# tensor4all/tensor4all-rs

Measured on AMD Instinct MI355X. Metric: TCI2 full-sweep GF/s (d=30, chi=256 fp64), higher is better.
Workload: dtype f64

## Files before the change

include/t4a_gpu.h:

```cpp
#ifndef T4A_GPU_H
#define T4A_GPU_H

#include <stddef.h>
#include <stdint.h>

#ifdef __cplusplus
extern "C" {
#endif
#if defined(__GNUC__)
#pragma GCC visibility push(default)
#endif

typedef int32_t t4a_gpu_status;
#define T4A_GPU_SUCCESS 0
#define T4A_GPU_NULL_POINTER (-1)
#define T4A_GPU_INVALID_ARGUMENT (-2)
#define T4A_GPU_BUFFER_TOO_SMALL (-5)
#define T4A_GPU_INTERNAL_ERROR (-6)
#define T4A_GPU_NOT_IMPLEMENTED (-7)
#define T4A_GPU_NAN_ENCOUNTERED (-8)
#define T4A_GPU_SINGULAR_MATRIX (-9)
#define T4A_GPU_NO_DEVICE (-10)
#define T4A_GPU_KERNEL_TIMEOUT (-11)
#define T4A_GPU_CALLBACK_ERROR (-12)
// ... 372 lines not shown
t4a_gpu_status t4a_gpu_mpo_from_tt(const t4a_gpu_tt* tt, t4a_gpu_mpo** out);
t4a_gpu_status t4a_gpu_mpo_to_tt(const t4a_gpu_mpo* mpo, t4a_gpu_tt** out);
t4a_gpu_status t4a_gpu_mpo_transpose(const t4a_gpu_mpo* mpo, t4a_gpu_mpo** out);

typedef struct t4a_gpu_qt_op t4a_gpu_qt_op;
#define T4A_GPU_QT_PERIODIC 0
#define T4A_GPU_QT_ANTIPERIODIC 1
#define T4A_GPU_QT_OPEN 2
#define T4A_GPU_QT_LOWER 0
#define T4A_GPU_QT_UPPER 1
t4a_gpu_status t4a_gpu_qt_shift_operator(size_t r, int64_t offset, int32_t bc, t4a_gpu_qt_op** out);
t4a_gpu_status t4a_gpu_qt_shift_operator_multivar(size_t r, int64_t offset, int32_t bc, size_t nvariables, size_t target_var,
                                                  t4a_gpu_qt_op** out);
t4a_gpu_status t4a_gpu_qt_flip_operator(size_t r, int32_t bc, t4a_gpu_qt_op** out);
t4a_gpu_status t4a_gpu_qt_flip_operator_multivar(size_t r, int32_t bc, size_t nvariables, size_t target_var, t4a_gpu_qt_op** out);
t4a_gpu_status t4a_gpu_qt_triangle_operator(size_t r, int32_t triangle, t4a_gpu_qt_op** out);
t4a_gpu_status t4a_gpu_qt_cumsum_operator(size_t r, t4a_gpu_qt_op** out);
t4a_gpu_status t4a_gpu_qt_affine_operator(size_t r, const int64_t* a, size_t a_len, const int64_t* b, size_t b_len, int64_t scale,
                                          size_t m, size_t n, const int32_t* bc, size_t n_bc, t4a_gpu_qt_op** out);
void t4a_gpu_qt_op_release(t4a_gpu_qt_op* h);
t4a_gpu_status t4a_gpu_qt_op_len(const t4a_gpu_qt_op* h, size_t* out);
t4a_gpu_status t4a_gpu_qt_op_dims(const t4a_gpu_qt_op* h, size_t* dims4 );
t4a_gpu_status t4a_gpu_qt_op_site_tensor(const t4a_gpu_qt_op* h, size_t site, double* out);
t4a_gpu_status t4a_gpu_qt_op_to_mpo(const t4a_gpu_qt_op* h, t4a_gpu_mpo** out);
t4a_gpu_status t4a_gpu_qt_difference_kernel(const t4a_gpu_tt* f, int32_t bc, t4a_gpu_mpo** out);

t4a_gpu_status t4a_gpu_tt_to_tensors(const t4a_gpu_tt* tt, const int64_t* site_labels, const int64_t* bond_labels,
                                     t4a_gpu_tensor** out);
t4a_gpu_status t4a_gpu_tensors_to_tt(const t4a_gpu_tensor* const* tensors, size_t n_sites, t4a_gpu_tt** out);

typedef struct t4a_gpu_aci_options {
    size_t max_iters;
    size_t min_iters;
    int32_t has_max_bond_dim;
    size_t max_bond_dim;
    double tolerance;
    int32_t scale_tolerance;
    uint64_t rng_seed;
    int32_t enable_global_guard;
    size_t nsearch_global_pivots;
    size_t max_nglobal_pivot;
    size_t nsweeps_global_search;
    double tol_margin_global_search;
} t4a_gpu_aci_options;
t4a_gpu_status t4a_gpu_aci_options_default(t4a_gpu_aci_options* opts);
typedef int32_t (*t4a_gpu_aci_op_fn)(void* user, const double* values, size_t n_inputs, size_t n_points, double* out);
#define T4A_GPU_ACI_OP_CALLBACK 0
#define T4A_GPU_ACI_OP_PRODUCT 1
#define T4A_GPU_ACI_OP_SUM 2
t4a_gpu_status t4a_gpu_aci_elementwise(const t4a_gpu_tt* const* inputs, size_t n_inputs, int32_t op_kind, t4a_gpu_aci_op_fn op,
                                       void* user, const t4a_gpu_aci_options* options, const t4a_gpu_tt* initial_guess,
                                       t4a_gpu_tt** result, size_t* n_iters, size_t* ranks, double* errors,
                                       size_t* nglobal_pivots, int32_t* termination);
typedef struct t4a_gpu_aci_problem t4a_gpu_aci_problem;
t4a_gpu_status t4a_gpu_aci_problem_new(const t4a_gpu_tt* const* inputs, size_t n_inputs, int32_t op_kind, t4a_gpu_aci_op_fn op,
                                       void* user, const t4a_gpu_aci_options* options, const t4a_gpu_tt* initial_guess,
                                       t4a_gpu_aci_problem** out);
void t4a_gpu_aci_problem_release(t4a_gpu_aci_problem* h);
t4a_gpu_status t4a_gpu_aci_problem_local_update(t4a_gpu_aci_problem* h, size_t bond, int32_t left_orthogonal);
t4a_gpu_status t4a_gpu_aci_problem_add_global_pivots(t4a_gpu_aci_problem* h, const size_t* pivots, size_t n_pivots,
                                                     size_t* added);
t4a_gpu_status t4a_gpu_aci_problem_find_global_pivots(t4a_gpu_aci_problem* h, uint64_t seed, size_t* count, size_t* out);
t4a_gpu_status t4a_gpu_aci_problem_solution(t4a_gpu_aci_problem* h, t4a_gpu_tt** out);
t4a_gpu_status t4a_gpu_aci_problem_frame(t4a_gpu_aci_problem* h, int32_t right, size_t input, size_t site, size_t* rows,
                                         size_t* cols, double* out);
t4a_gpu_status t4a_gpu_aci_problem_errors(const t4a_gpu_aci_problem* h, double* pivot_errors, double* pivot_scales);

t4a_gpu_status t4a_gpu_treeaci_local_update_f64(size_t n_inputs, const size_t* bond_dims, const double* const* row_frames,
                                                const double* const* col_frames, size_t row_count, size_t col_count, int32_t op_kind,
                                                t4a_gpu_aci_op_fn op, void* user, size_t max_bond_dim, double tolerance,
                                                int32_t scale_tolerance, int32_t left_orthogonal, size_t* rank, size_t* row_indices,
                                                size_t* col_indices, double* pivot_errors, size_t* n_pivot_errors, double* left,
                                                double* right, double* sampled_scale, double* local_values);

t4a_gpu_status t4a_gpu_tci2_last_sweep_shapes(const t4a_gpu_tci2* h, size_t* out);
#define T4A_GPU_PROFILE_SLOTS 16
t4a_gpu_status t4a_gpu_tci2_profile_enable(t4a_gpu_tci2* h, int32_t enable);
t4a_gpu_status t4a_gpu_tci2_profile_reset(t4a_gpu_tci2* h);
t4a_gpu_status t4a_gpu_tci2_profile_get(const t4a_gpu_tci2* h, double* out );
t4a_gpu_status t4a_gpu_tci2_profile_variants(const t4a_gpu_tci2* h, double* out , size_t cap_rows, size_t* n_rows);

t4a_gpu_status t4a_gpu_tci2_chain_stats(const t4a_gpu_tci2* h, uint64_t* out );
t4a_gpu_status t4a_gpu_tci2_chain_stats_ext(const t4a_gpu_tci2* h, uint64_t* out );
t4a_gpu_status t4a_gpu_tci2_fill_stats(const t4a_gpu_tci2* h, uint64_t* out );
t4a_gpu_status t4a_gpu_tci2_rook_stats(const t4a_gpu_tci2* h, uint64_t* out );
t4a_gpu_status t4a_gpu_tci2_optimize_group(t4a_gpu_tci2* const* handles, size_t n_handles, const t4a_gpu_tci2_options* options,
                                           int32_t final_sweep1site);
t4a_gpu_status t4a_gpu_tci2_fill_site_tensors_group(t4a_gpu_tci2* const* handles, size_t n_handles);
t4a_gpu_status t4a_gpu_tci2_set_chain(t4a_gpu_tci2* h, int32_t enable, int32_t verify);
t4a_gpu_status t4a_gpu_tci2_set_callback_threads(t4a_gpu_tci2* h, size_t n_threads);
t4a_gpu_status t4a_gpu_tci2_small_stats(const t4a_gpu_tci2* h, uint64_t* out );

t4a_gpu_status t4a_gpu_fn_eval(int32_t fid, int32_t n_acc, const double* params, const uint64_t* weights,
                               const size_t* local_dims, size_t n_sites, const size_t* idx, size_t n_pts,
                               double* out);

#if defined(__GNUC__)
#pragma GCC visibility pop
#endif
#ifdef __cplusplus
}
#endif
#endif
```

tensor4all-rs_amd/build.py:

```python
#!/usr/bin/env python3
import os
import subprocess
import sys
from concurrent.futures import ThreadPoolExecutor

HERE = os.path.dirname(os.path.abspath(__file__))
CSRC = os.path.join(HERE, "csrc")
OUT = os.path.join(HERE, "lib")
OBJ = os.path.join(HERE, "build")
SOURCES = ["kernels_rrlu.hip", "kernels_rrlu_reg.hip", "rrlu_xcd_plan.hip", "kernels_rrlu_xcd2.hip", "kernels_rrlu_xcd2_group.hip", "kernels_rrlu_xcd2m.hip", "kernels_rrlu_wg.hip", "kernels_rrlu_wg_group.hip", "kernels_rrlu_w1.hip", "kernels_rrlu_global.hip", "kernels_pi.hip", "kernels_chain.hip", "kernels_small.hip", "kernels_dense.hip", "kernels_linalg.hip",
           "kernels_tt.hip", "kernels_mpo.hip", "pool.hip", "engine.hip", "rook.hip", "tt.hip", "mpo.hip", "globalsearch.hip", "tci2.hip", "tci2_chain.hip", "tci2_small.hip", "conversion.hip", "patching.hip", "tree.hip", "quantics.hip", "tensorops.hip", "aci.hip", "quanticstransform.hip", "capi.hip"]
FLAGS = ["--offload-arch=gfx950", "-O3", "-std=c++17", "-fPIC", "-ffp-contract=off", "-Wall", "-Wno-unused-function",
         "-fvisibility=hidden"] + os.environ.get("T4A_EXTRA_FLAGS", "").split()
FILE_FLAGS = {"kernels_dense.hip": ["-mllvm", "-amdgpu-mfma-vgpr-form=1"], "kernels_linalg.hip": ["-ffp-contract=fast"]}
HEADERS = ["common.hpp", "stdrng.hpp", "pishard.hpp", "kernels.hpp", "kernels_rrlu_xcd_common.hpp", "kernels_rrlu_w1_body.hpp", "engine.hpp", "tci2.hpp", "tt.hpp", "mpo.hpp", "globalsearch.hpp", "rook.hpp", "patching.hpp", "tree.hpp", "quantics.hpp", "tensorops.hpp", "aci.hpp", "quanticstransform.hpp", "../../include/t4a_gpu.h",
           "../../include/t4a_testfunctions.h"]


_INC_CACHE = {}


def _includes(path):
    path = os.path.normpath(path)
    if path in _INC_CACHE:
        return _INC_CACHE[path]
    _INC_CACHE[path] = set()
    found = set()
    try:
        with open(path) as f:
            text = f.read()
    except OSError:
        return found
    import re
    for inc in re.findall(r'^\s*#\s*include\s+"([^"]+)"', text, flags=re.M):
        cand = os.path.normpath(os.path.join(os.path.dirname(path), inc))
        if os.path.exists(cand):
            found.add(cand)
            found |= _includes(cand)
    _INC_CACHE[path] = found
    return found


def _newer(target, deps):
    if not os.path.exists(target):
        return True
    t = os.path.getmtime(target)
    return any(os.path.getmtime(d) > t for d in deps)


def build(force=False, verbose=True):
    hipcc = os.environ.get("HIPCC", "/opt/rocm/bin/hipcc")
    os.makedirs(OUT, exist_ok=True)
    os.makedirs(OBJ, exist_ok=True)
    stamp = os.path.join(OBJ, "flags.stamp")
    flags_now = " ".join(FLAGS) + " | " + repr(sorted(FILE_FLAGS.items()))
    try:
        with open(stamp) as f:
            flags_then = f.read()
    except OSError:
        flags_then = None
    if flags_then != flags_now:
        force = True
    hdrs = [os.path.join(CSRC, h) for h in HEADERS]
    jobs = []
    objs = []
    for s in SOURCES:
        src = os.path.join(CSRC, s)
        obj = os.path.join(OBJ, s.replace(".hip", ".o"))
        objs.append(obj)
        if force or _newer(obj, [src] + sorted(_includes(src))):
            jobs.append([hipcc] + FLAGS + FILE_FLAGS.get(s, []) + ["-c", src, "-o", obj])

    def run(cmd):
        if verbose:
            print(" ".join(cmd), flush=True)
        subprocess.check_call(cmd)

    with ThreadPoolExecutor(max_workers=4) as ex:
        list(ex.map(run, jobs))
    lib = os.path.join(OUT, "libt4a_gpu.so")
    if force or jobs or not os.path.exists(lib):
        run([hipcc, "--offload-arch=gfx950", "-shared", "-fPIC", "-o", lib] + objs)
    with open(stamp, "w") as f:
        f.write(flags_now)
    hooks = os.path.join(OUT, "libt4a_gpu_testhooks.so")
    src = os.path.join(CSRC, "tci2.hip")
    hobj = os.path.join(OBJ, "tci2_testhooks.obj")
    if force or jobs or _newer(hobj, [src] + sorted(_includes(src))) or not os.path.exists(hooks):
        run([hipcc] + FLAGS + ["-DT4A_TEST_HOOKS", "-c", src, "-o", hobj])
        run([hipcc, "--offload-arch=gfx950", "-shared", "-fPIC", "-o", hooks] + [o for o in objs if os.path.basename(o) != "tci2.o"] + [hobj])
    return lib


if __name__ == "__main__":
    print(build(force="--force" in sys.argv))
```

tensor4all-rs_amd/csrc/capi.hip:

```cpp
#include "stdrng.hpp"
#include "smallrng.hpp"
#include <memory>
#include <initializer_list>
#include <mutex>

#include "patching.hpp"
#include "tci2.hpp"
#include "tree.hpp"
#include "quantics.hpp"
#include "tensorops.hpp"
#include "aci.hpp"
#include "globalsearch.hpp"
#include "mpo.hpp"
#include "quanticstransform.hpp"

struct t4a_gpu_tci2 {
    t4a::Tci2 impl;
    explicit t4a_gpu_tci2(const std::vector<size_t>& d) : impl(d) {}
};

struct t4a_gpu_treetci {
    t4a::TreeTci impl;
    t4a_gpu_treetci(const std::vector<size_t>& d, const t4a::TreeGraph& g) : impl(d, g) {}
};
// ... 1084 lines not shown
        h->impl.keep_site_tensors = keep != 0;
    });
}

t4a_gpu_status t4a_gpu_tci2_last_sweep_shapes(const t4a_gpu_tci2* h, size_t* out)
{
    return guarded([&] {
        T4A_REQUIRE_PTR(h);
        T4A_REQUIRE_PTR(out);
        for (size_t b = 0; b < h->impl.last_sweep_shapes.size(); ++b)
            for (int k = 0; k < 3; ++k) out[3 * b + k] = h->impl.last_sweep_shapes[b][k];
    });
}

t4a_gpu_status t4a_gpu_tci2_profile_enable(t4a_gpu_tci2* h, int32_t enable)
{
    return guarded([&] {
        T4A_REQUIRE_PTR(h);
        h->impl.eng.prof.enabled = enable != 0;
    });
}
t4a_gpu_status t4a_gpu_tci2_profile_reset(t4a_gpu_tci2* h)
{
    return guarded([&] {
        T4A_REQUIRE_PTR(h);
        for (double& v : h->impl.eng.prof.v) v = 0.0;
        h->impl.eng.variant_stats_.clear();
    });
}
t4a_gpu_status t4a_gpu_tci2_profile_get(const t4a_gpu_tci2* h, double* out)
{
    return guarded([&] {
        T4A_REQUIRE_PTR(h);
        T4A_REQUIRE_PTR(out);
        for (int i = 0; i < T4A_GPU_PROFILE_SLOTS; ++i) out[i] = h->impl.eng.prof.v[i];
        double best = -1.0;
        for (const auto& kv : h->impl.eng.variant_stats_)
            if (kv.second[0] > best) {
                best = kv.second[0];
                out[12] = kv.second[0];
                out[13] = kv.second[1];
                out[14] = kv.second[2];
                out[15] = (double)kv.first;
            }
    });
}
t4a_gpu_status t4a_gpu_tci2_profile_variants(const t4a_gpu_tci2* h, double* out, size_t cap_rows, size_t* n_rows)
{
    return guarded([&] {
        T4A_REQUIRE_PTR(h);
        T4A_REQUIRE_PTR(n_rows);
        const auto& vs = h->impl.eng.variant_stats_;
        *n_rows = vs.size();
        if (out == nullptr) return;
        if (cap_rows < vs.size()) throw Error(T4A_GPU_BUFFER_TOO_SMALL, "profile_variants: buffer too small");
        size_t i = 0;
        for (const auto& kv : vs) {
            out[5 * i + 0] = (double)kv.first;
            for (int j = 0; j < 4; ++j) out[5 * i + 1 + j] = kv.second[j];
            ++i;
        }
    });
}


t4a_gpu_status t4a_gpu_tci2_chain_stats(const t4a_gpu_tci2* h, uint64_t* out)
{
    return guarded([&] {
        T4A_REQUIRE_PTR(h);
        T4A_REQUIRE_PTR(out);
        for (int k = 0; k < 5; ++k) out[k] = h->impl.chain_stats[k];
    });
}

t4a_gpu_status t4a_gpu_tci2_chain_stats_ext(const t4a_gpu_tci2* h, uint64_t* out)
{
    return guarded([&] {
        T4A_REQUIRE_PTR(h);
        T4A_REQUIRE_PTR(out);
        for (int k = 0; k < 4; ++k) out[k] = h->impl.chain_stats_ext[k];
    });
}

t4a_gpu_status t4a_gpu_tci2_rook_stats(const t4a_gpu_tci2* h, uint64_t* out)
{
    return guarded([&] {
        T4A_REQUIRE_PTR(h);
        T4A_REQUIRE_PTR(out);
        const RookWork& w = h->impl.rook_work();
        out[0] = w.n_device_searches;
        out[1] = w.n_device_visits;
        out[2] = w.n_host_searches;
        out[3] = w.n_host_syncs;
    });
}

t4a_gpu_status t4a_gpu_tci2_fill_stats(const t4a_gpu_tci2* h, uint64_t* out)
{
    return guarded([&] {
        T4A_REQUIRE_PTR(h);
        T4A_REQUIRE_PTR(out);
        for (int k = 0; k < 3; ++k) out[k] = h->impl.fill_stats()[k];
    });
}

t4a_gpu_status t4a_gpu_tci2_set_chain(t4a_gpu_tci2* h, int32_t enable, int32_t verify)
{
    return guarded([&] {
        T4A_REQUIRE_PTR(h);
        h->impl.chain_enabled = enable != 0;
        h->impl.chain_verify = (verify & 1) != 0;
        h->impl.chain_event_timing = (verify & 2) != 0;
        h->impl.small_enabled = (verify & 4) == 0;
        h->impl.small_stamps = (verify & 8) != 0;
        h->impl.fill_graph_relaxed = (verify & 16) != 0;
        h->impl.small_tile_max = (verify & 32) ? 32 : 16;
    });
}

t4a_gpu_status t4a_gpu_tci2_set_callback_threads(t4a_gpu_tci2* h, size_t n_threads)
{
    return guarded([&] {
        T4A_REQUIRE_PTR(h);
        if (n_threads < 1 || n_threads > 256) throw Error(T4A_GPU_INVALID_ARGUMENT, "callback threads: between 1 and 256");
        h->impl.callback_threads = n_threads;
    });
}

t4a_gpu_status t4a_gpu_tci2_small_stats(const t4a_gpu_tci2* h, uint64_t* out)
{
    return guarded([&] {
        T4A_REQUIRE_PTR(h);
        T4A_REQUIRE_PTR(out);
        for (int k = 0; k < 4; ++k) out[k] = h->impl.small_stats[k];
        for (int k = 0; k < 3; ++k) out[4 + k] = h->impl.small_last_clocks_[k];
        out[7] = (uint64_t)h->impl.small_last_reason_;
        for (int k = 0; k < 8; ++k) out[8 + k] = h->impl.small_last_clocks_[3 + k];
    });
}

extern "C++" {
static void rook_outputs(Engine& e, const LuciResult& r, size_t m, size_t n, size_t* rank, size_t* rows, size_t* cols,
                         double* pivot_errors, double* left, double* right)
{
    *rank = (size_t)r.rank;
    for (int i = 0; i < r.rank; ++i) {
        rows[i] = (size_t)r.row_perm[i];
        cols[i] = (size_t)r.col_perm[i];
    }
    for (size_t i = 0; i < r.pivot_errors.size(); ++i) pivot_errors[i] = r.pivot_errors[i];
    if (r.rank > 0) {
        download(e, left, e.left(), m * (size_t)r.rank);
        download(e, right, e.right(), n * (size_t)r.rank);
    }
}
static RookWork& dense_rook_work()
{
    static RookWork w;
    return w;
}
}

t4a_gpu_status t4a_gpu_luci_blocks_f64(size_t m, size_t n, t4a_gpu_fill_block_fn fill_block, void* ctx,
                                       size_t max_bond_dim, double rel_tol, double abs_tol, int32_t left_orthogonal,
                                       size_t* rank, size_t* rows, size_t* cols, double* pivot_errors, double* left,
                                       double* right)
{
    return guarded([&] {
        T4A_REQUIRE_PTR(rank);
        T4A_REQUIRE_PTR(rows);
        T4A_REQUIRE_PTR(cols);
        T4A_REQUIRE_PTR(pivot_errors);
        const size_t count = checked_mul(m, n, "matrix shape");
        require_int_dims({m, n}, "matrix shape");
        if (count) {
            T4A_REQUIRE_PTR(fill_block);
            T4A_REQUIRE_PTR(left);
            T4A_REQUIRE_PTR(right);
        }
        if (m > 65535 || n > 65535) throw Error(T4A_GPU_NOT_IMPLEMENTED, "luci: dimensions above 65535 are not supported");
        std::lock_guard<std::mutex> lock(g_dense_mutex);
        Engine& e = dense_engine();
        hipStream_t st = e.stream();
        std::vector<size_t> all_rows(m), all_cols(n);
        for (size_t i = 0; i < m; ++i) all_rows[i] = i;
        for (size_t j = 0; j < n; ++j) all_cols[j] = j;
        std::vector<double> hbuf(std::max(m, n));
        RookSource src;
        src.M = (int)m;
        src.N = (int)n;
        src.column = [&](int c, double* d_out) {
            const size_t cc = (size_t)c;
            fill_block(ctx, all_rows.data(), m, &cc, 1, hbuf.data());
            T4A_HIP(hipMemcpyAsync(d_out, hbuf.data(), m * sizeof(double), hipMemcpyHostToDevice, st));
            T4A_HIP(hipStreamSynchronize(st));
        };
        src.row = [&](int r, double* d_out) {
            const size_t rr = (size_t)r;
            fill_block(ctx, &rr, 1, all_cols.data(), n, hbuf.data());
// ... 2350 lines not shown
```

tensor4all-rs_amd/csrc/engine.hip:

```cpp
#include "engine.hpp"

#include <algorithm>
#include <cmath>
#include <cstdio>
#include <cstdlib>
#include <cstring>
#include <atomic>
#include <condition_variable>
#include <mutex>

namespace t4a {

namespace {
thread_local std::string g_last_error;

__global__ void __launch_bounds__(256) tri_extract_kernel(const double* __restrict__ in, int ldi, int rows, int cols,
                                                          int keep_lower, int unit_diag, double* __restrict__ out,
                                                          int ldo)
{
    const int i = blockIdx.x * blockDim.x + threadIdx.x;
    if (i >= rows) return;
    for (int j = blockIdx.y; j < cols; j += gridDim.y) {
        double v;
        if (i == j)
// ... 37 lines not shown
                                std::getenv("T4A_WG_MIN") ? std::atol(std::getenv("T4A_WG_MIN")) : 64};
    return env;
}
void acquire_for(XcdArbiter::Lock& lock, RrluLock scope, int xcc)
{
    if (scope != RrluLock::None) lock.acquire(scope == RrluLock::Chip ? -1 : xcc);
}
void reg_args(RrluRegArgs& a, const RrluRoute& rt, bool left, const double* A, int max_steps, double rel_tol, double abs_tol, const RrluBlock& blk)
{
    std::memset(&a, 0, sizeof(a));
    a.A = A;
    a.M = rt.kM;
    a.N = rt.kN;
    a.max_steps = max_steps;
    a.rel_tol = rel_tol;
    a.abs_tol = abs_tol;
    a.tie_row_major = left ? 0 : 1;
    a.out_transposed = left ? 0 : 1;
    a.W = rt.reg.W;
    a.TR = rt.reg.TR;
    a.TC = rt.reg.TC;
    a.row_perm = left ? blk.row_perm() : blk.col_perm();
    a.col_perm = left ? blk.col_perm() : blk.row_perm();
    a.iresult = blk.iresult();
    a.dresult = blk.dresult();
    a.pivot_vals = blk.pivot_vals();
    a.ncopy = 1;
    a.spec = 2;
    a.spec_frac = 0.8;
    a.key16 = 1;
    a.spin_limit = 1u << 20;
    a.h_block = reinterpret_cast<unsigned long long*>(blk.host);
    a.block_u64 = (int)(blk.bytes / 8);
    a.ts_u64 = (int)(blk.off_ts / 8);
}
}

RrluRoute RrluRoute::of_xcd(const RrluXcdPlan& plan, int kM, int kN)
{
    RrluRoute rt;
    rt.kind = plan.wg == 2 ? RrluKind::OneWave : plan.wg ? RrluKind::OneWorkgroup : plan.big() ? RrluKind::MultiXcd : RrluKind::SingleXcd;
    rt.xcd = plan;
    rt.kM = kM;
    rt.kN = kN;
    return rt;
}
RrluRoute RrluRoute::of_reg(const RrluRegPlan& plan, int kM, int kN)
{
    RrluRoute rt;
    rt.kind = RrluKind::Reg;
    rt.reg = plan;
    rt.kM = kM;
    rt.kN = kN;
    rt.fused = plan.RPT * plan.CPT <= RRLU_FUSED_MAX_VALUES;
    return rt;
}
int RrluRoute::code(bool tie_row_major, bool saturated) const
{
    const int tie = tie_row_major ? 4 : 0, sat = saturated ? 10000000 : 0;
    switch (kind) {
    case RrluKind::OneWave: return sat + 300000 + xcd.RPT * 1000 + xcd.CPT * 10 + tie;
    case RrluKind::OneWorkgroup: return sat + 200000 + xcd.RPT * 1000 + xcd.CPT * 10 + tie;
    case RrluKind::SingleXcd: return sat + 100000 + xcd.RPT * 100 + xcd.CPT * 10 + tie;
    case RrluKind::MultiXcd: return sat + 400000 + xcd.K * 10000 + xcd.RPT * 100 + xcd.CPT * 10 + tie;
    case RrluKind::Reg: return sat + reg.RPT * 1000 + reg.CPT * 10 + tie + (reg.W == 1 ? 2 : 0) + ((reg.TR % 64) == 0 ? 1 : 0);
    case RrluKind::Lds: return sat + (lds.W == 1 ? -1 : -2);
    case RrluKind::Global: return sat - 3;
    default: return 0;
    }
}
RrluLock RrluRoute::lock() const
{
    switch (kind) {
    case RrluKind::OneWave:
    case RrluKind::OneWorkgroup:
    case RrluKind::SingleXcd:
    case RrluKind::MultiXcd:
        return xcd.W > kXcdSharedMaxW || xcd.K > 1 ? RrluLock::Chip : RrluLock::Xcd;
    case RrluKind::Reg: return reg.W > 1 ? RrluLock::Chip : RrluLock::None;
    case RrluKind::Lds: return lds.W > 1 ? RrluLock::Chip : RrluLock::None;
    default: return RrluLock::None;
    }
}
size_t RrluRoute::xcd_mailbox_words() const { return (rrlu_xcd_keys_bytes(xcd) + rrlu_xcd_cols_bytes(xcd, kM)) / sizeof(unsigned long long); }
void RrluRoute::launch(const RrluXcdArgs& args, hipStream_t stream) const
{
    switch (kind) {
    case RrluKind::OneWave: rrlu_w1_launch(xcd, args, stream); break;
    case RrluKind::OneWorkgroup: rrlu_wg_launch(xcd, args, stream); break;
    case RrluKind::SingleXcd: rrlu_xcd2_launch(xcd, args, stream); break;
    case RrluKind::MultiXcd: rrlu_xcd2m_launch(xcd, args, stream); break;
    default: throw Error(T4A_GPU_INTERNAL_ERROR, "rrLU: the route has no single-XCD launch");
    }
}
void RrluRoute::launch_group(const RrluXcdGroupArgs& args, bool tie_row_major, hipStream_t stream) const
{
    switch (kind) {
    case RrluKind::OneWave: rrlu_w1_group_launch(xcd, args, tie_row_major, stream); break;
    case RrluKind::OneWorkgroup: rrlu_wg_group_launch(xcd, args, tie_row_major, stream); break;
    case RrluKind::SingleXcd: rrlu_xcd2_group_launch(xcd, args, tie_row_major, stream); break;
    default: throw Error(T4A_GPU_INTERNAL_ERROR, "rrLU: the route has no group launch");
    }
}

RrluBlock RrluBlock::layout(size_t max_steps, size_t M, size_t N, bool with_timestamps)
{
    RrluBlock b;
    b.off_rp = b.off_piv + sizeof(double) * std::max<size_t>(max_steps, 1);
    b.off_cp = b.off_rp + sizeof(int) * M;
    const size_t end = (b.off_cp + sizeof(int) * N + 7) / 8 * 8;
    b.off_ts = with_timestamps ? end : 0;
    b.bytes = with_timestamps ? end + 16 : end;
    return b;
}

namespace {
__global__ void xcd_census_kernel(unsigned* counts)
{
    if (threadIdx.x == 0) {
        unsigned v;
        asm volatile("s_getreg_b32 %0, hwreg(HW_REG_XCC_ID)" : "=s"(v));
        atomicAdd(&counts[v & 0xF], 1u);
        if ((v & 0xF) != (blockIdx.x & 7u)) atomicAdd(&counts[16], 1u);
    }
}
std::once_flag g_census_once;
void xcd_census()
{
    if (g_xcd_disabled.load(std::memory_order_relaxed) || std::getenv("T4A_NO_XCD")) return;
    unsigned* d = nullptr;
    unsigned h[17] = {0};
    if (hipMalloc(&d, sizeof(h)) != hipSuccess) return;
    bool ok = hipMemset(d, 0, sizeof(h)) == hipSuccess;
    if (ok) {
        hipLaunchKernelGGL(xcd_census_kernel, dim3(256), dim3(64), 0, nullptr, d);
        ok = hipMemcpy(h, d, sizeof(h), hipMemcpyDeviceToHost) == hipSuccess;
    }
    (void)hipFree(d);
    if (!ok) {
        (void)hipGetLastError();
        return;
    }
    bool even = true;
    for (int x = 0; x < 8; ++x) even &= (h[x] == 32u);
    if (!even) xcd_disable();
}
}
int xcd_assign() { return g_xcd_next.fetch_add(1, std::memory_order_relaxed) & 7; }
int xcd_plan_max_w() { return g_live_engines.load(std::memory_order_relaxed) > 1 ? kXcdSharedMaxW : 32; }
namespace {
std::mutex g_arb_mutex;
std::condition_variable g_arb_cv;
std::thread::id g_arb_owner[8];
int g_arb_count[8] = {0, 0, 0, 0, 0, 0, 0, 0};
}
void XcdArbiter::Lock::acquire(int xcc)
{
    release();
    const std::thread::id me = std::this_thread::get_id();
    std::unique_lock<std::mutex> lk(g_arb_mutex);
    auto holds_some = [&] {
        for (int i = 0; i < 8; ++i)
            if (g_arb_count[i] > 0 && g_arb_owner[i] == me) return true;
        return false;
    };
    auto take = [&](int i) {
        g_arb_owner[i] = me;
        ++g_arb_count[i];
        held_ |= 1 << i;
    };
    owner_ = me;
    if (xcc >= 0) {
        const int i = xcc & 7;
// ... 501 lines not shown
    a.h_block = reinterpret_cast<unsigned long long*>(blk.host);
    a.block_u64 = (int)(blk.bytes / 8);
    a.ts_u64 = (int)(blk.off_ts / 8);
}

void Engine::rrlu_account(const RrluRoute& rt, bool tie_row_major, int M, int N, int rank, bool record, float ms, bool saturated)
{
    double bytes = 8.0 * M * N, flops = 0.0;
    for (int k = 0; k < rank; ++k) {
        const double mr = (double)(M - k - 1), nr = (double)(N - k - 1);
        bytes += 16.0 * mr * nr;
        flops += 2.0 * mr * nr + mr;
    }
    prof.v[8] += rank;
    prof.v[9] += bytes;
    prof.v[10] += flops;
    if (!record) return;
    auto add = [&](int code) {
        auto& vs = variant_stats_[code];
        vs[0] += ms;
        vs[1] += 1.0;
        vs[2] += bytes;
        vs[3] += rank;
    };
    add(rt.code(tie_row_major));
    if (saturated) add(rt.code(tie_row_major, true));
}

RrluRoute Engine::chain_route(int kM, int kN) const
{
    if (kM < 1 || kN < 1 || kM > 65535 || kN > 65535) return RrluRoute();
    RrluXcdPlan xplan;
    if ((long long)kM * kN > rrlu_env().wg_min && (rrlu_w1_make_plan(kM, kN, &xplan, 63) || rrlu_wg_make_plan(kM, kN, &xplan, 63)))
        return RrluRoute::of_xcd(xplan, kM, kN);
    RrluRegPlan rplan;
    if ((long long)kM * kN <= 64 * 64 && rrlu_reg_make_plan(kM, kN, num_cus_, &rplan) && rplan.W == 1) return RrluRoute::of_reg(rplan, kM, kN);
    if (!xcd_disabled() && (rrlu_xcd_make_plan(kM, kN, &xplan, true, xcd_plan_max_w()) || rrlu_xcd_make_plan(kM, kN, &xplan, true, 32, true)))
        return RrluRoute::of_xcd(xplan, kM, kN);
    return RrluRoute();
}

void Engine::chain_begin(const std::vector<RrluRoute>& routes, size_t reserve_mailbox_words)
{
    chain_group_reserve(routes, reserve_mailbox_words, stream_);
    RrluLock scope = RrluLock::None;
    for (const RrluRoute& rt : routes)
        if (rt.on_xcd()) scope = std::max(scope, rt.lock());
    acquire_for(chain_lock_, scope, xcc_);
}

void Engine::chain_end() { chain_lock_.release(); }

RrluRoute Engine::chain_group_route(int kM, int kN)
{
    if (kM < 1 || kN < 1 || kM > 1024 || kN > 1024 || xcd_disabled()) return RrluRoute();
    RrluXcdPlan xplan;
    if (rrlu_w1_make_plan(kM, kN, &xplan, 0) || rrlu_wg_make_plan(kM, kN, &xplan, 0) || rrlu_xcd_make_plan(kM, kN, &xplan, true, 32))
        return RrluRoute::of_xcd(xplan, kM, kN);
    return RrluRoute();
}

void Engine::chain_group_reserve(const std::vector<RrluRoute>& routes, size_t reserve_mailbox_words, hipStream_t order_stream)
{
    size_t need = 0;
    for (const RrluRoute& rt : routes)
        if (rt.on_xcd()) need = std::max(need, rt.xcd_mailbox_words());
    if (need > 0 && (need > d_xkeys_.cap || !d_xticket_.get())) xcd_mailbox_clear(std::max(need, reserve_mailbox_words), order_stream);
}

unsigned Engine::chain_group_args(const RrluRoute& rt, bool left, const double* d_a, const int* d_dims, size_t max_bond_dim, double rel_tol,
                                  double abs_tol, const RrluBlock& blk, int slot, RrluXcdArgs* out, hipStream_t order_stream)
{
    if (++xcd_salt_ > 65535u) {
        T4A_HIP(hipMemsetAsync(d_xkeys_.get(), 0, d_xkeys_.cap * sizeof(unsigned long long), order_stream));
        xcd_salt_ = 1;
    }
    xcd_args(*out, rt, left, d_a, chain_max_steps(rt, max_bond_dim), rel_tol, abs_tol, blk, slot);
    out->dims = d_dims;
    out->dims_swap = left ? 0 : 1;
    return xcd_salt_;
}

unsigned Engine::chain_rrlu(const RrluRoute& rt, bool left, const double* d_a, const int* d_rowmap, const FusedPi* fused, const int* d_dims,
                            size_t max_bond_dim, double rel_tol, double abs_tol, const RrluBlock& blk, const XcdSpecArgs* spec, double* d_aout, double* d_urows)
{
    unsigned token = 0u;
    if (rt.on_xcd()) {
        RrluXcdArgs a;
        token = chain_group_args(rt, left, d_a, d_dims, max_bond_dim, rel_tol, abs_tol, blk, xcc_, &a, stream_);
        a.rowmap = d_rowmap;
        a.Aout = d_aout;
        a.urows = d_aout ? d_urows : nullptr;
        if (spec) a.spec = *spec;
        rt.launch(a, stream_);
    } else {
        if (++done_token_ == 0u) ++done_token_;
        RrluRegArgs a;
        reg_args(a, rt, left, d_a, chain_max_steps(rt, max_bond_dim), rel_tol, abs_tol, blk);
        a.Aout = d_aout;
        a.salt = 1;
        a.fused = (rt.fused && fused) ? 1 : 0;
        if (a.fused) {
            a.rowacc = fused->d_rowacc;
            a.colacc = fused->d_colacc;
            a.fn = fused->fn;
        }
        a.dims = d_dims;
        a.dims_swap = left ? 0 : 1;
        a.rowmap = a.fused ? nullptr : d_rowmap;
        a.dev_token = done_token_;
        a.done_token = done_token_;
        rrlu_reg_launch(rt.reg, a, stream_, true);
        token = done_token_;
    }
    T4A_HIP(hipGetLastError());
    return token;
}

void Engine::build_factors(const LuciResult& r, bool left_orth) { build_factors_from(d_lu_.get(), d_rowperm_ptr_, d_colperm_ptr_, r.M, r.N, r.rank, left_orth); }

void Engine::build_factors_from(const double* lu, const int* d_rowperm_ptr_, const int* d_colperm_ptr_, int M, int N, int rk, bool left_orth)
{
    d_left_.reserve((size_t)M * (rk > 0 ? rk : 1));
    d_right_.reserve((size_t)N * (rk > 0 ? rk : 1));
    if (rk == 0) return;
    if (luci_factors_small_launch(lu, M, N, rk, d_rowperm_ptr_, d_colperm_ptr_, left_orth, d_left_.get(), d_right_.get(), stream_)) {
        T4A_HIP(hipGetLastError());
        return;
    }
    d_w1_.reserve((size_t)(M > N ? M : N) * rk + (size_t)rk * rk);
    d_w2_.reserve((size_t)(M > N ? M : N) * rk + (size_t)rk * rk);
    d_trsm_.reserve(1);
    h_trsm_.reserve(1);

    if (left_orth) {
        double* Wl = d_w1_.get();
        set_identity_launch(Wl, M, rk, M, stream_);
        if (rk < M) {
            double* Tt = d_w2_.get();
            double* Bt = d_w2_.get() + (size_t)rk * rk;
            transpose_launch(lu, rk, rk, M, Tt, rk, stream_);
            transpose_launch(lu + rk, M - rk, rk, M, Bt, rk, stream_);
            TrsmProblem tp;
            tp.T = Tt;
            tp.ldt = rk;
            tp.n = rk;
            tp.B = Bt;
            tp.ldb = rk;
            tp.nrhs = M - rk;
            tp.lower = 0;
            tp.unit_diag = 1;
            tp.skip_flag = nullptr;
            T4A_HIP(hipStreamSynchronize(stream_));
            *h_trsm_.get() = tp;
            T4A_HIP(hipMemcpyAsync(d_trsm_.get(), h_trsm_.get(), sizeof(TrsmProblem), hipMemcpyHostToDevice, stream_));
            trsm_left_batched_launch(d_trsm_.get(), 1, rk, M - rk, stream_);
            transpose_launch(Bt, rk, M - rk, rk, Wl + rk, M, stream_);
        }
        scatter_rows_launch(Wl, M, d_rowperm_ptr_, M, rk, d_left_.get(), M, stream_);
        double* L11 = d_w2_.get();
        double* Ue = d_w1_.get();
        tri_extract_launch(lu, M, rk, rk, 1, 1, L11, rk, stream_);
        tri_extract_launch(lu, M, rk, N, 0, 0, Ue, rk, stream_);
        double* Rp = d_w2_.get() + (size_t)rk * rk;
        GemmDesc g;
        g.m = rk;
        g.n = N;
        g.k = rk;
        g.A = L11;
        g.lda = rk;
        g.strideA = 0;
        g.transA = 0;
        g.B = Ue;
        g.ldb = rk;
        g.strideB = 0;
        g.transB = 0;
        g.C = Rp;
// ... 270 lines not shown
```

tensor4all-rs_amd/csrc/engine.hpp:

```cpp
#pragma once

#include <array>
#include <functional>
#include <thread>
#include <map>
#include <limits>
#include <vector>

#include "common.hpp"
#include "kernels.hpp"

namespace t4a {

struct RrLUOptions {
    size_t max_bond_dim = std::numeric_limits<size_t>::max();
    double rel_tol = 1e-14;
    double abs_tol = 0.0;
    bool left_orthogonal = true;
};

struct LuciResult {
    int M = 0, N = 0;
    int rank = 0;
    std::vector<int> row_perm, col_perm;
    std::vector<double> pivot_errors;
    double last_error = 0.0;
    double abs_max = 0.0;
    bool has_factors = false;
};

struct FusedPi {
    FnDevice fn;
    const uint64_t* d_rowacc;
    const uint64_t* d_colacc;
    bool host_resident = false;
};

struct Profile {
    double v[T4A_GPU_PROFILE_SLOTS] = {0};
    bool enabled = false;
};

bool xcd_disabled();
void xcd_disable();
int xcd_assign();
int xcd_plan_max_w();
struct XcdArbiter {
    class Lock {
    public:
        Lock() = default;
        Lock(const Lock&) = delete;
        Lock& operator=(const Lock&) = delete;
        ~Lock() { release(); }
        void acquire(int xcc);
        void release();
    private:
        int held_ = 0;
        std::thread::id owner_;
    };
};

enum class RrluKind {
    None,
    OneWave,
    OneWorkgroup,
    SingleXcd,
    MultiXcd,
    Reg,
    Lds,
    Global,
};
enum class RrluLock { None, Xcd, Chip };
struct RrluRoute {
    RrluKind kind = RrluKind::None;
    RrluXcdPlan xcd;
    RrluRegPlan reg;
    RrluPlan lds;
    int kM = 0, kN = 0;
    bool fused = false;

    static RrluRoute of_xcd(const RrluXcdPlan& plan, int kM, int kN);
    static RrluRoute of_reg(const RrluRegPlan& plan, int kM, int kN);
    bool ok() const { return kind != RrluKind::None; }
    bool on_xcd() const { return kind == RrluKind::OneWave || kind == RrluKind::OneWorkgroup || kind == RrluKind::SingleXcd || kind == RrluKind::MultiXcd; }
    int code(bool tie_row_major, bool saturated = false) const;
    RrluLock lock() const;
    size_t xcd_mailbox_words() const;
    void launch(const RrluXcdArgs& args, hipStream_t stream) const;
    void launch_group(const RrluXcdGroupArgs& args, bool tie_row_major, hipStream_t stream) const;
};

struct RrluBlock {
    char* dev = nullptr;
    char* host = nullptr;
    size_t off_piv = 32, off_rp = 0, off_cp = 0, off_ts = 0, bytes = 0;
    static RrluBlock layout(size_t max_steps, size_t M, size_t N, bool with_timestamps);
    double* dresult() const { return reinterpret_cast<double*>(dev); }
    int* iresult() const { return reinterpret_cast<int*>(dev + 16); }
    double* pivot_vals() const { return reinterpret_cast<double*>(dev + off_piv); }
    int* row_perm() const { return reinterpret_cast<int*>(dev + off_rp); }
    int* col_perm() const { return reinterpret_cast<int*>(dev + off_cp); }
};

class Engine {
public:
    Engine();
    ~Engine();
    Engine(const Engine&) = delete;
    Engine& operator=(const Engine&) = delete;

    hipStream_t stream() const { return stream_; }
    int num_cus() const { return num_cus_; }
    void sync() { T4A_HIP(hipStreamSynchronize(stream_)); }

    double* pi(size_t count)
    {
        d_pi_.reserve(count);
        return d_pi_.get();
    }
    double* lu_buf() { return d_lu_.get(); }
    double* left() { return d_left_.get(); }
    double* right() { return d_right_.get(); }
    void reserve_factors(size_t left_count, size_t right_count)
    {
        d_left_.reserve(left_count > 0 ? left_count : 1);
        d_right_.reserve(right_count > 0 ? right_count : 1);
    }

    LuciResult luci(const double* d_a, int M, int N, const RrLUOptions& opts, bool need_factors, bool want_lu_copy,
                    const FusedPi* fused = nullptr);

    void lu_permuted_factors(const LuciResult& r, bool left_orth);

    static constexpr size_t FACTOR_DIM_MAX = 65535;
    static void require_factor_dims(size_t m, size_t n, const std::string& what)
    {
        if (m > FACTOR_DIM_MAX || n > FACTOR_DIM_MAX)
            throw Error(T4A_GPU_NOT_IMPLEMENTED, what + " above " + std::to_string(FACTOR_DIM_MAX) + " are not supported");
    }
    void svd(const double* d_a, int M, int N, double* d_u, double* d_s, double* d_vt);
    void svd_plain(const double* d_a, int M, int N, double* d_u, double* d_s, double* d_vt);
    void svd_in_range(const double* d_a, int M, int N, double* d_u, double* d_s, double* d_vt);
    void qr(const double* d_a, int M, int N, double* d_q, double* d_r);

    RrluRoute chain_route(int kM, int kN) const;
    void chain_begin(const std::vector<RrluRoute>& routes, size_t reserve_mailbox_words = 0);
    unsigned chain_rrlu(const RrluRoute& rt, bool left, const double* d_a, const int* d_rowmap, const FusedPi* fused, const int* d_dims,
                        size_t max_bond_dim, double rel_tol, double abs_tol, const RrluBlock& blk, const XcdSpecArgs* spec, double* d_aout = nullptr, double* d_urows = nullptr);
    void chain_end();
    static RrluRoute chain_group_route(int kM, int kN);
    void chain_group_reserve(const std::vector<RrluRoute>& routes, size_t reserve_mailbox_words, hipStream_t order_stream);
    void chain_group_lock() { chain_lock_.acquire(-1); }
    unsigned chain_group_args(const RrluRoute& rt, bool left, const double* d_a, const int* d_dims, size_t max_bond_dim, double rel_tol,
                              double abs_tol, const RrluBlock& blk, int slot, RrluXcdArgs* out, hipStream_t order_stream);
    void rrlu_account(const RrluRoute& rt, bool tie_row_major, int M, int N, int rank, bool record, float ms, bool saturated);
    int xcc() const { return xcc_; }
    void set_xcc(int xcc) { xcc_ = xcc & 7; }

    std::function<void()> overlap_hook;

    Profile prof;
    std::map<int, std::array<double, 4>> variant_stats_;

    DevBuf<double> d_tmp, d_tmp2;

private:
    RrluRoute luci_route(int M, int N, bool left) const;
    void build_factors(const LuciResult& r, bool left_orth);
public:
    void build_factors_from(const double* d_lu, const int* d_rowperm, const int* d_colperm, int M, int N, int rank, bool left_orth);
private:

    XcdArbiter::Lock chain_lock_;
    hipStream_t stream_ = nullptr;
    int num_cus_ = 0;
    unsigned rrlu_salt_ = 0;
    int xcc_ = 0;
    bool nonfinite_retry_ = false;
    unsigned xcd_salt_ = 0, xcd_ticket_base_ = 0, xcd_ticket_base_multi_ = 0;
    void xcd_take_tickets(const RrluXcdPlan& plan, RrluXcdArgs& a);
    void xcd_mailbox_clear(size_t words, hipStream_t stream);
    void xcd_args(RrluXcdArgs& a, const RrluRoute& rt, bool left, const double* A, int max_steps, double rel_tol, double abs_tol,
                  const RrluBlock& blk, int xcc);
    DevBuf<unsigned long long> d_xkeys_;
    DevBuf<unsigned> d_xticket_;
    DevBuf<double> d_xurows_;
    bool header_clean_ = false, keys_clean_ = false;
    unsigned done_token_ = 0;
    DevBuf<uint64_t> d_accstage_;
    char* header_ptr_ = nullptr;
    int key_parity_ = 0;
    DevBuf<double> d_pi_, d_lu_, d_left_, d_right_, d_w1_, d_w2_, d_at_;
    DevBuf<char> d_out_;
    PinBuf<char> h_out_;
    int* d_rowperm_ptr_ = nullptr;
    int* d_colperm_ptr_ = nullptr;
    DevBuf<unsigned long long> d_keys_, d_cols_, d_rkeys_, d_rcols_, d_stamps_;
    DevBuf<TrsmProblem> d_trsm_;
    PinBuf<TrsmProblem> h_trsm_;
    DevBuf<int> d_gints_;
    DevBuf<double> d_gdbls_;
    EventTimer ev_rrlu_, ev_fac_;
#ifdef T4A_RRLU_TRACE
    DevBuf<unsigned long long> d_trace_;
    int trace_dumps_ = 0;
#endif
    DevBuf<double> d_sw_, d_sv_, d_su_, d_svs_, d_ssig_;
    DevBuf<double> d_pa_, d_pq_, d_pr_, d_pl_, d_pul_, d_pvl_, d_pu_;
    size_t svd_sweeps_last_ = 0;
    DevBuf<int> d_sflags_;
    DevBuf<unsigned long long> d_sabs_;
    DevBuf<double> d_sscaled_;
};

void tri_extract_launch(const double* in, int ldi, int rows, int cols, int keep_lower, int unit_diag, double* out,
                        int ldo, hipStream_t stream);

}
```

tensor4all-rs_amd/csrc/kernels.hpp:

```cpp
#pragma once

#include <hip/hip_runtime.h>

#include <cstddef>
#include <cstdint>

#include "../../include/t4a_testfunctions.h"

namespace t4a {

struct RrluWorkspace;

struct RrluPlan {
    int W = 1;
    int T = 256;
    int cpw = 0;
    int Mld = 0;
    size_t lds_bytes = 0;
};

RrluPlan rrlu_make_plan(int M, int N, int num_cus);

struct RrluArgs {
    const double* A;
// ... 74 lines not shown
    double* pivot_vals;
    unsigned long long* keys;
    unsigned long long* cols;
    unsigned salt;
    int col_delay;
    int poll_delay;
    int ncopy;
    int key16;
    int spec;
    double spec_frac;
    unsigned spin_limit;
    unsigned long long* stamps;
    unsigned long long* h_block;
    int block_u64;
    unsigned long long* keys_next;
    int keys_next_u64;
    unsigned long long* trace;
    int fused;
    const uint64_t* rowacc;
    const uint64_t* colacc;
    FnDevice fn;
    unsigned done_token;
    const int* dims;
    int dims_swap;
    unsigned dev_token;
    const int* rowmap;
    int ts_u64;
};
bool rrlu_reg_make_plan(int M, int N, int num_cus, RrluRegPlan* out);
size_t rrlu_reg_keys_bytes(const RrluRegPlan& plan);
size_t rrlu_reg_cols_bytes(const RrluRegPlan& plan, int M);
void rrlu_reg_launch(const RrluRegPlan& plan, const RrluRegArgs& args, hipStream_t stream, bool keys_zeroed = false);

struct XcdSpecArgs {
    double* out;
    const uint64_t* dep_acc;
    const uint64_t* w_site;
    const uint64_t* ext_acc;
    const int* ext_cnt;
    const uint64_t* ind_acc;
    const int* ind_cnt;
    unsigned* tile_counter;
    int total, d;
    FnDevice fn;
};
struct RrluXcdPlan {
    int W = 1;
    int RPT = 1, CPT = 1;
    int grid = 8;
    size_t lds_bytes = 0;
    int wg = 0;
    int K = 1;
    bool big() const { return K > 1 || RPT > 16; }
};
struct RrluXcdArgs {
    const double* A;
    double* Aout;
    double* urows;
    int M, N;
    int max_steps;
    double rel_tol, abs_tol;
    int tie_row_major;
    int out_transposed;
    int W;
    int xcc;
    unsigned* ticket;
    unsigned ticket_base;
    int* row_perm;
    int* col_perm;
    int* iresult;
    double* dresult;
    double* pivot_vals;
    unsigned long long* keys;
    unsigned salt;
    double spec_frac;
    unsigned long long* stamps;
    unsigned long long* h_block;
    int block_u64;
    const int* dims;
    int dims_swap;
    const int* rowmap;
    XcdSpecArgs spec;
    int ts_u64;
};
bool rrlu_xcd_make_plan(int M, int N, RrluXcdPlan* out, bool any_size = false, int max_w = 32, bool allow_big = false);
size_t rrlu_xcd_keys_bytes(const RrluXcdPlan& plan);
size_t rrlu_xcd_cols_bytes(const RrluXcdPlan& plan, int M);
struct RrluXcdGroupArgs {
    RrluXcdArgs p[8];
};
void rrlu_xcd2_launch(const RrluXcdPlan& plan, const RrluXcdArgs& args, hipStream_t stream);
void rrlu_xcd2m_launch(const RrluXcdPlan& plan, const RrluXcdArgs& args, hipStream_t stream);
void rrlu_xcd2_group_launch(const RrluXcdPlan& plan, const RrluXcdGroupArgs& args, bool tie_row_major, hipStream_t stream);
bool rrlu_wg_make_plan(int M, int N, RrluXcdPlan* out, int spec_blocks = 0);
void rrlu_wg_launch(const RrluXcdPlan& plan, const RrluXcdArgs& args, hipStream_t stream);
void rrlu_wg_group_launch(const RrluXcdPlan& plan, const RrluXcdGroupArgs& args, bool tie_row_major, hipStream_t stream);
bool rrlu_w1_make_plan(int M, int N, RrluXcdPlan* out, int spec_blocks = 0);
void rrlu_w1_launch(const RrluXcdPlan& plan, const RrluXcdArgs& args, hipStream_t stream);
void rrlu_w1_group_launch(const RrluXcdPlan& plan, const RrluXcdGroupArgs& args, bool tie_row_major, hipStream_t stream);

void pi_eval_launch(const FnDevice& fn, const uint64_t* rowacc, int M, const uint64_t* colacc, int N, double* out,
                    int ld, bool transpose_out, unsigned long long* max_abs_bits, hipStream_t stream);
struct PiJob {
    const uint64_t* rowacc;
    const uint64_t* colacc;
    double* out;
    unsigned long long* max_abs_bits;
    int M, N, ld, pad_;
};
void pi_eval_batched_launch(const FnDevice& fn, const PiJob* d_jobs, int n_jobs, int max_M, int max_N, hipStream_t stream);
struct PackJob {
    const double* src;
    double* core;
    const int* info;
    int ld, L, S, R, last, pad_;
};
struct LuProblem;
constexpr int FILL_SMALL_MAX_N = 32, FILL_SMALL_MAX_RHS = 64;
void fill_small_launch(const FnDevice& fn, const PiJob* d_pis, const LuProblem* d_lups, const PackJob* d_packs, int n_jobs, int last_site,
                       hipStream_t stream);
void stage_copy_launch(const uint64_t* pinned_src, uint64_t* dst, size_t count, hipStream_t stream);
void absmax_launch(const double* data, size_t count, unsigned long long* max_abs_bits, hipStream_t stream);

constexpr int CHAIN_MAX_SET = 1024;
struct ChainTab {
    uint64_t* code;
    uint64_t* acc;
    int* cnt;
};
struct ChainCommon {
    ChainTab I, J, HI, HJ;
    ChainTab mI, mJ;
    int cap, K;
    const uint64_t* w;
    int total;
    const int* ldim;
    const int* woff;
    int forward, use_extras;
    int one_site;
    uint64_t* ind_code;
    uint64_t* ind_acc;
    int* ind_cnt;
    int ind_cap;
    uint64_t* dep_code;
    uint64_t* dep_acc;
    int dep_cap;
    int* rowmap;
    int* dims;
    int* hdims;
    uint64_t* snap_dst;
    int* snap_cnt_dst;
    size_t snap_words;
    int n_sites;
    uint64_t* zero_a;
    size_t zero_a_words;
    uint64_t* zero_b;
    size_t zero_b_words;
};
struct ChainPrepArgs {
    int b;
    int do_build;
    int with_rowmap;
    int prev_b;
    const int* prev_iresult;
    const int* prev_rowperm;
    const int* prev_colperm;
    unsigned prev_token;
    unsigned long long* dbg;
    int defer_host_writes;
};
struct ChainWalkArgs {
    char* blocks;
    size_t block_bytes, off_piv, off_rp, off_cp, off_ts;
    double* pi;
    int n_bonds;
    int max_steps;
    double rel_tol, abs_tol;
    double* factors;
    size_t factors_stride;
    unsigned token_base;
    int timed;
    int lean_prep;
    unsigned long long* phase_ticks;
};
void chain_walk_launch(const ChainCommon& c, const FnDevice& fn, const ChainWalkArgs& w, int columns, hipStream_t stream);
void chain_indep_launch(const ChainCommon& c, int n_bonds, hipStream_t stream);
void chain_last_core_launch(const ChainCommon& c, const FnDevice& fn, double* core, int max_entries, hipStream_t stream);
void chain_prep_launch(const ChainCommon& c, const ChainPrepArgs& a, hipStream_t stream);
void chain_pi_launch(const ChainCommon& c, const FnDevice& fn, int b, int n_dep_ub, int n_ind_ub, double* out, hipStream_t stream);

constexpr int CHAIN_GROUP_MAX = 8;
struct ChainGroupSlot {
    ChainCommon c;
    FnDevice fn;
    double* pi;
};
struct ChainPrepGroupArgs {
    ChainPrepArgs a[CHAIN_GROUP_MAX];
};
void chain_indep_group_launch(const ChainGroupSlot* d_slots, int n_handles, int n_bonds, hipStream_t stream);
void chain_prep_group_launch(const ChainGroupSlot* d_slots, const ChainPrepGroupArgs& a, int n_handles, hipStream_t stream);
void chain_pi_group_launch(const ChainGroupSlot* d_slots, int n_handles, int b, int n_dep_ub, int n_ind_ub, hipStream_t stream);

struct GemmDesc {
    int m, n, k;
    const double* A; int lda; long long strideA; int transA;
    const double* B; int ldb; long long strideB; int transB;
    double* C; int ldc; long long strideC;
    double alpha, beta;
    int batch;
    int ksplit = 1;
    double* partial = nullptr;
};
void gemm_launch(const GemmDesc& d, hipStream_t stream);

constexpr int LUCI_LEFT_CORES_MAX_JOBS = 80;
constexpr int LUCI_LEFT_CORES_MAX_RANK = 16;
struct LeftCoreJob {
    const double* lu;
    const int* dims;
    const int* iresult;
    const int* row_perm;
    double* core;
    int S;
    unsigned token;
};
struct LeftCoreJobs {
    LeftCoreJob j[LUCI_LEFT_CORES_MAX_JOBS];
};
void luci_left_cores_batched_launch(const LeftCoreJobs& jobs, int n_jobs, int max_rows, hipStream_t stream);
bool luci_factors_small_launch(const double* lu, int M, int N, int rk, const int* row_perm, const int* col_perm, bool left_orth,
                               double* left, double* right, hipStream_t stream);
void transpose_launch(const double* in, int rows, int cols, int ldi, double* out, int ldo, hipStream_t stream);

struct TrsmProblem {
    const double* T; int ldt; int n;
    double* B; int ldb; int nrhs;
    int lower; int unit_diag;
    const int* skip_flag;
};
void trsm_left_batched_launch(const TrsmProblem* d_problems, int n_problems, int max_n, int max_nrhs, hipStream_t stream);

struct LuProblem {
    double* A; int lda; int n;
    int* piv;
    int* info;
    double* B; int ldb; int nrhs;
    const unsigned long long* pmax_bits;
};
void lu_batched_launch(const LuProblem* d_problems, int n_problems, int max_n, hipStream_t stream);
constexpr int LU_MAX_PANEL_STEPS = 128;
bool lu_forward_blocked_launch(const LuProblem* d_problems, int n_problems, int max_n, int max_nrhs, hipStream_t stream, int avoid_xcc = -1,
// ... 121 lines not shown
```

tensor4all-rs_amd/csrc/kernels_chain.hip:

```cpp
#include "kernels.hpp"
#include "kernels_rrlu_w1_body.hpp"

namespace t4a {

namespace {

__device__ __forceinline__ const char* chain_kernarg_base()
{
#if defined(__HIP_DEVICE_COMPILE__)
    return (const char*)__builtin_amdgcn_kernarg_segment_ptr();
#else
    return nullptr;
#endif
}

constexpr int CHAIN_T = 1024;
constexpr int WALK_T = 1024;
constexpr int CHAIN_HASH = 4096;

__device__ __forceinline__ unsigned chain_hash(unsigned long long c)
{
    c ^= c >> 33;
    c *= 0xff51afd7ed558ccdull;
    c ^= c >> 29;
    return (unsigned)c & (CHAIN_HASH - 1);
}

__device__ __forceinline__ int block_scan_flag(bool flag, int* wave_sums, int* total)
{
    const int lane = threadIdx.x & 63, wave = threadIdx.x >> 6;
    const unsigned long long bal = __ballot(flag);
    const int before = __builtin_popcountll(bal & ((1ull << lane) - 1ull));
    __syncthreads();
    if (lane == 0) wave_sums[wave] = __builtin_popcountll(bal);
    __syncthreads();
    int base = 0, tot = 0;
    for (int w = 0; w < (int)blockDim.x / 64; ++w) {
        const int v = wave_sums[w];
        if (w < wave) base += v;
        tot += v;
    }
    *total = tot;
    return base + before;
}

template <bool PARENT_OUTER>
__device__ int build_side(const uint64_t* __restrict__ pcode, const uint64_t* __restrict__ pacc, int np, int d,
                          const uint64_t* __restrict__ w, int K, int total_w, int w_off, const uint64_t* __restrict__ ecode,
                          const uint64_t* __restrict__ eacc, int ne, uint64_t* __restrict__ ocode, uint64_t* __restrict__ oacc, int ocap,
                          const int* srcpos, int n_prev, int* __restrict__ rowmap, unsigned long long* hkeys, int* wave_sums)
{
    const int tid = threadIdx.x;
    const int m0 = np * d;
    if (m0 > ocap) return -1;
    if (ne > 0) {
        for (int e = tid; e < CHAIN_HASH; e += (int)blockDim.x) hkeys[e] = 0ull;
        __syncthreads();
    }
    for (int idx = tid; idx < m0; idx += (int)blockDim.x) {
        const int i = PARENT_OUTER ? idx / d : idx % np;
        const int s = PARENT_OUTER ? idx % d : idx / np;
        const uint64_t c = pcode[i];
        ocode[idx] = (uint64_t)s + (uint64_t)d * c;
        for (int k = 0; k < K; ++k) oacc[(size_t)idx * K + k] = pacc[(size_t)i * K + k] + w[(size_t)k * total_w + w_off + s];
        if (rowmap) rowmap[idx] = srcpos[i] * d + s;
    }
    if (ne <= 0) return m0;
    for (int i = tid; i < np; i += (int)blockDim.x) {
        const unsigned long long key = (unsigned long long)pcode[i] + 1ull;
        unsigned h = chain_hash(key);
        for (;;) {
            const unsigned long long old = atomicCAS(&hkeys[h], 0ull, key);
            if (old == 0ull || old == key) break;
            h = (h + 1) & (CHAIN_HASH - 1);
        }
    }
    __syncthreads();
    int count = m0;
    for (int base = 0; base < ne; base += (int)blockDim.x) {
        const int e = base + tid;
        bool keep = false;
        uint64_t c = 0ull;
        if (e < ne) {
            c = ecode[e];
            const unsigned long long key = (unsigned long long)(c / (uint64_t)d) + 1ull;
            unsigned h = chain_hash(key);
            keep = true;
            for (;;) {
                const unsigned long long v = hkeys[h];
                if (v == 0ull) break;
                if (v == key) {
                    keep = false;
                    break;
                }
                h = (h + 1) & (CHAIN_HASH - 1);
            }
        }
        int tot = 0;
        const int pos = block_scan_flag(keep, wave_sums, &tot);
        if (count + tot > ocap) return -1;
        if (keep) {
            const int o = count + pos;
            ocode[o] = c;
            for (int k = 0; k < K; ++k) oacc[(size_t)o * K + k] = eacc[(size_t)e * K + k];
            if (rowmap) rowmap[o] = n_prev * d + e;
        }
        count += tot;
    }
    return count;
}

__device__ __forceinline__ void chain_indep_body(const ChainCommon& c)
{
    __shared__ unsigned long long hkeys[CHAIN_HASH];
    __shared__ int wave_sums[CHAIN_T / 64];
    const int b = blockIdx.x;
    const int K = c.K;
    const size_t cap = (size_t)c.cap;
    uint64_t* ocode = c.ind_code + (size_t)b * c.ind_cap;
    uint64_t* oacc = c.ind_acc + (size_t)b * c.ind_cap * K;
    int n;
    if (c.one_site) {
        const ChainTab& T = c.forward ? c.J : c.I;
        const int site = c.forward ? b : b + 1;
        const int np = T.cnt[site];
        n = (np >= 1 && np <= c.cap && np <= c.ind_cap) ? np : -1;
        for (int i = threadIdx.x; i < n; i += (int)blockDim.x) {
            ocode[i] = T.code[(size_t)site * cap + i];
            for (int k = 0; k < K; ++k) oacc[(size_t)i * K + k] = T.acc[((size_t)site * cap + i) * K + k];
        }
    } else if (c.forward) {
        const int np = c.J.cnt[b + 1], ne = c.use_extras ? c.HJ.cnt[b] : 0;
        n = (np >= 1 && np <= c.cap && ne <= c.cap)
                ? build_side<false>(c.J.code + (size_t)(b + 1) * cap, c.J.acc + (size_t)(b + 1) * cap * K, np, c.ldim[b + 1], c.w, K, c.total,
                                    c.woff[b + 1], c.HJ.code + (size_t)b * cap, c.HJ.acc + (size_t)b * cap * K, ne, ocode, oacc, c.ind_cap,
                                    nullptr, 0, nullptr, hkeys, wave_sums)
                : -1;
    } else {
        const int np = c.I.cnt[b], ne = c.use_extras ? c.HI.cnt[b + 1] : 0;
        n = (np >= 1 && np <= c.cap && ne <= c.cap)
                ? build_side<true>(c.I.code + (size_t)b * cap, c.I.acc + (size_t)b * cap * K, np, c.ldim[b], c.w, K, c.total, c.woff[b],
                                   c.HI.code + (size_t)(b + 1) * cap, c.HI.acc + (size_t)(b + 1) * cap * K, ne, ocode, oacc, c.ind_cap,
                                   nullptr, 0, nullptr, hkeys, wave_sums)
                : -1;
    }
    if (threadIdx.x == 0) c.ind_cnt[b] = n;
    const size_t gtid = (size_t)blockIdx.x * blockDim.x + threadIdx.x, gsz = (size_t)gridDim.x * blockDim.x;
    if (c.snap_dst) {
        for (size_t i = gtid; i < c.snap_words; i += gsz) c.snap_dst[i] = c.I.code[i];
        for (size_t i = gtid; i < (size_t)2 * c.n_sites; i += gsz) c.snap_cnt_dst[i] = c.I.cnt[i];
    }
    for (size_t i = gtid; i < c.zero_a_words; i += gsz) c.zero_a[i] = 0ull;
    for (size_t i = gtid; i < c.zero_b_words; i += gsz) c.zero_b[i] = 0ull;
}
__global__ void __launch_bounds__(CHAIN_T) chain_indep_kernel(ChainCommon c) { chain_indep_body(c); }
__global__ void __launch_bounds__(CHAIN_T) chain_indep_group_kernel(const ChainGroupSlot* __restrict__ slots)
{
    chain_indep_body(slots[blockIdx.y].c);
}

constexpr int WALK_MAX_BONDS = 128;
constexpr int WALK_MAX_LIST = 64;
constexpr int WALK_MAX_IND = 32;
constexpr int WALK_MAX_W = 512;
struct WalkShared {
    int prev_ires[4];
    int perm_rp[WALK_MAX_LIST], perm_cp[WALK_MAX_LIST];
    int np;
    int pad_;
    uint64_t par_code[WALK_MAX_LIST], par_acc[WALK_MAX_LIST * T4A_FN_MAX_ACC];
    uint64_t dep_code[WALK_MAX_LIST], dep_acc[WALK_MAX_LIST * T4A_FN_MAX_ACC];
    int dims[WALK_MAX_BONDS * 4];
    int ind_cnt[WALK_MAX_BONDS];
    uint64_t ind_code[2][WALK_MAX_IND], ind_acc[2][WALK_MAX_IND * T4A_FN_MAX_ACC];
    uint64_t ext_code[2][WALK_MAX_LIST], ext_acc[2][WALK_MAX_LIST * T4A_FN_MAX_ACC];
    int ext_cnt[2];
    int ldim[WALK_MAX_BONDS + 1], woff[WALK_MAX_BONDS + 1];
    uint64_t w[WALK_MAX_W];
};

__device__ __forceinline__ void chain_prep_body(const ChainCommon& c, const ChainPrepArgs& p, unsigned long long* dbg = nullptr, WalkShared* ws = nullptr)
{
    unsigned long long dbg_last = dbg ? wall_clock64() : 0ull;
    auto stamp = [&](int slot) {
        if (dbg) {
            const unsigned long long now = wall_clock64();
            if (threadIdx.x == 0) dbg[slot] += now - dbg_last;
            dbg_last = now;
        }
    };
    __shared__ unsigned long long hkeys[CHAIN_HASH];
    __shared__ int wave_sums[CHAIN_T / 64];
    __shared__ int s_srcpos[CHAIN_MAX_SET];
// ... 590 lines not shown
```

tensor4all-rs_amd/csrc/kernels_rrlu_xcd2.hip:

```cpp
#include "kernels_rrlu_xcd_common.hpp"

namespace t4a {

namespace {

template <int RPT, int KX = 1> struct Xcd2Lds {
    static constexpr int LSTR = xcd_lstr(RPT);
    static constexpr int TBL = xcd2_tbl(RPT, KX);
    static constexpr int o_l = 0;
    static constexpr int o_wd = o_l + 64 * LSTR * 8;
    static constexpr int o_wi = o_wd + 16;
    static constexpr int o_pp = o_wi + 64;
    static constexpr int o_st = o_pp + 16;
    static constexpr int o_pv = o_st + 128;
    static constexpr int o_pr = o_pv + TBL * 8;
    static constexpr int o_rp = o_pr + TBL * 2;
    static constexpr int o_pc = o_rp + TBL * 2;
    static constexpr int o_cp = o_pc + TBL * 2;
    static constexpr int bytes = o_cp + TBL * 2;
};
static_assert(Xcd2Lds<12>::bytes == (int)xcd_lds_total(12), "plan.lds_bytes must cover the layout");
static_assert(Xcd2Lds<24>::bytes == (int)xcd2_lds_total(24), "plan.lds_bytes must cover the layout (plans beyond 1024 rows)");
static_assert(Xcd2Lds<16, 3>::bytes == (int)xcd2_lds_total(16, 3), "plan.lds_bytes must cover the layout (plans beyond 1024 columns)");

#ifndef T4A_XCD_STAMP_WAVE
#define T4A_XCD_STAMP_WAVE 0
#endif

constexpr unsigned X2_META_VALID = 1u << 13;
constexpr unsigned X2_ROW_MASK = 2047u;
constexpr int X2_QSHIFT = 11, X2_PSHIFT = 11;

constexpr int X2_DIVW = XWAVES - 1;

template <int RPT, int CPT, bool ROWMAJOR, int KX = 1>
__device__ __forceinline__ void rrlu_xcd2_body(const RrluXcdArgs& p, const RrluXcdArgs* pk)
{
    static_assert(XWAVES == 8, "the second-generation kernel is written for eight waves per workgroup");
    static_assert(KX >= 1 && KX <= 3, "instantiated for up to three XCDs");
    constexpr int ST_AUX = KX > 1 ? BUF_SC1 : 0;
    extern __shared__ __attribute__((aligned(16))) char smem_raw[];
    using L = Xcd2Lds<RPT, KX>;
    constexpr int LSTR = L::LSTR;
    constexpr int MP = 64 * RPT;
    double* const lbuf = reinterpret_cast<double*>(smem_raw + L::o_l);
    int* const ctl = reinterpret_cast<int*>(smem_raw + L::o_wi);
    unsigned long long* const lds_ptrs = reinterpret_cast<unsigned long long*>(smem_raw + L::o_pp);
    unsigned long long* const lds_stamps = reinterpret_cast<unsigned long long*>(smem_raw + L::o_st);
    double* const lds_pivots = reinterpret_cast<double*>(smem_raw + L::o_pv);
    unsigned short* const posrow = reinterpret_cast<unsigned short*>(smem_raw + L::o_pr);
    unsigned short* const rowpos = reinterpret_cast<unsigned short*>(smem_raw + L::o_rp);
    unsigned short* const poscol = reinterpret_cast<unsigned short*>(smem_raw + L::o_pc);
    unsigned short* const colpos = reinterpret_cast<unsigned short*>(smem_raw + L::o_cp);

    const int tid = threadIdx.x;
    const int lane = tid & 63;
    const int wave = __builtin_amdgcn_readfirstlane(tid >> 6);
    const unsigned long long t_entry = (kXcdStamps && p.stamps) ? __builtin_amdgcn_s_memtime() : 0ull;

    if (tid == 0) {
        int rank = -1;
        if constexpr (KX == 1) {
            if ((int)xcc_id() == p.xcc) {
                const unsigned t = atomicAdd(p.ticket, 1u) - p.ticket_base;
                if (t < (unsigned)p.W) rank = (int)t;
            }
        } else {
            const unsigned x = xcc_id() & 7u;
            const unsigned t = atomicAdd(p.ticket + x, 1u) - p.ticket_base;
            const unsigned xi = (x - (unsigned)p.xcc) & 7u;
            if (xi < (unsigned)KX && t < (unsigned)p.W) rank = (int)(xi * (unsigned)p.W + t);
        }
        ctl[3] = rank;
        ctl[0] = 0;
        ctl[1] = 0;
        ctl[2] = 0;
        for (int e = 8; e < 16; ++e) ctl[e] = 0;
        lds_ptrs[0] = (unsigned long long)p.iresult;
        lds_ptrs[1] = (unsigned long long)p.h_block;
        for (int e = 0; e < 16; ++e) lds_stamps[e] = 0ull;
    }
    __syncthreads();
    const int rank = __builtin_amdgcn_readfirstlane(ctl[3]);
    if (rank < 0) {
        if (p.spec.out && p.dims) {
            const int m_spec = p.dims[2] != 0 ? 0 : (p.dims_swap ? p.dims[1] : p.dims[0]);
            if (m_spec > 0 && m_spec <= p.M)
                xcd_spec_work(reinterpret_cast<const XcdSpecArgs*>(kernarg_base() + offsetof(RrluXcdArgs, spec)), m_spec, ctl + 8);
        }
        return;
    }
    const unsigned long long ts_begin = p.ts_u64 > 0 ? wall_clock64() : 0ull;
    const unsigned long long t_elected = (kXcdStamps && p.stamps) ? __builtin_amdgcn_s_memtime() : 0ull;
    const int NWL = p.W * XWAVES;
    const int NW = KX * NWL;
    const int g = rank * XWAVES + wave;
    const bool poller = wave == 0;
    const int xi = KX > 1 ? rank / p.W : 0;
    const int pbase = xi * NWL;
    int M = p.M, N = p.N, max_steps = p.max_steps;
    int lda = p.M;
    if (p.dims) {
        const int d0 = __builtin_amdgcn_readfirstlane(p.dims[0]), d1 = __builtin_amdgcn_readfirstlane(p.dims[1]);
        M = p.dims_swap ? d1 : d0;
        N = p.dims_swap ? d0 : d1;
        if (M > p.M || N > p.N) M = N = 0;
        const int mn = M < N ? M : N;
        max_steps = max_steps < mn ? max_steps : mn;
        if (mn <= 0) return;
        lda = p.rowmap ? __builtin_amdgcn_readfirstlane(p.dims[3]) : M;
    }
    M = __builtin_amdgcn_readfirstlane(M);
    N = __builtin_amdgcn_readfirstlane(N);
    max_steps = __builtin_amdgcn_readfirstlane(max_steps);
    lda = __builtin_amdgcn_readfirstlane(lda);

    unsigned active = 0u;
#pragma unroll
    for (int q = 0; q < CPT; ++q)
        if (g + NW * q < N) active |= 1u << q;
    XSlab<RPT> a[CPT];
    double local_sqmax = 0.0;
    bool bad = false;
    int srow[RPT];
    unsigned rowmask = 0u;
#pragma unroll
    for (int r = 0; r < RPT; ++r) {
        const int i = lane + 64 * r;
        const bool rok = i < M;
        rowmask |= rok ? (1u << r) : 0u;
        srow[r] = rok ? i : 0;
        if (p.rowmap) srow[r] = p.rowmap[rok ? i : 0];
    }
#pragma unroll
    for (int q = 0; q < CPT; ++q) {
        const bool cok = g + NW * q < N;
        const double* const colp = p.A + (cok ? (size_t)(g + NW * q) * lda : (size_t)0);
        const unsigned rm = (unsigned)opaque_v((int)rowmask);
#pragma unroll
        for (int r = 0; r < RPT; ++r) a[q].set(r, colp[(cok && ((rm >> r) & 1u)) ? srow[r] : 0]);
    }
#pragma unroll
    for (int q = 0; q < CPT; ++q) {
        const bool cok = g + NW * q < N;
        const unsigned rm = (unsigned)opaque_v((int)rowmask);
#pragma unroll
        for (int r = 0; r < RPT; ++r) {
            const bool ok = cok && ((rm >> r) & 1u);
            const double v = ok ? a[q].get(r) : 0.0;
            const double sqv = v * v;
            if (sqv > local_sqmax) local_sqmax = sqv;
            bad |= !((v - v) == 0.0);
            a[q].set(r, v);
        }
    }
    for (int i = tid; i < M; i += XT) {
        posrow[i] = (unsigned short)i;
        rowpos[i] = (unsigned short)i;
    }
    for (int j = tid; j < N; j += XT) {
        poscol[j] = (unsigned short)j;
        colpos[j] = (unsigned short)j;
    }
    for (int e = tid; e < 64 * LSTR; e += XT) lbuf[e] = 0.0;
    {
        const double wm = wave_max_f64(sqrt(local_sqmax));
        if (lane == 0 && wm > 0.0)
            atomicMax((unsigned long long*)&p.dresult[1], (unsigned long long)__double_as_longlong(wm));
    }
    const unsigned wave_bad = __ballot(bad) != 0ull ? 1u : 0u;
    __syncthreads();

    const bool stamp_on = kXcdStamps && (p.stamps != nullptr) && rank == 0 && tid == 64 * T4A_XCD_STAMP_WAVE;
    unsigned long long stamp_last = stamp_on ? __builtin_amdgcn_s_memtime() : 0ull;
    const unsigned long long t_loop = stamp_last;

    const unsigned k2_base = 2u * (unsigned)NW * 16u;
    const unsigned cols_base = 4u * (unsigned)NW * 16u;
    const unsigned fin_base = cols_base + 2u * (unsigned)NW * (unsigned)(MP / 16) * 256u;
    const unsigned k3_base = fin_base + 256u;
    const __amdgpu_buffer_rsrc_t mail =
        __builtin_amdgcn_make_buffer_rsrc((void*)p.keys, 0, (int)(k3_base + (KX > 1 ? 2u * (unsigned)NW * 16u : 0u)), 0x00020000);

    int npiv = 0;
    double max_error = 0.0;
    double error = __builtin_nan("");
    bool timed_out = false;
    const double min_pivot_abs = (p.rel_tol == 0.0 && p.abs_tol == 0.0) ? 0.0 : 2.220446049250313e-16;
    double u[CPT];
#pragma unroll
    for (int q = 0; q < CPT; ++q) u[q] = 0.0;
    double prev_sq = __builtin_huge_val();
    double spec_frac = p.spec_frac, rel_tol_v = p.rel_tol, abs_tol_v = p.abs_tol;
    asm volatile("" : "+v"(spec_frac), "+v"(rel_tol_v), "+v"(abs_tol_v));
    constexpr unsigned XSPIN = 1u << 20;

    double mq[CPT];
#pragma unroll
    for (int q = 0; q < CPT; ++q) {
        mq[q] = -1.0;
        if (active & (1u << q)) {
            double m0 = -1.0, m1 = -1.0;
#pragma unroll
            for (int r = 0; r < RPT; ++r) {
                if (r & 1) m1 = vmax_abs(m1, a[q].get(r));
                else m0 = vmax_abs(m0, a[q].get(r));
            }
            mq[q] = vmax(m0, m1);
        }
    }
    constexpr int XR = (RPT + X2_DIVW - 1) / X2_DIVW;
    const int sr0 = wave - 1;

    for (int kn = 0; kn < max_steps; ++kn) {
        const int k = kn - 1;
        const int par = kn & 1;
        const unsigned tag = (p.salt << 16) | (unsigned)(kn + 1);
        double m = mq[0];
#pragma unroll
        for (int q = 1; q < CPT; ++q) m = vmax(m, mq[q]);
        const int whi = wave_max_i32((int)hi32(m));
        const unsigned long long whb = __ballot((int)hi32(m) == whi);
        const bool hi_single = __builtin_popcountll(whb) == 1;
        const double wmax = hi_single ? readlane_f64(m, (int)__builtin_ctzll(whb)) : wave_max_f64(m);
        const double sq = wmax * wmax;
        const int kslot = (par * NW + g) * 16;
        {
            const double k1 = (wmax >= 0.0) ? wmax : 0.0;
            u32x4 kv;
            kv.x = lo32(k1);
            kv.y = hi32(k1);
            kv.z = wave_bad;
            kv.w = tag ^ kv.x ^ kv.y ^ kv.z;
            if (lane == 0) __builtin_amdgcn_raw_buffer_store_b128(kv, mail, kslot, 0, 0);
        }
        u32x4 kg[4], kh[4];
        bool has_cand = false;
        double cval = 0.0;
        int cirow = 0, qstar = 0;
        if (wmax >= 0.0) {
            bool done = false;
            if (hi_mid(whi)) {
                unsigned long long bq[CPT];
                int nhit = 0;
#pragma unroll
                for (int q = 0; q < CPT; ++q) {
                    bq[q] = __ballot(mq[q] == wmax);
                    nhit += __builtin_popcountll(bq[q]);
                }
                if (nhit == 1) {
#pragma unroll
                    for (int q = 0; q < CPT; ++q)
                        if (bq[q] != 0ull) {
                            const int hl = (int)__builtin_ctzll(bq[q]);
                            unsigned bits = 0u;
#pragma unroll
                            for (int r = 0; r < RPT; ++r)
                                asm("v_cmp_eq_f64 vcc, |%1|, %2\n\tv_addc_co_u32 %0, vcc, %0, %0, vcc" : "+v"(bits) : "v"((double)a[q].get(r)), "s"(wmax) : "vcc");
                            const unsigned hb_ = (unsigned)__builtin_amdgcn_readlane((int)bits, hl);
                            if (__builtin_popcount(hb_) == 1) {
                                const int rstar = RPT - 1 - (int)__builtin_ctz(hb_);
                                cirow = hl + 64 * rstar;
                                has_cand = true;
                                cval = readlane_f64(a[q].dyn(rstar), hl);
                                qstar = q;
// ... 342 lines not shown
                *reinterpret_cast<int4*>(ctl + 4) = rec;
            }
            XSTAMP(9);
        }
        __syncthreads();
        XSTAMP(3);
        int4 rec;
        {
            int zero = 0;
            asm volatile("ds_read_b128 %0, %1 offset:%2\n\ts_waitcnt lgkmcnt(0)" : "=&v"(rec) : "v"(zero), "n"(L::o_wi + 16) : "memory");
        }
        const unsigned recw = (unsigned)__builtin_amdgcn_readfirstlane(rec.x);
        if (recw >> 30) {
            timed_out = true;
            break;
        }
        const int wag = (int)recw;
        if (g == wag && !early_pub) {
            if (qstar == 0) xcd_publish_column<0, RPT, ST_AUX>(a[0], mail, myslot, tag, 4 * CS);
            if constexpr (CPT > 1) if (qstar == 1) xcd_publish_column<1, RPT, ST_AUX>(a[1], mail, myslot, tag, 4 * CS);
            if constexpr (CPT > 2) if (qstar == 2) xcd_publish_column<2, RPT, ST_AUX>(a[2], mail, myslot, tag, 4 * CS);
            if constexpr (CPT > 3) if (qstar == 3) xcd_publish_column<3, RPT, ST_AUX>(a[3], mail, myslot, tag, 4 * CS);
        }
        const int slot_off = (int)cols_base + (par * NW + wag) * SLOTB + ((lane >> 4) + 4 * sr0) * CS + (lane & 15) * 16;
        u32x4 cc[XR];
#pragma unroll
        for (int j = 0; j < XR; ++j)
            if (sr0 >= 0 && sr0 + X2_DIVW * j < RPT) cc[j] = __builtin_amdgcn_raw_buffer_load_b128(mail, slot_off + j * X2_DIVW * 4 * CS, 0, BUF_SC1);
        int rk_ = 0, ck_ = 0;
        int prp_ = 0, pcp_ = 0;
        if (wave == 0) {
            rk_ = posrow[kn];
            ck_ = poscol[kn];
            prp_ = rowpos[rec.w & (int)X2_ROW_MASK];
            pcp_ = colpos[min(wag + NW * ((rec.w >> X2_QSHIFT) & 3), N - 1)];
        }
        const double wval = mk_f64((unsigned)__builtin_amdgcn_readfirstlane(rec.y), (unsigned)__builtin_amdgcn_readfirstlane(rec.z));
        const unsigned wmeta = (unsigned)__builtin_amdgcn_readfirstlane(rec.w);
        const int irow_p = (int)(wmeta & X2_ROW_MASK);
        const int qslot = (int)((wmeta >> X2_QSHIFT) & 3u);
        XSTAMP(10);
        const bool p_mid = exp_mid(wval);
        double rp = refined_rcp(wval);
        asm volatile("" : "+v"(rp));
        prev_sq = wval * wval;
        {
            const int ls = irow_p & 63, rs = irow_p >> 6;
            double ue[CPT];
#pragma unroll
            for (int q = 0; q < CPT; ++q) ue[q] = a[q].dyn(rs);
#pragma unroll
            for (int q = 0; q < CPT; ++q) u[q] = readlane_f64(ue[q], ls);
            if (p.urows) {
#pragma unroll
                for (int q = 0; q < CPT; ++q)
                    if ((active & (1u << q)) && lane == ls) p.urows[(unsigned)(kn * N + (g + NW * q))] = u[q];
            }
        }
        if (g == wag) active &= ~(1u << qslot);
        if (wave == 0) {
            const double wsq = wval * wval;
            double pivot_abs = __builtin_fabs(wval);
            if (!(wsq >= 2.2250738585072014e-308 && wsq < __builtin_huge_val())) pivot_abs = sqrt(mk_f64((unsigned)opaque_v((int)lo32(wsq)), hi32(wsq)));
            error = pivot_abs;
            int stop = 0;
            if (kn > 0 && (pivot_abs < rel_tol_v * max_error || pivot_abs < abs_tol_v)) stop = 1;
            else if (pivot_abs <= min_pivot_abs) stop = 1;
            else max_error = fmax(max_error, pivot_abs);
            if (lane == 0) {
                if (stop) {
                    ctl[0] = 1;
                } else {
                    const int prp = prp_, pcp = pcp_;
                    const int pc = wag + NW * qslot;
                    posrow[prp] = (unsigned short)rk_;
                    posrow[kn] = (unsigned short)irow_p;
                    rowpos[rk_] = (unsigned short)prp;
                    rowpos[irow_p] = (unsigned short)kn;
                    poscol[pcp] = (unsigned short)ck_;
                    poscol[kn] = (unsigned short)pc;
                    colpos[ck_] = (unsigned short)pcp;
                    colpos[pc] = (unsigned short)kn;
                    lds_pivots[kn] = wval;
                }
            }
        }
        XSTAMP(11);

        if (sr0 >= 0) {
            unsigned spins = 0;
            for (;;) {
                bool ok = true;
#pragma unroll
                for (int j = 0; j < XR; ++j)
                    if (sr0 + X2_DIVW * j < RPT) ok &= ((cc[j].x ^ cc[j].y ^ cc[j].z ^ cc[j].w) == tag);
                if (__all(ok)) break;
                xcd_poll_again();
                if (++spins > XSPIN) {
                    atomicExch(reinterpret_cast<int*>(lds_ptrs[0]) + 1, 1);
                    if (lds_ptrs[1]) reinterpret_cast<volatile int*>(lds_ptrs[1])[5] = 1;
                    ctl[1] = 1;
                    break;
                }
#pragma unroll
                for (int j = 0; j < XR; ++j)
                    if (sr0 + X2_DIVW * j < RPT) cc[j] = __builtin_amdgcn_raw_buffer_load_b128(mail, slot_off + j * X2_DIVW * 4 * CS, 0, BUF_SC1);
            }
            XSTAMP(12);
            double lq[XR];
            bool slow = false;
#pragma unroll
            for (int j = 0; j < XR; ++j) {
                lq[j] = 0.0;
                if (sr0 + X2_DIVW * j < RPT) {
                    const double x = mk_f64(cc[j].x, cc[j].y);
                    const double q0 = x * rp;
                    const double qf = __builtin_fma(__builtin_fma(-wval, q0, x), rp, q0);
                    lq[j] = (x == 0.0) ? q0 : qf;
                    slow |= (__builtin_fabs(x) < 4.909093465297727e-91) & (x != 0.0);
                }
            }
            slow |= !p_mid;
            if (__ballot(slow) != 0ull) {
#pragma unroll
                for (int j = 0; j < XR; ++j)
                    if (sr0 + X2_DIVW * j < RPT) {
                        const double x = mk_f64(cc[j].x, cc[j].y);
                        if (!(p_mid & (exp_mid(x) | (x == 0.0)))) lq[j] = x / wval;
                    }
            }
#pragma unroll
            for (int j = 0; j < XR; ++j)
                if (sr0 + X2_DIVW * j < RPT) lbuf[lane * LSTR + sr0 + X2_DIVW * j] = lq[j];
        }
        XSTAMP(4);
        __syncthreads();
        XSTAMP(13);
        int2 fl;
        {
            static_assert(L::o_wi % 8 == 0, "the verdict pair is read with one 8-byte LDS load");
            int zero = 0;
            asm volatile("ds_read_b64 %0, %1 offset:%2" : "=&v"(fl) : "v"(zero), "n"(L::o_wi) : "memory");
        }
        constexpr int NH = RPT > 16 ? 2 : 1, HR = RPT / NH;
        static_assert(RPT % NH == 0, "row slots split evenly into the halves of the l read");
        xvec<HR> l;
#pragma unroll
        for (int r = 0; r < HR; ++r) l[r] = lbuf[lane * LSTR + r];
        {
            asm volatile("s_waitcnt lgkmcnt(%1)" : "+v"(fl) : "n"((HR + 1) / 2) : "memory");
            if (__builtin_amdgcn_readfirstlane(fl.y)) {
                timed_out = true;
                break;
            }
            if (__builtin_amdgcn_readfirstlane(fl.x)) break;
        }
        XSTAMP(7);
        if constexpr (NH == 1) {
#pragma unroll
            for (int q = 0; q < CPT; ++q) {
                mq[q] = -1.0;
                if (active & (1u << q)) {
#pragma unroll
                    for (int r = 0; r < RPT; ++r) {
                        double t = a[q].get(r);
                        sub_in_place(t, l[r] * u[q]);
                        a[q].set(r, t);
                    }
                    double m0 = -1.0, m1 = -1.0;
#pragma unroll
                    for (int r = 0; r < RPT; ++r) {
                        if (r & 1) m1 = vmax_abs(m1, a[q].get(r));
                        else m0 = vmax_abs(m0, a[q].get(r));
                    }
                    mq[q] = vmax(m0, m1);
                }
            }
        } else {
            double m0[CPT], m1[CPT];
#pragma unroll
            for (int q = 0; q < CPT; ++q) m0[q] = m1[q] = -1.0;
#pragma unroll
            for (int h = 0; h < NH; ++h) {
                if (h > 0) {
                    asm volatile("" ::: "memory");
#pragma unroll
                    for (int r = 0; r < HR; ++r) l[r] = lbuf[lane * LSTR + h * HR + r];
                }
#pragma unroll
                for (int q = 0; q < CPT; ++q) {
                    if (active & (1u << q)) {
#pragma unroll
                        for (int r = 0; r < HR; ++r) {
                            double t = a[q].get(h * HR + r);
                            sub_in_place(t, l[r] * u[q]);
                            a[q].set(h * HR + r, t);
                        }
#pragma unroll
                        for (int r = 0; r < HR; ++r) {
                            if (r & 1) m1[q] = vmax_abs(m1[q], a[q].get(h * HR + r));
                            else m0[q] = vmax_abs(m0[q], a[q].get(h * HR + r));
                        }
                    }
                }
            }
#pragma unroll
            for (int q = 0; q < CPT; ++q) mq[q] = (active & (1u << q)) ? vmax(m0[q], m1[q]) : -1.0;
        }
        npiv = kn + 1;
        XSTAMP(0);
    }

    const RrluXcdArgs* pe_ptr = pk;
    asm volatile("" : "+s"(pe_ptr));
    const RrluXcdArgs& pe = *pe_ptr;
    const int Me = opaque_s(M), Ne = opaque_s(N);
    const unsigned long long t_done = stamp_on ? __builtin_amdgcn_s_memtime() : 0ull;
    __syncthreads();
    if (ctl[1]) timed_out = true;
    if (npiv >= (Me < Ne ? Me : Ne)) error = 0.0;
    if (rank == 0 && tid == 0) {
        pe.iresult[0] = npiv;
        pe.dresult[0] = error;
    }
    if (stamp_on) {
        for (int e = 0; e < 16; ++e) pe.stamps[e] = lds_stamps[e];
        pe.stamps[16] = t_elected - t_entry;
        pe.stamps[17] = t_loop - t_elected;
        pe.stamps[18] = t_done - t_loop;
    }
    if (timed_out) return;
    if (rank == 0) {
        int* const h_rp = pe.h_block ? reinterpret_cast<int*>(reinterpret_cast<char*>(pe.h_block) + (reinterpret_cast<const char*>(pe.row_perm) - reinterpret_cast<const char*>(pe.dresult))) : nullptr;
        int* const h_cp = pe.h_block ? reinterpret_cast<int*>(reinterpret_cast<char*>(pe.h_block) + (reinterpret_cast<const char*>(pe.col_perm) - reinterpret_cast<const char*>(pe.dresult))) : nullptr;
        for (int i = tid; i < Me; i += XT) {
            const int v = posrow[i];
            pe.row_perm[i] = v;
            if (h_rp) h_rp[i] = v;
        }
        for (int j = tid; j < Ne; j += XT) {
            const int v = poscol[j];
            pe.col_perm[j] = v;
            if (h_cp) h_cp[j] = v;
        }
        unsigned long long* const h_pv = pe.h_block ? pe.h_block + (reinterpret_cast<const char*>(pe.pivot_vals) - reinterpret_cast<const char*>(pe.dresult)) / 8 : nullptr;
        for (int e = tid; e < npiv; e += XT) {
            const double v = lds_pivots[e];
            pe.pivot_vals[e] = v;
            if (h_pv) h_pv[e] = (unsigned long long)__double_as_longlong(v);
        }
    }
    int nan_seen = 0;
#pragma unroll
    for (int q = 0; q < CPT; ++q)
#pragma unroll
        for (int r = 0; r < RPT; ++r) {
            const int i = lane + 64 * r;
            if (g + NW * q < Ne && i < Me) {
                const int cp = colpos[g + NW * q], rp = rowpos[i];
                const bool from_u = (rp < npiv) && (cp >= rp);
                double v = a[q].get(r);
                const bool in_l = (cp < npiv) && (rp > cp);
                if (in_l) {
                    const double pv = lds_pivots[cp];
                    v = xcd_div(v, pv, refined_rcp(pv), exp_mid(pv));
                    if (v != v) nan_seen = 1;
                }
                if (pe.Aout) {
                    if (from_u)
                        v = __longlong_as_double((long long)__hip_atomic_load(
                            reinterpret_cast<const unsigned long long*>(pe.urows) + ((size_t)rp * Ne + (g + NW * q)), __ATOMIC_RELAXED,
                            __HIP_MEMORY_SCOPE_AGENT));
                    if (pe.out_transposed)
                        pe.Aout[(size_t)rp * Ne + cp] = v;
                    else
                        pe.Aout[(size_t)cp * Me + rp] = v;
                }
            }
        }
    if (nan_seen) {
        atomicExch(&pe.iresult[2], 1);
        if (pe.h_block) ((volatile int*)pe.h_block)[6] = 1;
    }
    if (pe.h_block && rank == 0 && tid == 0) {
        pe.h_block[0] = (unsigned long long)__double_as_longlong(error);
        pe.h_block[1] = __hip_atomic_load(reinterpret_cast<const unsigned long long*>(pe.dresult) + 1, __ATOMIC_RELAXED, __HIP_MEMORY_SCOPE_AGENT);
        ((volatile int*)pe.h_block)[4] = npiv;
        ((volatile int*)pe.h_block)[7] = (int)pe.salt;
        if (pe.ts_u64 > 0) {
            pe.h_block[pe.ts_u64] = ts_begin;
            pe.h_block[pe.ts_u64 + 1] = wall_clock64();
        }
        reinterpret_cast<unsigned long long*>(pe.dresult)[1] = 0ull;
        if (pe.dims) {
            __threadfence();
            pe.iresult[3] = (int)pe.salt;
        }
        if (stamp_on) pe.stamps[19] = __builtin_amdgcn_s_memtime() - t_done;
    }
    if (!pe.h_block && pe.dims && rank == 0 && tid == 0) {
        if (pe.ts_u64 > 0) {
            unsigned long long* const blk = reinterpret_cast<unsigned long long*>(pe.dresult);
            blk[pe.ts_u64] = ts_begin;
            blk[pe.ts_u64 + 1] = wall_clock64();
        }
        __threadfence();
        pe.iresult[3] = (int)pe.salt;
    }
}

#if defined(T4A_XCD2_MULTI_TU)
template <int RPT, int CPT, bool ROWMAJOR, int KX>
__global__ void __launch_bounds__(XT) __attribute__((amdgpu_waves_per_eu(XWAVES / 4, XWAVES / 4))) rrlu_xcd2m_kernel(RrluXcdArgs p)
{
    rrlu_xcd2_body<RPT, CPT, ROWMAJOR, KX>(p, reinterpret_cast<const RrluXcdArgs*>(kernarg_base()));
}
template <int RPT, int CPT, bool ROWMAJOR, int KX> void xcd2m_launch_tie(const RrluXcdPlan& plan, const RrluXcdArgs& a, hipStream_t stream)
{
    static std::once_flag attr_once;
    std::call_once(attr_once, [] {
        (void)hipFuncSetAttribute(reinterpret_cast<const void*>(&rrlu_xcd2m_kernel<RPT, CPT, ROWMAJOR, KX>),
                                  hipFuncAttributeMaxDynamicSharedMemorySize, 160 * 1024);
    });
    hipLaunchKernelGGL((rrlu_xcd2m_kernel<RPT, CPT, ROWMAJOR, KX>), dim3(plan.grid), dim3(XT), plan.lds_bytes, stream, a);
}
template <int RPT, int CPT, int KX> bool xcd2m_launch_rc(const RrluXcdPlan& plan, const RrluXcdArgs& a, hipStream_t stream)
{
    if (plan.RPT != RPT || plan.CPT != CPT || plan.K != KX) return false;
    if (a.tie_row_major) xcd2m_launch_tie<RPT, CPT, true, KX>(plan, a, stream);
    else xcd2m_launch_tie<RPT, CPT, false, KX>(plan, a, stream);
    return true;
}
#elif !defined(T4A_XCD_GROUP_TU)
template <int RPT, int CPT, bool ROWMAJOR>
__global__ void __launch_bounds__(XT) __attribute__((amdgpu_waves_per_eu(XWAVES / 4, XWAVES / 4))) rrlu_xcd2_kernel(RrluXcdArgs p)
{
    rrlu_xcd2_body<RPT, CPT, ROWMAJOR>(p, reinterpret_cast<const RrluXcdArgs*>(kernarg_base()));
}
template <int RPT, int CPT, bool ROWMAJOR> void xcd2_launch_tie(const RrluXcdPlan& plan, const RrluXcdArgs& a, hipStream_t stream)
{
    static std::once_flag attr_once;
    std::call_once(attr_once, [] {
        (void)hipFuncSetAttribute(reinterpret_cast<const void*>(&rrlu_xcd2_kernel<RPT, CPT, ROWMAJOR>),
                                  hipFuncAttributeMaxDynamicSharedMemorySize, 160 * 1024);
    });
    hipLaunchKernelGGL((rrlu_xcd2_kernel<RPT, CPT, ROWMAJOR>), dim3(plan.grid), dim3(XT), plan.lds_bytes, stream, a);
}

template <int RPT, int CPT> void xcd2_launch_rc(const RrluXcdPlan& plan, const RrluXcdArgs& a, hipStream_t stream)
{
    if (a.tie_row_major) xcd2_launch_tie<RPT, CPT, true>(plan, a, stream);
    else xcd2_launch_tie<RPT, CPT, false>(plan, a, stream);
}

template <int RPT> void xcd2_launch_r(const RrluXcdPlan& plan, const RrluXcdArgs& a, hipStream_t stream)
{
    switch (plan.CPT) {
    case 1: xcd2_launch_rc<RPT, 1>(plan, a, stream); break;
    case 2: xcd2_launch_rc<RPT, 2>(plan, a, stream); break;
    case 3: if constexpr (RPT * 3 <= XCD_MAX_VALUES) xcd2_launch_rc<RPT, 3>(plan, a, stream); break;
    default: if constexpr (RPT * 4 <= XCD_MAX_VALUES) xcd2_launch_rc<RPT, 4>(plan, a, stream); break;
    }
}

#else
template <int RPT, int CPT, bool ROWMAJOR>
__global__ void __launch_bounds__(XT) __attribute__((amdgpu_waves_per_eu(XWAVES / 4, XWAVES / 4))) rrlu_xcd2_group_kernel(RrluXcdGroupArgs g)
{
    (void)g;
    const unsigned x = (unsigned)__builtin_amdgcn_readfirstlane((int)xcc_id()) & 7u;
    const RrluXcdArgs* const slot = reinterpret_cast<const RrluXcdArgs*>(kernarg_base() + (size_t)x * sizeof(RrluXcdArgs));
    rrlu_xcd2_body<RPT, CPT, ROWMAJOR>(*slot, slot);
}

template <int RPT, int CPT, bool ROWMAJOR> void xcd2_group_launch_tie(const RrluXcdPlan& plan, const RrluXcdGroupArgs& a, hipStream_t stream)
{
    static std::once_flag attr_once;
    std::call_once(attr_once, [] {
        (void)hipFuncSetAttribute(reinterpret_cast<const void*>(&rrlu_xcd2_group_kernel<RPT, CPT, ROWMAJOR>),
                                  hipFuncAttributeMaxDynamicSharedMemorySize, 160 * 1024);
    });
    hipLaunchKernelGGL((rrlu_xcd2_group_kernel<RPT, CPT, ROWMAJOR>), dim3(plan.grid), dim3(XT), plan.lds_bytes, stream, a);
}
template <int RPT, int CPT> void xcd2_group_launch_rc(const RrluXcdPlan& plan, const RrluXcdGroupArgs& a, bool row_major, hipStream_t stream)
{
    if (row_major) xcd2_group_launch_tie<RPT, CPT, true>(plan, a, stream);
    else xcd2_group_launch_tie<RPT, CPT, false>(plan, a, stream);
}
template <int RPT> void xcd2_group_launch_r(const RrluXcdPlan& plan, const RrluXcdGroupArgs& a, bool row_major, hipStream_t stream)
{
    switch (plan.CPT) {
    case 1: xcd2_group_launch_rc<RPT, 1>(plan, a, row_major, stream); break;
    case 2: xcd2_group_launch_rc<RPT, 2>(plan, a, row_major, stream); break;
    case 3: if constexpr (RPT * 3 <= XCD_MAX_VALUES) xcd2_group_launch_rc<RPT, 3>(plan, a, row_major, stream); break;
    default: if constexpr (RPT * 4 <= XCD_MAX_VALUES) xcd2_group_launch_rc<RPT, 4>(plan, a, row_major, stream); break;
    }
}

#endif

}

#if defined(T4A_XCD2_MULTI_TU)
void rrlu_xcd2m_launch(const RrluXcdPlan& plan, const RrluXcdArgs& a, hipStream_t stream)
{
    const bool ok = xcd2m_launch_rc<24, 1, 1>(plan, a, stream) || xcd2m_launch_rc<24, 2, 1>(plan, a, stream) ||
                    xcd2m_launch_rc<16, 2, 3>(plan, a, stream) || xcd2m_launch_rc<24, 2, 3>(plan, a, stream) ||
                    xcd2m_launch_rc<16, 3, 2>(plan, a, stream) || xcd2m_launch_rc<24, 2, 2>(plan, a, stream);
    if (!ok) throw std::runtime_error("no kernel instantiation for this multi-XCD rrLU plan");
}
#elif !defined(T4A_XCD_GROUP_TU)
void rrlu_xcd2_launch(const RrluXcdPlan& plan, const RrluXcdArgs& a, hipStream_t stream)
{
    switch (plan.RPT) {
#ifdef T4A_XCD_DEV
    case 2: xcd2_launch_r<2>(plan, a, stream); break;
    default: xcd2_launch_r<12>(plan, a, stream); break;
#else
    case 1: xcd2_launch_r<1>(plan, a, stream); break;
    case 2: xcd2_launch_r<2>(plan, a, stream); break;
    case 3: xcd2_launch_r<3>(plan, a, stream); break;
    case 4: xcd2_launch_r<4>(plan, a, stream); break;
    case 6: xcd2_launch_r<6>(plan, a, stream); break;
    case 8: xcd2_launch_r<8>(plan, a, stream); break;
    case 12: xcd2_launch_r<12>(plan, a, stream); break;
    default: xcd2_launch_r<16>(plan, a, stream); break;
#endif
    }
}
#else
void rrlu_xcd2_group_launch(const RrluXcdPlan& plan, const RrluXcdGroupArgs& a, bool tie_row_major, hipStream_t stream)
{
    switch (plan.RPT) {
    case 1: xcd2_group_launch_r<1>(plan, a, tie_row_major, stream); break;
    case 2: xcd2_group_launch_r<2>(plan, a, tie_row_major, stream); break;
    case 3: xcd2_group_launch_r<3>(plan, a, tie_row_major, stream); break;
    case 4: xcd2_group_launch_r<4>(plan, a, tie_row_major, stream); break;
    case 6: xcd2_group_launch_r<6>(plan, a, tie_row_major, stream); break;
    case 8: xcd2_group_launch_r<8>(plan, a, tie_row_major, stream); break;
    case 12: xcd2_group_launch_r<12>(plan, a, tie_row_major, stream); break;
    default: xcd2_group_launch_r<16>(plan, a, tie_row_major, stream); break;
    }
}
#endif

}
```

tensor4all-rs_amd/csrc/tci2.hpp:

```cpp
#pragma once

#include <memory>
#include <vector>

#include "engine.hpp"
#include "stdrng.hpp"
#include "pishard.hpp"
#include "rook.hpp"
#include "tt.hpp"

namespace t4a {

struct IndexSet {
    size_t width = 0;
    size_t count = 0;
    std::vector<uint32_t> d;
    const uint32_t* at(size_t k) const { return d.data() + k * width; }
    void push(const uint32_t* v)
    {
        d.insert(d.end(), v, v + width);
        ++count;
    }
    void clear()
    {
// ... 15 lines not shown
    int sweep_strategy = 2;
    size_t ncheck_history = 3;
    bool strictly_nested = false;
    double tol_margin_global_search = 10.0;
    bool has_seed = false;
    uint64_t seed = 0;
    size_t max_bond_dim_or_max() const
    {
        return max_bond_dim == 0 ? std::numeric_limits<size_t>::max() : max_bond_dim;
    }
    void validate() const;
};

struct FromTensorTrainOptions {
    double tolerance = 1e-12;
    size_t max_bond_dim = 0;
    size_t max_iter = 3;
};

class Tci2 {
    pool::IdleScope idle_scope_;
public:
    explicit Tci2(const std::vector<size_t>& local_dims);
    ~Tci2();

    void set_builtin(int fid, int n_acc, const double* params, const uint64_t* weights);
    void set_callback(t4a_gpu_batch_eval_fn cb, void* ctx);

    size_t len() const { return n_; }
    size_t rank() const;
    std::vector<size_t> link_dims() const;
    double max_bond_error() const;
    void add_global_pivots(const std::vector<std::vector<uint32_t>>& pivots);
    void crossinterpolate2(std::vector<std::vector<uint32_t>> initial_pivots, const TCI2Options& options);
    void optimize(const TCI2Options& options, bool final_sweep1site);
    static void optimize_group(const std::vector<Tci2*>& handles, const TCI2Options& options, bool final_sweep1site);
    static void fill_site_tensors_group(const std::vector<Tci2*>& handles);
    struct OptRun {
        TCI2Options options;
        bool final_sweep1site = false;
        std::vector<size_t> nglobal_hist;
        StdRng rng;
        bool pending_fill = false;
        size_t iter = 0;
        bool done = false;
        double norm = 1.0, abs_tol = 0.0;
        bool is_forward = true, chained = false, fill_ahead = false;
        long ext_idx = -1;
        bool allow_small = true;
        bool small_complete = false;
    };
    bool small_enabled = true;
    std::array<uint64_t, 4> small_stats{{0, 0, 0, 0}};
    uint64_t small_last_clocks_[12] = {0, 0, 0, 0, 0, 0, 0, 0, 0, 0, 0, 0};
    int small_tile_max = 16;
    bool small_stamps = false;
    int small_last_reason_ = 0;
    bool small_engine_eligible(const TCI2Options& options) const;
    bool small_engine_run(OptRun& r);
    void opt_begin(OptRun& r);
    void opt_iter_issue_pending_fill(OptRun& r);
    void opt_end_issue_fill(OptRun& r);
    bool opt_iter_start(OptRun& r, bool defer_launch = false);
    void opt_iter_finish(OptRun& r);
    void opt_end(OptRun& r);
    void sweep2site(bool forward, const TCI2Options& options);
    void sweep1site(bool forward, double rel_tol, double abs_tol, size_t max_bond_dim, bool update_tensors);
    void fill_site_tensors();
    void fill_site_tensors_impl(bool async);
    void fill_wait();
    void export_site_tensors_async(double* d_dst, size_t stride, hipStream_t consumer);
    void export_site_shard_async(double* d_dst, size_t stride, hipStream_t consumer);
    void import_site_shard_async(const double* d_src, size_t stride, size_t per_rank, hipStream_t producer);
    void make_canonical(double rel_tol, double abs_tol, size_t max_bond_dim);
    void invalidate_site_tensors();
    void flush_pivot_errors() { pivot_errors.clear(); }
    void mark_sets_changed()
    {
        chain_.tables_valid = false;
        chain_.digits_stale = false;
    }
    std::array<uint64_t, 5> chain_stats{{0, 0, 0, 0, 0}};
    std::array<uint64_t, 4> chain_stats_ext{{0, 0, 0, 0}};
    const uint64_t* fill_stats() const { return fill_stats_; }
    const RookWork& rook_work() const { return rook_work_; }
    bool chain_enabled = true;
    bool chain_verify = false;
    bool chain_event_timing = false;

    std::vector<double> evaluate(const uint32_t* idx, size_t n_pts);
    double sum();
    std::vector<double> site_tensor_host(size_t site, size_t dims3[3]);

    void assign_from_tensor_train(const TensorTrain& tt, const FromTensorTrainOptions& options);

    size_t n_;
    std::vector<size_t> local_dims;
    std::vector<IndexSet> i_set, j_set;
    struct HistEntry {
        std::vector<IndexSet> is, js;
        bool digits_valid = true;
        std::vector<uint64_t> code;
        size_t cap = 0;
        uint64_t serial = 0;
    };
    std::vector<HistEntry> history;
    void clear_history()
    {
        history.clear();
        chain_.hist_serial += 16;
    }
    void sync_digits();
    std::vector<double> bond_errors, pivot_errors;
    double max_sample_value = 0.0;
    std::vector<DevCore> cores;
    std::vector<size_t> ranks_hist;
    std::vector<double> errors_hist;
    int termination = T4A_GPU_TCI2_MAX_ITERATIONS;
    std::vector<std::array<size_t, 3>> last_sweep_shapes;
    size_t shard_rank = 0, shard_world = 1;
    PiShard pi_shard;
    bool keep_site_tensors = false;
    size_t callback_threads = 1;
    Engine eng;

private:
    enum class FnKind { None, Builtin, Callback };
    FnKind fn_kind_ = FnKind::None;
    FnDevice fn_dev_{};
    std::vector<uint64_t> weights_;
    std::vector<size_t> offset_;
    size_t total_ = 0;
    t4a_gpu_batch_eval_fn cb_ = nullptr;
    void* cb_ctx_ = nullptr;

    IndexSet kronecker_i(size_t p) const;
    IndexSet kronecker_j(size_t p) const;
    static void union_extras(IndexSet& base, const IndexSet& extras);
    void accumulate(const IndexSet& set, size_t first_site, std::vector<uint64_t>& acc) const;

    void eval_matrix(const IndexSet& a, size_t a0, const IndexSet& b, size_t b0, double* d_out,
                     unsigned long long* d_maxbits, const std::vector<uint64_t>* acc_a = nullptr,
                     const std::vector<uint64_t>* acc_b = nullptr);
    void stage_accumulators(const IndexSet& a, size_t a0, const IndexSet& b, size_t b0, const std::vector<uint64_t>* acc_a,
                            const std::vector<uint64_t>* acc_b, const uint64_t** d_ra, const uint64_t** d_rb, bool in_place = false);
    std::vector<double> eval_points_host(const std::vector<uint32_t>& idx, size_t n_pts);
    void require_fn() const;

    struct BondOut {
        LuciResult lu;
    };
    struct SidePrep {
        bool valid = false;
        size_t bond = 0;
        bool cols = false;
        IndexSet set;
        std::vector<uint64_t> acc;
    };
    SidePrep prep_;
    struct Prefetch {
        bool wanted = false;
        size_t bond = 0;
        bool cols = false;
        const IndexSet* extra = nullptr;
        long fill_site = -1;
    } prefetch_;
    struct FillAcc {
        bool valid = false;
        std::vector<uint64_t> accJ, accK, accI;
    };
// ... 135 lines not shown
```

tensor4all-rs_amd/csrc/tci2_chain.hip:

```cpp
#include "tci2.hpp"

#include <algorithm>
#include <atomic>
#include <chrono>
#include <cmath>
#include <cstdlib>

namespace t4a {

namespace {
size_t round_up_sz(size_t v, size_t m) { return (v + m - 1) / m * m; }
std::atomic<int> g_chains_inflight{0};
}
thread_local double g_chain_wait_seconds = 0.0;

bool Tci2::chain_usable(const TCI2Options& options) const
{
    static const bool off = std::getenv("T4A_NO_CHAIN") != nullptr;
    if (off || !chain_enabled || fn_kind_ != FnKind::Builtin || options.pivot_search != 0) return false;
    long double space = 1.0L;
    for (size_t d : local_dims) space *= (long double)d;
    if (space >= 9.0e18L) return false;
    for (size_t p = 0; p < n_; ++p) {
        if (i_set[p].count == 0 || j_set[p].count == 0) return false;
// ... 199 lines not shown
        cI[p] = i_set[p].count;
        cJ[p] = j_set[p].count;
        if (ext) {
            eI[p] = ext->is[p].count;
            eJ[p] = ext->js[p].count;
        }
        use_extras |= eI[p] != 0 || eJ[p] != 0;
        need_cap = std::max({need_cap, cI[p], cJ[p], eI[p], eJ[p]});
    }
    std::vector<size_t> order(nb);
    for (size_t k = 0; k < nb; ++k) order[k] = forward ? k : nb - 1 - k;
    std::vector<size_t> dep_ub(nb), ind_ub(nb), lda_ub(nb, 0);
    std::vector<RrluRoute> plans(nb);
    size_t Mcap = 1, Ncap = 1, steps_cap = 1, pi_cap = 0, spec_cap = 0, dep_cap = 1, ind_cap = 1;
    for (size_t k = 0; k < nb; ++k) {
        const size_t b = order[k];
        const size_t Mub = one ? (forward ? cI[b] * local_dims[b] : cI[b + 1]) : cI[b] * local_dims[b] + eI[b + 1];
        const size_t Nub = one ? (forward ? cJ[b] : cJ[b + 1] * local_dims[b + 1]) : cJ[b + 1] * local_dims[b + 1] + eJ[b];
        const size_t rub = std::max<size_t>(std::min({Mub, Nub, chi}), 1);
        cI[b + 1] = rub;
        cJ[b] = rub;
        need_cap = std::max(need_cap, rub);
        dep_ub[b] = forward ? Mub : Nub;
        ind_ub[b] = forward ? Nub : Mub;
        if (dep_ub[b] > 65535 || ind_ub[b] > 65535 || !(plans[b] = eng.chain_route((int)dep_ub[b], (int)ind_ub[b])).ok()) {
            ++(one ? chain_stats_ext[2] : chain_stats[3]);
            return false;
        }
        Mcap = std::max(Mcap, Mub);
        Ncap = std::max(Ncap, Nub);
        dep_cap = std::max(dep_cap, dep_ub[b]);
        ind_cap = std::max(ind_cap, ind_ub[b]);
        steps_cap = std::max(steps_cap, rub);
        const bool fused = plans[b].fused;
        if (!launch) pi_cap = std::max(pi_cap, dep_ub[b] * ind_ub[b]);
        if (!fused) {
            pi_cap = std::max(pi_cap, dep_ub[b] * ind_ub[b]);
            if (k > 0 && plans[order[k - 1]].on_xcd()) {
                const size_t site = forward ? b : b + 1;
                lda_ub[b] = dep_ub[order[k - 1]] * local_dims[site] + (forward ? eI[b + 1] : eJ[b]);
                spec_cap = std::max(spec_cap, lda_ub[b] * ind_ub[b]);
            }
        }
    }
    if (need_cap > (size_t)CHAIN_MAX_SET) {
        ++(one ? chain_stats_ext[2] : chain_stats[3]);
        return false;
    }

    size_t cap_side = 0;
    {
        size_t dmax = 1;
        for (size_t d : local_dims) dmax = std::max(dmax, d);
        if (chi <= (size_t)CHAIN_MAX_SET && chi * dmax + chi <= 2048) {
            need_cap = std::max(need_cap, chi);
            const size_t side = chi * dmax + chi;
            dep_cap = std::max(dep_cap, side);
            ind_cap = std::max(ind_cap, side);
            Mcap = std::max(Mcap, side);
            Ncap = std::max(Ncap, side);
            steps_cap = std::max(steps_cap, chi);
            spec_cap = std::max(spec_cap, (side * dmax + chi) * side);
            pi_cap = std::max(pi_cap, side * side);
            cap_side = side;
        }
    }
    chain_layout(round_up_sz(need_cap, 64));
    const size_t cap = chain_.cap;
    if (!chain_.weights_valid) {
        chain_.weights.reserve(weights_.size());
        chain_.siteinfo.reserve(2 * n_);
        std::vector<int> si(2 * n_);
        for (size_t p = 0; p < n_; ++p) {
            si[p] = (int)local_dims[p];
            si[n_ + p] = (int)offset_[p];
        }
        T4A_HIP(hipMemcpyAsync(chain_.weights.get(), weights_.data(), weights_.size() * sizeof(uint64_t), hipMemcpyHostToDevice, st));
        T4A_HIP(hipMemcpyAsync(chain_.siteinfo.get(), si.data(), si.size() * sizeof(int), hipMemcpyHostToDevice, st));
        T4A_HIP(hipStreamSynchronize(st));
        chain_.weights_valid = true;
    }
    chain_.ind.reserve(nb * ind_cap * (1 + K));
    chain_.ind_cnt.reserve(nb);
    chain_.dep.reserve(dep_cap * (1 + K));
    chain_.rowmap.reserve(dep_cap);
    chain_.pi.reserve(std::max<size_t>(pi_cap, 64 * 64));
    chain_.factors_stride = 0;
    if (one && chain_.one_factors) {
        size_t stride = 1;
        for (size_t b = 0; b < nb; ++b) stride = std::max(stride, dep_ub[b] * ind_ub[b]);
        if (nb * stride > ((size_t)1 << 27)) {
            ++chain_stats_ext[2];
            return false;
        }
        chain_.factors_stride = stride;
        chain_.factors.reserve(nb * stride);
        chain_.urows.reserve(std::max<size_t>(steps_cap, 1) * std::max(dep_cap, ind_cap));
    }
    if (spec_cap) {
        chain_.spec[0].reserve(spec_cap);
        chain_.spec[1].reserve(spec_cap);
    }
    const RrluBlock proto = RrluBlock::layout(steps_cap, Mcap, Ncap, true);
    chain_.blocks.reserve(nb * proto.bytes);
    chain_.hblocks.reserve(nb * proto.bytes);
    chain_.dims.reserve(nb * 5 + 2);
    chain_.hdims.reserve(nb * 4);
    const bool timed = eng.prof.enabled;
    const bool timed_events = timed && chain_event_timing;
    while (timed_events && chain_.t0.size() < nb) {
        hipEvent_t a = nullptr, b2 = nullptr;
        T4A_HIP(hipEventCreate(&a));
        T4A_HIP(hipEventCreate(&b2));
        chain_.t0.push_back(a);
        chain_.t1.push_back(b2);
    }

    if (!chain_.tables_valid) chain_upload_current();
    int ext_slot = 0;
    if (use_extras) {
        const uint64_t want = ext->serial;
        if (chain_.snap_serial[0] == want)
            ext_slot = 0;
        else if (chain_.snap_serial[1] == want)
            ext_slot = 1;
        else {
            ext_slot = (in_optimize && chain_.snap_serial[0] == chain_.hist_serial) ? 1 : 0;
            chain_upload_hist(*ext, ext_slot);
            chain_.snap_serial[ext_slot] = want;
        }
    }
    int snap = -1;
    if (in_optimize) {
        snap = use_extras ? 1 - ext_slot : 0;
        chain_.snap_serial[snap] = chain_.hist_serial;
    }

    for (size_t b = 0; b < nb; ++b) {
        std::memset(chain_.hblocks.get() + b * proto.bytes, 0, 32);
        std::memset(chain_.hdims.get() + b * 4, 0xFF, 4 * sizeof(int));
    }
    ChainCommon c;
    std::memset(&c, 0, sizeof(c));
    c.I = chain_tab(0);
    c.J = chain_tab(1);
    c.HI = chain_tab(2 + 2 * ext_slot);
    c.HJ = chain_tab(3 + 2 * ext_slot);
    c.mI = chain_mirror(1 - chain_.mcur, 0);
    c.mJ = chain_mirror(1 - chain_.mcur, 1);
    c.cap = (int)cap;
    c.K = (int)K;
    c.w = chain_.weights.get();
    c.total = (int)total_;
    c.ldim = chain_.siteinfo.get();
    c.woff = chain_.siteinfo.get() + n_;
    c.forward = forward ? 1 : 0;
    c.use_extras = use_extras ? 1 : 0;
    c.one_site = one ? 1 : 0;
    c.ind_code = chain_.ind.get();
    c.ind_acc = chain_.ind.get() + nb * ind_cap;
    c.ind_cnt = chain_.ind_cnt.get();
    c.ind_cap = (int)ind_cap;
    c.dep_code = chain_.dep.get();
    c.dep_acc = chain_.dep.get() + dep_cap;
    c.dep_cap = (int)dep_cap;
    c.rowmap = chain_.rowmap.get();
    c.dims = chain_.dims.get();
    c.hdims = chain_.hdims.get();
    c.n_sites = (int)n_;
    if (snap >= 0) {
        c.snap_dst = chain_tab(2 + 2 * snap).code;
        c.snap_cnt_dst = chain_tab(2 + 2 * snap).cnt;
        c.snap_words = 2 * n_ * cap * (1 + K);
    }
    c.zero_a = reinterpret_cast<uint64_t*>(chain_.blocks.get());
    c.zero_a_words = nb * proto.bytes / 8;
    c.zero_b = reinterpret_cast<uint64_t*>(chain_.dims.get());
    c.zero_b_words = (nb * 5 * sizeof(int) + 7) / 8;

    chain_.common = c;
    chain_.prepared = true;
    chain_.forward = forward;
    chain_.in_optimize = in_optimize;
    chain_.ext_idx = ext_idx;
    chain_.chi = chi;
    chain_.tol = options.tolerance;
    chain_.order = std::move(order);
    chain_.plans = std::move(plans);
    chain_.dep_ub = std::move(dep_ub);
    chain_.ind_ub = std::move(ind_ub);
    chain_.use_extras = use_extras;
    chain_.ind_cap = ind_cap;
    chain_.cap_side = cap_side;
    chain_.proto = proto;
    chain_.timed = timed;
    chain_.timed_events = timed_events;
    chain_.tokens.assign(nb, 0u);
    if (launch) chain_launch();
    return true;
}

void Tci2::chain_launch()
{
    if (!chain_.prepared) throw Error(T4A_GPU_INTERNAL_ERROR, "bond chain: nothing prepared to launch");
    chain_.prepared = false;
    const size_t nb = n_ - 1;
    const size_t K = (size_t)chain_.n_acc, cap = chain_.cap;
    const bool forward = chain_.forward, use_extras = chain_.use_extras, timed_events = chain_.timed_events;
    const size_t chi = chain_.chi, ind_cap = chain_.ind_cap, cap_side = chain_.cap_side;
    const ChainCommon& c = chain_.common;
    const RrluBlock& proto = chain_.proto;
    const std::vector<size_t>& order = chain_.order;
    const std::vector<RrluRoute>& plans = chain_.plans;
    const std::vector<size_t>& dep_ub = chain_.dep_ub;
    const std::vector<size_t>& ind_ub = chain_.ind_ub;
    std::vector<unsigned>& tokens = chain_.tokens;
    hipStream_t st = eng.stream();
    auto block_of = [&](size_t b) {
        RrluBlock k = proto;
        k.dev = chain_.blocks.get() + b * proto.bytes;
        return k;
    };
    {
        size_t reserve_words = 0;
        const RrluRoute cr = cap_side ? eng.chain_route((int)cap_side, (int)cap_side) : RrluRoute();
        if (cr.on_xcd()) reserve_words = cr.xcd_mailbox_words();
        eng.chain_begin(plans, reserve_words);
    }
    bool counted = false;
    try {
        chain_indep_launch(c, (int)nb, st);
        unsigned* tile_counters = reinterpret_cast<unsigned*>(chain_.dims.get() + nb * 4);
        const bool solo = g_chains_inflight.fetch_add(1) == 0;
        counted = true;
        static const bool no_walk = std::getenv("T4A_NO_WALK") != nullptr;
        size_t walk_cols = 0;
        bool walk = !no_walk && !timed_events && nb <= 128;
        for (size_t b = 0; walk && b < nb; ++b) {
            walk = dep_ub[b] <= 64 && ind_ub[b] <= 32;
            walk_cols = std::max(walk_cols, ind_ub[b]);
        }
        if (walk) {
            ChainWalkArgs w;
            std::memset(&w, 0, sizeof(w));
            w.blocks = chain_.blocks.get();
            w.block_bytes = proto.bytes;
            w.off_piv = proto.off_piv;
            w.off_rp = proto.off_rp;
            w.off_cp = proto.off_cp;
            w.off_ts = proto.off_ts;
            w.pi = chain_.pi.get();
            w.n_bonds = (int)nb;
            w.max_steps = (int)std::min<size_t>(chi, 64);
            w.rel_tol = chain_.tol;
            w.abs_tol = chain_.one_site ? chain_.abs_tol : 0.0;
            w.factors = chain_.factors_stride ? chain_.factors.get() : nullptr;
            w.factors_stride = chain_.factors_stride;
            if (chain_.walk_token > 0xFFFF0000u || chain_.walk_token == 0u) chain_.walk_token = 1u;
            w.token_base = chain_.walk_token;
            chain_.walk_token += (unsigned)nb;
            w.timed = chain_.timed ? 1 : 0;
            w.lean_prep = 1;
            static const bool walk_dbg = std::getenv("T4A_WALK_DEBUG") != nullptr;
            if (walk_dbg) {
                chain_.walk_dbg.reserve(8);
                T4A_HIP(hipMemsetAsync(chain_.walk_dbg.get(), 0, 8 * sizeof(unsigned long long), st));
                w.phase_ticks = chain_.walk_dbg.get();
            }
            chain_.walked = true;
            for (size_t k = 0; k < nb; ++k) tokens[order[k]] = w.token_base + (unsigned)k;
            chain_walk_launch(c, fn_dev_, w, (int)walk_cols, st);
            ++chain_stats_ext[0];
        }
        static const bool want_prep_dbg = std::getenv("T4A_PREP_DEBUG") != nullptr;
        unsigned long long* prep_dbg = nullptr;
        if (want_prep_dbg && !walk) {
            chain_.walk_dbg.reserve(8);
            T4A_HIP(hipMemsetAsync(chain_.walk_dbg.get(), 0, 8 * sizeof(unsigned long long), st));
            prep_dbg = chain_.walk_dbg.get();
            chain_.prep_dbg = true;
        }
        bool spec_pending = false;
        for (size_t k = 0; !walk && k < nb; ++k) {
            const size_t b = order[k];
            const RrluRoute& pl = plans[b];
            const bool fused = pl.fused;
            const bool spec_here = spec_pending && !fused;
            const RrluBlock blk = block_of(b);
            ChainPrepArgs pa;
            std::memset(&pa, 0, sizeof(pa));
            pa.b = (int)b;
            pa.do_build = 1;
            pa.dbg = prep_dbg;
            pa.defer_host_writes = 0;
            pa.with_rowmap = spec_here ? 1 : 0;
            pa.prev_b = -1;
            if (k > 0) {
                const size_t pb = order[k - 1];
                const RrluBlock pblk = block_of(pb);
                pa.prev_b = (int)pb;
                pa.prev_iresult = pblk.iresult();
                pa.prev_rowperm = pblk.row_perm();
                pa.prev_colperm = pblk.col_perm();
                pa.prev_token = tokens[pb];
            }
            chain_prep_launch(c, pa, st);
            if (!fused && !spec_here) chain_pi_launch(c, fn_dev_, (int)b, (int)dep_ub[b], (int)ind_ub[b], chain_.pi.get(), st);
            XcdSpecArgs sp;
            std::memset(&sp, 0, sizeof(sp));
            spec_pending = false;
            if (solo && k + 1 < nb && pl.on_xcd()) {
                const size_t nx = order[k + 1];
                if (!plans[nx].fused) {
                    const size_t site = forward ? nx : nx + 1;
                    const ChainTab& H = forward ? c.HI : c.HJ;
                    const size_t hsite = forward ? nx + 1 : nx;
                    sp.out = chain_.spec[(k + 1) & 1].get();
                    sp.dep_acc = c.dep_acc;
                    sp.w_site = c.w + offset_[site];
                    sp.ext_acc = H.acc + hsite * cap * K;
                    sp.ext_cnt = use_extras ? H.cnt + hsite : nullptr;
                    sp.ind_acc = c.ind_acc + nx * ind_cap * K;
                    sp.ind_cnt = c.ind_cnt + nx;
                    sp.tile_counter = tile_counters + nx;
                    sp.total = (int)total_;
                    sp.d = (int)local_dims[site];
                    sp.fn = fn_dev_;
                    spec_pending = true;
                }
            }
            FusedPi fp;
            fp.fn = fn_dev_;
            fp.d_rowacc = c.dep_acc;
            fp.d_colacc = c.ind_acc + b * ind_cap * K;
            fp.host_resident = false;
            const double* A = fused ? nullptr : (spec_here ? chain_.spec[k & 1].get() : chain_.pi.get());
            if (timed_events) T4A_HIP(hipEventRecord(chain_.t0[b], st));
            tokens[b] = eng.chain_rrlu(pl, forward, A, spec_here ? c.rowmap : nullptr, fused ? &fp : nullptr, c.dims + b * 4, chi, chain_.tol,
                                       chain_.one_site ? chain_.abs_tol : 0.0, blk, spec_pending ? &sp : nullptr,
                                       chain_.factors_stride ? chain_.factors.get() + b * chain_.factors_stride : nullptr, chain_.urows.get());
            if (timed_events) T4A_HIP(hipEventRecord(chain_.t1[b], st));
        }
        if (!walk) {
            const size_t pb = order[nb - 1];
            const RrluBlock pblk = block_of(pb);
            ChainPrepArgs pa;
            std::memset(&pa, 0, sizeof(pa));
            pa.do_build = 0;
            pa.defer_host_writes = 0;
            pa.prev_b = (int)pb;
            pa.prev_iresult = pblk.iresult();
            pa.prev_rowperm = pblk.row_perm();
            pa.prev_colperm = pblk.col_perm();
            pa.prev_token = tokens[pb];
            chain_prep_launch(c, pa, st);
        }
        chain_.cores_batched = false;
        if (chain_.one_site && chain_.factors_stride && forward && nb <= (size_t)LUCI_LEFT_CORES_MAX_JOBS) {
            LeftCoreJobs jobs;
            std::memset(&jobs, 0, sizeof(jobs));
            size_t max_rows = 1;
            for (size_t b = 0; b < nb; ++b) {
                const RrluBlock blk = block_of(b);
                const size_t rub = std::max<size_t>(std::min({dep_ub[b], ind_ub[b], chi}), 1);
                DevCore& core = cores[b];
                core.buf.reserve(std::max<size_t>(dep_ub[b] * rub, 1));
                LeftCoreJob& j = jobs.j[b];
                j.lu = chain_.factors.get() + b * chain_.factors_stride;
                j.dims = c.dims + b * 4;
                j.iresult = blk.iresult();
                j.row_perm = blk.row_perm();
                j.core = core.buf.get();
                j.S = (int)local_dims[b];
                j.token = tokens[b];
                max_rows = std::max(max_rows, dep_ub[b]);
            }
            luci_left_cores_batched_launch(jobs, (int)nb, (int)max_rows, st);
            chain_.cores_batched = true;
        }
        chain_.last_core_launched = false;
        if (chain_.one_site && chain_.factors_stride && forward) {
            const size_t last = n_ - 1;
            const size_t a_ub = std::max<size_t>(std::min({dep_ub[nb - 1], ind_ub[nb - 1], chi}), 1);
            const size_t entries = a_ub * local_dims[last] * std::max<size_t>(j_set[last].count, 1);
            if (entries <= ((size_t)1 << 24)) {
                cores[last].buf.reserve(entries);
                chain_last_core_launch(c, fn_dev_, cores[last].buf.get(), (int)entries, st);
                chain_.last_core_launched = true;
            }
        }
        T4A_HIP(hipMemcpyAsync(chain_.hblocks.get(), chain_.blocks.get(), nb * proto.bytes, hipMemcpyDeviceToHost, st));
        T4A_HIP(hipGetLastError());
    } catch (...) {
        (void)hipStreamSynchronize(st);
        eng.chain_end();
        if (counted) g_chains_inflight.fetch_sub(1);
        chain_.tables_valid = false;
        chain_.snap_serial[0] = chain_.snap_serial[1] = ~0ull;
        throw;
    }
    chain_.inflight = true;
    chain_.wait_stream = st;
    chain_.group_role = 0;
}

void Tci2::chain_group_launch(const std::vector<Tci2*>& hs)
{
    const size_t nh = hs.size();
    if (nh == 0) return;
    bool ok = nh >= 2 && nh <= (size_t)CHAIN_GROUP_MAX;
    Tci2* lead = hs[0];
    for (Tci2* h : hs) {
        if (!h->chain_.prepared) throw Error(T4A_GPU_INTERNAL_ERROR, "bond chain: a handle of the group has nothing prepared");
        ok = ok && h->n_ == lead->n_ && h->chain_.forward == lead->chain_.forward && h->chain_.chi == lead->chain_.chi &&
             h->chain_.tol == lead->chain_.tol && !h->chain_.timed_events;
    }
    const size_t nb = lead->n_ - 1;
    const bool forward = lead->chain_.forward;
    std::vector<RrluRoute> gplans(nb);
    size_t side_ub = 0;
    if (ok) {
        for (size_t b = 0; b < nb && ok; ++b) {
            size_t dm = 1, im = 1;
            for (Tci2* h : hs) {
                dm = std::max(dm, h->chain_.dep_ub[b]);
                im = std::max(im, h->chain_.ind_ub[b]);
            }
            gplans[b] = Engine::chain_group_route((int)dm, (int)im);
            ok = gplans[b].ok();
        }
        for (Tci2* h : hs) side_ub = std::max(side_ub, h->chain_.cap_side);
    }
    if (!ok) {
        for (Tci2* h : hs) h->chain_launch();
        return;
    }
    hipStream_t st = lead->eng.stream();
    size_t reserve_words = 0;
// ... 68 lines not shown
            ChainPrepGroupArgs pg;
            std::memset(&pg, 0, sizeof(pg));
            for (size_t i = 0; i < nh; ++i) prev_of(hs[i], order[nb - 1], pg.a[i]);
            chain_prep_group_launch(d_slots, pg, (int)nh, st);
        }
        for (Tci2* h : hs)
            T4A_HIP(hipMemcpyAsync(h->chain_.hblocks.get(), h->chain_.blocks.get(), nb * h->chain_.proto.bytes, hipMemcpyDeviceToHost, st));
        T4A_HIP(hipGetLastError());
    } catch (...) {
        (void)hipStreamSynchronize(st);
        if (locked) lead->eng.chain_end();
        for (size_t i = 0; i < nh; ++i) {
            if (counted[i]) g_chains_inflight.fetch_sub(1);
            hs[i]->chain_.prepared = false;
            hs[i]->chain_.tables_valid = false;
            hs[i]->chain_.snap_serial[0] = hs[i]->chain_.snap_serial[1] = ~0ull;
        }
        throw;
    }
    for (Tci2* h : hs) {
        h->chain_.plans = gplans;
        h->chain_.inflight = true;
        h->chain_.wait_stream = st;
        h->chain_.group_role = h == lead ? 1 : 2;
    }
}

void Tci2::chain_abort() noexcept
{
    if (chain_.prepared) {
        chain_.snap_serial[0] = chain_.snap_serial[1] = ~0ull;
        chain_.tables_valid = false;
    }
    chain_.prepared = false;
    chain_.walked = false;
    if (!chain_.inflight) return;
    chain_.inflight = false;
    hipStream_t st = chain_.wait_stream ? chain_.wait_stream : eng.stream();
    (void)hipStreamSynchronize(st);
    (void)hipGetLastError();
    if (chain_.group_role != 2) eng.chain_end();
    chain_.group_role = 0;
    chain_.wait_stream = nullptr;
    g_chains_inflight.fetch_sub(1);
    chain_.tables_valid = false;
    chain_.snap_serial[0] = chain_.snap_serial[1] = ~0ull;
}

void Tci2::chain_finish(const TCI2Options& options)
{
    if (!chain_.inflight) return;
    chain_.inflight = false;
    hipStream_t st = chain_.wait_stream ? chain_.wait_stream : eng.stream();
    const size_t nb = n_ - 1;
    const size_t K = (size_t)chain_.n_acc, cap = chain_.cap;
    const bool forward = chain_.forward;
    const RrluBlock& proto = chain_.proto;
    const auto wait_t0 = std::chrono::steady_clock::now();
    const hipError_t sync_err = hipStreamSynchronize(st);
    g_chain_wait_seconds += std::chrono::duration<double>(std::chrono::steady_clock::now() - wait_t0).count();
    if (chain_.group_role != 2) eng.chain_end();
    const bool was_group = chain_.group_role != 0;
    chain_.group_role = 0;
    chain_.wait_stream = nullptr;
    g_chains_inflight.fetch_sub(1);
    if (sync_err != hipSuccess) {
        chain_.tables_valid = false;
        T4A_HIP(sync_err);
    }
    if (chain_.walked && chain_.walk_dbg.get() && std::getenv("T4A_WALK_DEBUG")) {
        unsigned long long t[8] = {0, 0, 0, 0, 0, 0, 0, 0};
        (void)hipMemcpy(t, chain_.walk_dbg.get(), sizeof(t), hipMemcpyDeviceToHost);
        std::fprintf(stderr, "[t4a walk] %zu bonds: preparation %.1f us (gather %.1f, dependent list %.1f), candidate matrix %.1f us, rrLU %.1f us, kernel %.1f us\n", nb,
                     t[0] * 0.01, t[4] * 0.01, t[5] * 0.01, t[1] * 0.01, t[2] * 0.01, t[3] * 0.01);
    }
    chain_.walked = false;
    if (chain_.prep_dbg && chain_.walk_dbg.get()) {
        unsigned long long t[8] = {0, 0, 0, 0, 0, 0, 0, 0};
        (void)hipMemcpy(t, chain_.walk_dbg.get(), sizeof(t), hipMemcpyDeviceToHost);
        std::fprintf(stderr, "[t4a prep] %zu bonds: preparation kernels %.1f us in total: gather %.1f, dependent list %.1f, rest %.1f\n", nb, t[6] * 0.01, t[4] * 0.01,
                     t[5] * 0.01, (double)(t[6] - t[4] - t[5]) * 0.01);
    }
    chain_.prep_dbg = false;
    const int mnew = 1 - chain_.mcur;
    const ChainTab ni = chain_mirror(mnew, 0), nj = chain_mirror(mnew, 1);
    long failed_k = -1;
    bool failed_timeout = false;
    for (size_t k = 0; k < nb; ++k) {
        const size_t b = chain_.order[k];
        const int* hd = chain_.hdims.get() + b * 4;
        const char* hb = chain_.hblocks.get() + b * proto.bytes;
        const int* hi = reinterpret_cast<const int*>(hb + 16);
        if (hd[2] != 0 || hd[0] <= 0 || hd[1] <= 0) {
            failed_k = k > 0 ? (long)k - 1 : 0;
            break;
        }
        if (hi[1] != 0 || hi[3] != (int)chain_.tokens[b]) {
            failed_k = (long)k;
            failed_timeout = hi[1] != 2;
            break;
        }
        if (hi[2] != 0) {
            failed_k = (long)k;
            break;
        }
    }
    if (failed_k >= 0) {
        static const bool dbg = std::getenv("T4A_CHAIN_DEBUG") != nullptr;
        if (dbg) {
            const size_t b = chain_.order[(size_t)failed_k];
            const int* hd = chain_.hdims.get() + b * 4;
            const int* hi = reinterpret_cast<const int*>(chain_.hblocks.get() + b * proto.bytes + 16);
            const RrluRoute& pl = chain_.plans[b];
            std::fprintf(stderr, "[t4a chain] bond %zu (k = %ld of %zu, %s) did not complete: dims %d x %d poisoned %d lda %d | npiv %d flag %d nan %d token %d (want %u) | plan kind %d %d x %d wg %d RPT %d CPT %d W %d\n",
                         b, failed_k, nb, forward ? "forward" : "backward", hd[0], hd[1], hd[2], hd[3], hi[0], hi[1], hi[2], hi[3], chain_.tokens[b], (int)pl.kind, pl.kM, pl.kN,
                         pl.xcd.wg, pl.xcd.RPT, pl.xcd.CPT, pl.xcd.W);
        }
    }
    const size_t done = failed_k < 0 ? nb : (size_t)failed_k;
    for (size_t k = 0; k < done; ++k) {
        const size_t b = chain_.order[k];
        const int* hd = chain_.hdims.get() + b * 4;
        const char* hb = chain_.hblocks.get() + b * proto.bytes;
        const int* hi = reinterpret_cast<const int*>(hb + 16);
        const size_t M = (size_t)hd[0], N = (size_t)hd[1];
        const int rank = hi[0];
        double last_error, abs_max;
        std::memcpy(&last_error, hb, sizeof(double));
        std::memcpy(&abs_max, hb + 8, sizeof(double));
        const size_t cnt = (size_t)(rank > 0 ? rank : 1);
        if ((size_t)ni.cnt[b + 1] != cnt || (size_t)nj.cnt[b] != cnt)
            throw Error(T4A_GPU_INTERNAL_ERROR, "bond chain: gathered pivot count of bond " + std::to_string(b) + " disagrees with its rank");
        i_set[b + 1].count = cnt;
        j_set[b].count = cnt;
        i_set[b + 1].d.clear();
        j_set[b].d.clear();
        {
            float ms = 0.f;
            if (chain_.timed) {
                unsigned long long ts[2];
                std::memcpy(ts, hb + proto.off_ts, sizeof(ts));
                ms = ts[1] > ts[0] ? (float)((double)(ts[1] - ts[0]) * 1e-5) : 0.f;
                if (chain_.timed_events) T4A_HIP(hipEventElapsedTime(&ms, chain_.t0[b], chain_.t1[b]));
                eng.prof.v[0] += ms;
                eng.prof.v[1] += 1.0;
            }
            eng.rrlu_account(chain_.plans[b], !forward, (int)M, (int)N, rank, chain_.timed, ms, chain_.chi > 0 && (size_t)rank == chain_.chi);
            eng.prof.v[11] += (double)M * (double)N;
        }
        if (abs_max > max_sample_value) max_sample_value = abs_max;
        bond_errors[b] = last_error;
        if (chain_.one_site) {
            std::vector<double> pe((size_t)rank + 1);
            const double* pv = reinterpret_cast<const double*>(hb + proto.off_piv);
            for (int q = 0; q < rank; ++q) pe[(size_t)q] = std::sqrt(pv[q] * pv[q]);
            pe[(size_t)rank] = last_error;
            update_pivot_errors(pe);
        } else {
            last_sweep_shapes[b] = {M, N, (size_t)rank};
        }
    }
    if (done > 0) {
        const ChainTab oi = chain_mirror(chain_.mcur, 0), oj = chain_mirror(chain_.mcur, 1);
        std::vector<char> wi(n_, 0), wj(n_, 0);
        for (size_t k = 0; k < done; ++k) {
            wi[chain_.order[k] + 1] = 1;
// ... 129 lines not shown
```

tensor4all-rs_amd/python/t4a_amd/__init__.py:

```python
import ctypes
import os

import numpy as np

from .functions import (FnSpec, quantics_trig_exp, quantics_osc2d, lorentz, linear_sum,
                        FN_MAX_PARAMS)

_HERE = os.path.dirname(os.path.abspath(__file__))
LIB_PATH = os.environ.get("T4A_GPU_LIB") or os.path.normpath(os.path.join(_HERE, "..", "..", "lib", "libt4a_gpu.so"))

if not os.path.exists(LIB_PATH):
    raise ImportError(f"{LIB_PATH} not found: build it with `python tensor4all-rs_amd/build.py` "
                      "(the MI355X backend has no CPU fallback)")

_lib = ctypes.CDLL(LIB_PATH)

c_size_t = ctypes.c_size_t
c_double = ctypes.c_double
c_int32 = ctypes.c_int32
c_void_p = ctypes.c_void_p

SUCCESS = 0
NULL_POINTER = -1
INVALID_ARGUMENT = -2
# ... 633 lines not shown
        _check(_lib.t4a_gpu_tci2_import_site_shard_async(self._h, c_void_p(device_ptr), c_size_t(stride), c_size_t(per_rank),
                                                         c_void_p(producer_stream)))

    def set_keep_site_tensors(self, keep=True):
        _check(_lib.t4a_gpu_tci2_set_keep_site_tensors(self._h, c_int32(1 if keep else 0)))

    def set_site_shard(self, rank, world):
        _check(_lib.t4a_gpu_tci2_set_site_shard(self._h, c_size_t(rank), c_size_t(world)))
        self._site_shard = (int(rank), int(world))

    def site_shard(self):
        return getattr(self, "_site_shard", (0, 1))

    def history(self):
        n = c_size_t(0)
        _check(_lib.t4a_gpu_tci2_n_iterations(self._h, ctypes.byref(n)))
        ranks = np.zeros(max(n.value, 1), dtype=np.uintp)
        errors = np.zeros(max(n.value, 1), dtype=np.float64)
        _check(_lib.t4a_gpu_tci2_history(self._h, _p(ranks), _p(errors)))
        return [int(r) for r in ranks[: n.value]], errors[: n.value].copy()

    def termination(self):
        v = c_int32(0)
        _check(_lib.t4a_gpu_tci2_termination(self._h, ctypes.byref(v)))
        return v.value

    def evaluate(self, idx):
        idx = np.ascontiguousarray(np.asarray(idx, dtype=np.uintp).reshape(-1, len(self.local_dims)))
        out = np.zeros(idx.shape[0], dtype=np.float64)
        _check(_lib.t4a_gpu_tci2_evaluate(self._h, _p(idx), c_size_t(idx.shape[0]), _p(out)))
        return out

    def sum(self):
        v = c_double(0)
        _check(_lib.t4a_gpu_tci2_sum(self._h, ctypes.byref(v)))
        return v.value

    def to_tensor_train(self):
        h = c_void_p()
        _check(_lib.t4a_gpu_tci2_to_tensor_train(self._h, ctypes.byref(h)))
        return SimpleTensorTrain._adopt(h)

    @classmethod
    def from_tensor_train(cls, tt, tolerance=1e-12, max_bond_dim=None, max_iter=3):
        h = c_void_p()
        _check(_lib.t4a_gpu_tci2_from_tensor_train(tt._h, c_double(tolerance),
                                                   c_size_t(0 if max_bond_dim is None else max_bond_dim),
                                                   c_size_t(max_iter), ctypes.byref(h)))
        self = cls.__new__(cls)
        self.local_dims = [int(d) for d in tt.site_dims()]
        self._h = h
        self._cb_keepalive = None
        self.n_callback_calls = 0
        return self

    def last_sweep_shapes(self):
        out = np.zeros(3 * (len(self.local_dims) - 1), dtype=np.uintp)
        _check(_lib.t4a_gpu_tci2_last_sweep_shapes(self._h, _p(out)))
        return out.reshape(-1, 3).astype(np.int64)

    def profile_enable(self, on=True):
        _check(_lib.t4a_gpu_tci2_profile_enable(self._h, c_int32(1 if on else 0)))

    def profile_reset(self):
        _check(_lib.t4a_gpu_tci2_profile_reset(self._h))

    def profile(self):
        out = np.zeros(16, dtype=np.float64)
        _check(_lib.t4a_gpu_tci2_profile_get(self._h, _p(out)))
        keys = ["rrlu_ms", "rrlu_launches", "pi_ms", "pi_launches", "fill_ms", "fill_calls", "factor_ms",
                "factor_calls", "pivot_steps", "rrlu_bytes", "flops", "evals"]
        d = {k: float(out[i]) for i, k in enumerate(keys)}
        d.update(dom_ms=float(out[12]), dom_launches=float(out[13]), dom_bytes=float(out[14]), dom_code=int(out[15]))
        return d

    def profile_variants(self):
        n = c_size_t(0)
        _check(_lib.t4a_gpu_tci2_profile_variants(self._h, None, c_size_t(0), ctypes.byref(n)))
        out = np.zeros((max(n.value, 1), 5), dtype=np.float64)
        _check(_lib.t4a_gpu_tci2_profile_variants(self._h, _p(out), c_size_t(out.shape[0]), ctypes.byref(n)))
        return [dict(code=int(r[0]), ms=float(r[1]), launches=float(r[2]), bytes=float(r[3]), steps=float(r[4])) for r in out[: n.value]]


    def set_chain(self, enable=True, verify=False, event_timing=False, small_engine=True, small_stamps=False, fill_graph_relaxed=False, small_tile32=False):
        _check(_lib.t4a_gpu_tci2_set_chain(self._h, c_int32(1 if enable else 0),
                                           c_int32((1 if verify else 0) | (2 if event_timing else 0) | (0 if small_engine else 4) | (8 if small_stamps else 0)
                                                   | (16 if fill_graph_relaxed else 0) | (32 if small_tile32 else 0))))

    def set_callback_threads(self, n):
        _check(_lib.t4a_gpu_tci2_set_callback_threads(self._h, c_size_t(n)))

    def small_stats(self):
        out = (ctypes.c_uint64 * 16)()
        _check(_lib.t4a_gpu_tci2_small_stats(self._h, out))
        return {"completed": int(out[0]), "iterations": int(out[1]), "handed_back": int(out[2]), "not_eligible": int(out[3]),
                "device_us": (out[4] / 100.0, out[5] / 100.0, out[6] / 100.0), "reason": int(out[7]),
                "phase_cycles": dict(zip(("lists", "evaluation", "pivot_steps", "gather", "factors", "fill", "snapshots", "rest"), (int(out[8 + k]) for k in range(8))))}

    def rook_stats(self):
        out = (ctypes.c_uint64 * 4)()
        _check(_lib.t4a_gpu_tci2_rook_stats(self._h, out))
        return {"device_searches": int(out[0]), "device_visits": int(out[1]), "host_searches": int(out[2]), "host_syncs": int(out[3])}

    def fill_stats(self):
        out = (ctypes.c_uint64 * 3)()
        _check(_lib.t4a_gpu_tci2_fill_stats(self._h, out))
        return {"fills": int(out[0]), "graph_replays": int(out[1]), "graph_captures": int(out[2])}

    def chain_stats(self):
        out = np.zeros(5, dtype=np.uint64)
        _check(_lib.t4a_gpu_tci2_chain_stats(self._h, _p(out)))
        ext = np.zeros(4, dtype=np.uint64)
        _check(_lib.t4a_gpu_tci2_chain_stats_ext(self._h, _p(ext)))
        return dict(half_sweeps=int(out[0]), bonds=int(out[1]), fell_back=int(out[2]), not_eligible=int(out[3]),
                    group_half_sweeps=int(out[4]), walked_sweeps=int(ext[0]), one_site_sweeps=int(ext[1]),
                    one_site_not_eligible=int(ext[2]), one_site_fell_back=int(ext[3]))


def optimize_group(tcis, options, final_sweep1site=True):
    o = options.to_c()
    arr = (c_void_p * len(tcis))(*[t._h for t in tcis])
    _check(_lib.t4a_gpu_tci2_optimize_group(arr, c_size_t(len(tcis)), ctypes.byref(o), c_int32(1 if final_sweep1site else 0)))


def fill_site_tensors_group(tcis):
    arr = (c_void_p * len(tcis))(*[t._h for t in tcis])
    _check(_lib.t4a_gpu_tci2_fill_site_tensors_group(arr, c_size_t(len(tcis))))


def crossinterpolate2(f, local_dims, initial_pivots, options):
    options.to_c()
    tci = TensorCI2(local_dims)
    tci.set_function(f)
    tci.crossinterpolate2(initial_pivots, options)
    return tci


def svd_backend(a):
    a = _f(a)
    m, n = a.shape
    k = min(m, n)
    u = np.zeros((m, k), order="F")
    s = np.zeros(k)
    vt = np.zeros((k, n), order="F")
    _check(_lib.t4a_gpu_svd_f64(_p(a), c_size_t(m), c_size_t(n), _p(u), _p(s), _p(vt)))
    return u, s, vt


def randomized_svd(a, rank, oversample=8, power_iters=1, seed=0):
    a = _f(a)
    m, n = a.shape
    u = np.zeros((m, rank), order="F")
    s = np.zeros(rank)
    vt = np.zeros((rank, n), order="F")
    _check(_lib.t4a_gpu_rsvd_f64(_p(a), c_size_t(m), c_size_t(n), c_size_t(rank), c_size_t(oversample), c_size_t(power_iters),
                                 ctypes.c_uint64(seed), _p(u), _p(s), _p(vt)))
    return u, s, vt


def qr_backend(a):
    a = _f(a)
    m, n = a.shape
    k = min(m, n)
    q = np.zeros((m, k), order="F")
    r = np.zeros((k, n), order="F")
    _check(_lib.t4a_gpu_qr_f64(_p(a), c_size_t(m), c_size_t(n), _p(q), _p(r)))
    return q, r


def full_piv_lu_matrix(a):
    a = _f(a)
    n = a.shape[0]
    if a.shape[1] != n:
        raise T4aError(INVALID_ARGUMENT, "full_piv_lu expects a square matrix")
    out = [np.zeros((n, n), order="F") for _ in range(4)]
    _check(_lib.t4a_gpu_full_piv_lu_f64(_p(a), c_size_t(n), *[_p(x) for x in out]))
    return tuple(out)


COMPRESS_LU, COMPRESS_CI, COMPRESS_SVD = 0, 1, 2


class SimpleTensorTrain:

    def __init__(self, cores):
        cores = [np.asarray(c, dtype=np.float64) for c in cores]
        for c in cores:
            if c.ndim != 3:
                raise T4aError(INVALID_ARGUMENT, "site tensors must have three legs (left, site, right)")
        dims = np.array([c.shape for c in cores], dtype=np.uintp).reshape(-1)
        flat = np.ascontiguousarray(np.concatenate([c.reshape(-1, order="F") for c in cores])
                                    if cores else np.zeros(1))
        self._h = c_void_p()
        _check(_lib.t4a_gpu_tt_new(_p(dims) if len(cores) else None, c_size_t(len(cores)), _p(flat),
                                   ctypes.byref(self._h)))

    @classmethod
    def _adopt(cls, handle):
        self = cls.__new__(cls)
# ... 1149 lines not shown
```

Before: 304.9.

## Fuse next bond's chain prep into single-XCD rrLU kernel as a sidecar

Result: no change. 306.2, median of 3 (+0.4%).

```diff
diff --git a/include/t4a_gpu.h b/include/t4a_gpu.h
--- a/include/t4a_gpu.h
+++ b/include/t4a_gpu.h
@@ -478,6 +478,7 @@
 
 t4a_gpu_status t4a_gpu_tci2_chain_stats(const t4a_gpu_tci2* h, uint64_t* out );
 t4a_gpu_status t4a_gpu_tci2_chain_stats_ext(const t4a_gpu_tci2* h, uint64_t* out );
+t4a_gpu_status t4a_gpu_tci2_chain_side_stats(const t4a_gpu_tci2* h, uint64_t* out );
 t4a_gpu_status t4a_gpu_tci2_fill_stats(const t4a_gpu_tci2* h, uint64_t* out );
 t4a_gpu_status t4a_gpu_tci2_rook_stats(const t4a_gpu_tci2* h, uint64_t* out );
 t4a_gpu_status t4a_gpu_tci2_optimize_group(t4a_gpu_tci2* const* handles, size_t n_handles, const t4a_gpu_tci2_options* options,
diff --git a/tensor4all-rs_amd/build.py b/tensor4all-rs_amd/build.py
--- a/tensor4all-rs_amd/build.py
+++ b/tensor4all-rs_amd/build.py
@@ -13,7 +13,7 @@
 FLAGS = ["--offload-arch=gfx950", "-O3", "-std=c++17", "-fPIC", "-ffp-contract=off", "-Wall", "-Wno-unused-function",
          "-fvisibility=hidden"] + os.environ.get("T4A_EXTRA_FLAGS", "").split()
 FILE_FLAGS = {"kernels_dense.hip": ["-mllvm", "-amdgpu-mfma-vgpr-form=1"], "kernels_linalg.hip": ["-ffp-contract=fast"]}
-HEADERS = ["common.hpp", "stdrng.hpp", "pishard.hpp", "kernels.hpp", "kernels_rrlu_xcd_common.hpp", "kernels_rrlu_w1_body.hpp", "engine.hpp", "tci2.hpp", "tt.hpp", "mpo.hpp", "globalsearch.hpp", "rook.hpp", "patching.hpp", "tree.hpp", "quantics.hpp", "tensorops.hpp", "aci.hpp", "quanticstransform.hpp", "../../include/t4a_gpu.h",
+HEADERS = ["common.hpp", "stdrng.hpp", "pishard.hpp", "kernels.hpp", "kernels_rrlu_xcd_common.hpp", "kernels_chain_side.hpp", "kernels_rrlu_w1_body.hpp", "engine.hpp", "tci2.hpp", "tt.hpp", "mpo.hpp", "globalsearch.hpp", "rook.hpp", "patching.hpp", "tree.hpp", "quantics.hpp", "tensorops.hpp", "aci.hpp", "quanticstransform.hpp", "../../include/t4a_gpu.h",
            "../../include/t4a_testfunctions.h"]
 
 
diff --git a/tensor4all-rs_amd/csrc/capi.hip b/tensor4all-rs_amd/csrc/capi.hip
--- a/tensor4all-rs_amd/csrc/capi.hip
+++ b/tensor4all-rs_amd/csrc/capi.hip
@@ -1190,6 +1190,15 @@
     });
 }
 
+t4a_gpu_status t4a_gpu_tci2_chain_side_stats(const t4a_gpu_tci2* h, uint64_t* out)
+{
+    return guarded([&] {
+        T4A_REQUIRE_PTR(h);
+        T4A_REQUIRE_PTR(out);
+        for (int k = 0; k < 3; ++k) out[k] = h->impl.chain_side_stats[k];
+    });
+}
+
 t4a_gpu_status t4a_gpu_tci2_rook_stats(const t4a_gpu_tci2* h, uint64_t* out)
 {
     return guarded([&] {
@@ -1223,6 +1232,7 @@
         h->impl.small_stamps = (verify & 8) != 0;
         h->impl.fill_graph_relaxed = (verify & 16) != 0;
         h->impl.small_tile_max = (verify & 32) ? 32 : 16;
+        h->impl.chain_sidecar = (verify & 64) == 0;
     });
 }
 
diff --git a/tensor4all-rs_amd/csrc/engine.hip b/tensor4all-rs_amd/csrc/engine.hip
--- a/tensor4all-rs_amd/csrc/engine.hip
+++ b/tensor4all-rs_amd/csrc/engine.hip
@@ -143,13 +143,19 @@
     default: return RrluLock::None;
     }
 }
-size_t RrluRoute::xcd_mailbox_words() const { return (rrlu_xcd_keys_bytes(xcd) + rrlu_xcd_cols_bytes(xcd, kM)) / sizeof(unsigned long long); }
-void RrluRoute::launch(const RrluXcdArgs& args, hipStream_t stream) const
-{
+size_t RrluRoute::xcd_pivlog_offset() const { return rrlu_xcd_keys_bytes(xcd) + rrlu_xcd_cols_bytes(xcd, kM) + 256; }
+size_t RrluRoute::xcd_mailbox_words() const
+{
+    const size_t log = kind == RrluKind::SingleXcd ? 256 + ((size_t)std::min(kM, kN) + 1) * 16 : 0;
+    return (rrlu_xcd_keys_bytes(xcd) + rrlu_xcd_cols_bytes(xcd, kM) + log) / sizeof(unsigned long long);
+}
+void RrluRoute::launch(const RrluXcdArgs& args, hipStream_t stream, const ChainSideArgs* side) const
+{
+    if (side && kind != RrluKind::SingleXcd) throw Error(T4A_GPU_INTERNAL_ERROR, "rrLU: only the single-XCD launch carries a sidecar");
     switch (kind) {
     case RrluKind::OneWave: rrlu_w1_launch(xcd, args, stream); break;
     case RrluKind::OneWorkgroup: rrlu_wg_launch(xcd, args, stream); break;
-    case RrluKind::SingleXcd: rrlu_xcd2_launch(xcd, args, stream); break;
+    case RrluKind::SingleXcd: rrlu_xcd2_launch(xcd, args, stream, side); break;
     case RrluKind::MultiXcd: rrlu_xcd2m_launch(xcd, args, stream); break;
     default: throw Error(T4A_GPU_INTERNAL_ERROR, "rrLU: the route has no single-XCD launch");
     }
@@ -817,7 +823,8 @@
 }
 
 unsigned Engine::chain_rrlu(const RrluRoute& rt, bool left, const double* d_a, const int* d_rowmap, const FusedPi* fused, const int* d_dims,
-                            size_t max_bond_dim, double rel_tol, double abs_tol, const RrluBlock& blk, const XcdSpecArgs* spec, double* d_aout, double* d_urows)
+                            size_t max_bond_dim, double rel_tol, double abs_tol, const RrluBlock& blk, const XcdSpecArgs* spec, double* d_aout, double* d_urows,
+                            const ChainSideArgs* side)
 {
     unsigned token = 0u;
     if (rt.on_xcd()) {
@@ -827,7 +834,8 @@
         a.Aout = d_aout;
         a.urows = d_aout ? d_urows : nullptr;
         if (spec) a.spec = *spec;
-        rt.launch(a, stream_);
+        a.pivlog = side ? reinterpret_cast<unsigned*>(reinterpret_cast<char*>(a.keys) + rt.xcd_pivlog_offset()) : nullptr;
+        rt.launch(a, stream_, side);
     } else {
         if (++done_token_ == 0u) ++done_token_;
         RrluRegArgs a;
diff --git a/tensor4all-rs_amd/csrc/engine.hpp b/tensor4all-rs_amd/csrc/engine.hpp
--- a/tensor4all-rs_amd/csrc/engine.hpp
+++ b/tensor4all-rs_amd/csrc/engine.hpp
@@ -86,7 +86,8 @@
     int code(bool tie_row_major, bool saturated = false) const;
     RrluLock lock() const;
     size_t xcd_mailbox_words() const;
-    void launch(const RrluXcdArgs& args, hipStream_t stream) const;
+    size_t xcd_pivlog_offset() const;
+    void launch(const RrluXcdArgs& args, hipStream_t stream, const ChainSideArgs* side = nullptr) const;
     void launch_group(const RrluXcdGroupArgs& args, bool tie_row_major, hipStream_t stream) const;
 };
 
@@ -146,7 +147,8 @@
     RrluRoute chain_route(int kM, int kN) const;
     void chain_begin(const std::vector<RrluRoute>& routes, size_t reserve_mailbox_words = 0);
     unsigned chain_rrlu(const RrluRoute& rt, bool left, const double* d_a, const int* d_rowmap, const FusedPi* fused, const int* d_dims,
-                        size_t max_bond_dim, double rel_tol, double abs_tol, const RrluBlock& blk, const XcdSpecArgs* spec, double* d_aout = nullptr, double* d_urows = nullptr);
+                        size_t max_bond_dim, double rel_tol, double abs_tol, const RrluBlock& blk, const XcdSpecArgs* spec, double* d_aout = nullptr, double* d_urows = nullptr,
+                        const ChainSideArgs* side = nullptr);
     void chain_end();
     static RrluRoute chain_group_route(int kM, int kN);
     void chain_group_reserve(const std::vector<RrluRoute>& routes, size_t reserve_mailbox_words, hipStream_t order_stream);
diff --git a/tensor4all-rs_amd/csrc/kernels.hpp b/tensor4all-rs_amd/csrc/kernels.hpp
--- a/tensor4all-rs_amd/csrc/kernels.hpp
+++ b/tensor4all-rs_amd/csrc/kernels.hpp
@@ -180,6 +180,7 @@
     const int* rowmap;
     XcdSpecArgs spec;
     int ts_u64;
+    unsigned* pivlog;
 };
 bool rrlu_xcd_make_plan(int M, int N, RrluXcdPlan* out, bool any_size = false, int max_w = 32, bool allow_big = false);
 size_t rrlu_xcd_keys_bytes(const RrluXcdPlan& plan);
@@ -187,7 +188,9 @@
 struct RrluXcdGroupArgs {
     RrluXcdArgs p[8];
 };
-void rrlu_xcd2_launch(const RrluXcdPlan& plan, const RrluXcdArgs& args, hipStream_t stream);
+struct ChainSideArgs;
+constexpr bool rrlu_xcd2_has_sidecar(int RPT, int CPT) { return !(RPT == 16 && CPT == 4); }
+void rrlu_xcd2_launch(const RrluXcdPlan& plan, const RrluXcdArgs& args, hipStream_t stream, const ChainSideArgs* side = nullptr);
 void rrlu_xcd2m_launch(const RrluXcdPlan& plan, const RrluXcdArgs& args, hipStream_t stream);
 void rrlu_xcd2_group_launch(const RrluXcdPlan& plan, const RrluXcdGroupArgs& args, bool tie_row_major, hipStream_t stream);
 bool rrlu_wg_make_plan(int M, int N, RrluXcdPlan* out, int spec_blocks = 0);
@@ -266,6 +269,13 @@
     unsigned prev_token;
     unsigned long long* dbg;
     int defer_host_writes;
+};
+struct ChainSideArgs {
+    ChainCommon c;
+    const uint64_t* prev_dep_code;
+    const uint64_t* prev_dep_acc;
+    int b, prev_b;
+    unsigned* elect;
 };
 struct ChainWalkArgs {
     char* blocks;
diff --git a/tensor4all-rs_amd/csrc/kernels_chain.hip b/tensor4all-rs_amd/csrc/kernels_chain.hip
--- a/tensor4all-rs_amd/csrc/kernels_chain.hip
+++ b/tensor4all-rs_amd/csrc/kernels_chain.hip
@@ -1,5 +1,6 @@
 #include "kernels.hpp"
 #include "kernels_rrlu_w1_body.hpp"
+#include "kernels_chain_side.hpp"
 
 namespace t4a {
 
@@ -16,99 +17,6 @@
 
 constexpr int CHAIN_T = 1024;
 constexpr int WALK_T = 1024;
-constexpr int CHAIN_HASH = 4096;
-
-__device__ __forceinline__ unsigned chain_hash(unsigned long long c)
-{
-    c ^= c >> 33;
-    c *= 0xff51afd7ed558ccdull;
-    c ^= c >> 29;
-    return (unsigned)c & (CHAIN_HASH - 1);
-}
-
-__device__ __forceinline__ int block_scan_flag(bool flag, int* wave_sums, int* total)
-{
-    const int lane = threadIdx.x & 63, wave = threadIdx.x >> 6;
-    const unsigned long long bal = __ballot(flag);
-    const int before = __builtin_popcountll(bal & ((1ull << lane) - 1ull));
-    __syncthreads();
-    if (lane == 0) wave_sums[wave] = __builtin_popcountll(bal);
-    __syncthreads();
-    int base = 0, tot = 0;
-    for (int w = 0; w < (int)blockDim.x / 64; ++w) {
-        const int v = wave_sums[w];
-        if (w < wave) base += v;
-        tot += v;
-    }
-    *total = tot;
-    return base + before;
-}
-
-template <bool PARENT_OUTER>
-__device__ int build_side(const uint64_t* __restrict__ pcode, const uint64_t* __restrict__ pacc, int np, int d,
-                          const uint64_t* __restrict__ w, int K, int total_w, int w_off, const uint64_t* __restrict__ ecode,
-                          const uint64_t* __restrict__ eacc, int ne, uint64_t* __restrict__ ocode, uint64_t* __restrict__ oacc, int ocap,
-                          const int* srcpos, int n_prev, int* __restrict__ rowmap, unsigned long long* hkeys, int* wave_sums)
-{
-    const int tid = threadIdx.x;
-    const int m0 = np * d;
-    if (m0 > ocap) return -1;
-    if (ne > 0) {
-        for (int e = tid; e < CHAIN_HASH; e += (int)blockDim.x) hkeys[e] = 0ull;
-        __syncthreads();
-    }
-    for (int idx = tid; idx < m0; idx += (int)blockDim.x) {
-        const int i = PARENT_OUTER ? idx / d : idx % np;
-        const int s = PARENT_OUTER ? idx % d : idx / np;
-        const uint64_t c = pcode[i];
-        ocode[idx] = (uint64_t)s + (uint64_t)d * c;
-        for (int k = 0; k < K; ++k) oacc[(size_t)idx * K + k] = pacc[(size_t)i * K + k] + w[(size_t)k * total_w + w_off + s];
-        if (rowmap) rowmap[idx] = srcpos[i] * d + s;
-    }
-    if (ne <= 0) return m0;
-    for (int i = tid; i < np; i += (int)blockDim.x) {
-        const unsigned long long key = (unsigned long long)pcode[i] + 1ull;
-        unsigned h = chain_hash(key);
-        for (;;) {
-            const unsigned long long old = atomicCAS(&hkeys[h], 0ull, key);
-            if (old == 0ull || old == key) break;
-            h = (h + 1) & (CHAIN_HASH - 1);
-        }
-    }
-    __syncthreads();
-    int count = m0;
-    for (int base = 0; base < ne; base += (int)blockDim.x) {
-        const int e = base + tid;
-        bool keep = false;
-        uint64_t c = 0ull;
-        if (e < ne) {
-            c = ecode[e];
-            const unsigned long long key = (unsigned long long)(c / (uint64_t)d) + 1ull;
-            unsigned h = chain_hash(key);
-            keep = true;
-            for (;;) {
-                const unsigned long long v = hkeys[h];
-                if (v == 0ull) break;
-                if (v == key) {
-                    keep = false;
-                    break;
-                }
-                h = (h + 1) & (CHAIN_HASH - 1);
-            }
-        }
-        int tot = 0;
-        const int pos = block_scan_flag(keep, wave_sums, &tot);
-        if (count + tot > ocap) return -1;
-        if (keep) {
-            const int o = count + pos;
-            ocode[o] = c;
-            for (int k = 0; k < K; ++k) oacc[(size_t)o * K + k] = eacc[(size_t)e * K + k];
-            if (rowmap) rowmap[o] = n_prev * d + e;
-        }
-        count += tot;
-    }
-    return count;
-}
 
 __device__ __forceinline__ void chain_indep_body(const ChainCommon& c)
 {
diff --git a/tensor4all-rs_amd/csrc/kernels_chain_side.hpp b/tensor4all-rs_amd/csrc/kernels_chain_side.hpp
--- /dev/null
+++ b/tensor4all-rs_amd/csrc/kernels_chain_side.hpp
@@ -0,0 +1,278 @@
+#pragma once
+#include "kernels.hpp"
+#include "kernels_rrlu_xcd_common.hpp"
+
+namespace t4a {
+
+namespace {
+
+constexpr int CHAIN_HASH = 4096;
+
+__device__ __forceinline__ unsigned chain_hash(unsigned long long c)
+{
+    c ^= c >> 33;
+    c *= 0xff51afd7ed558ccdull;
+    c ^= c >> 29;
+    return (unsigned)c & (CHAIN_HASH - 1);
+}
+
+__device__ __forceinline__ int block_scan_flag(bool flag, int* wave_sums, int* total)
+{
+    const int lane = threadIdx.x & 63, wave = threadIdx.x >> 6;
+    const unsigned long long bal = __ballot(flag);
+    const int before = __builtin_popcountll(bal & ((1ull << lane) - 1ull));
+    __syncthreads();
+    if (lane == 0) wave_sums[wave] = __builtin_popcountll(bal);
+    __syncthreads();
+    int base = 0, tot = 0;
+    for (int w = 0; w < (int)blockDim.x / 64; ++w) {
+        const int v = wave_sums[w];
+        if (w < wave) base += v;
+        tot += v;
+    }
+    *total = tot;
+    return base + before;
+}
+
+template <bool PARENT_OUTER>
+__device__ int build_side(const uint64_t* __restrict__ pcode, const uint64_t* __restrict__ pacc, int np, int d,
+                          const uint64_t* __restrict__ w, int K, int total_w, int w_off, const uint64_t* __restrict__ ecode,
+                          const uint64_t* __restrict__ eacc, int ne, uint64_t* __restrict__ ocode, uint64_t* __restrict__ oacc, int ocap,
+                          const int* srcpos, int n_prev, int* __restrict__ rowmap, unsigned long long* hkeys, int* wave_sums)
+{
+    const int tid = threadIdx.x;
+    const int m0 = np * d;
+    if (m0 > ocap) return -1;
+    if (ne > 0) {
+        for (int e = tid; e < CHAIN_HASH; e += (int)blockDim.x) hkeys[e] = 0ull;
+        __syncthreads();
+    }
+    for (int idx = tid; idx < m0; idx += (int)blockDim.x) {
+        const int i = PARENT_OUTER ? idx / d : idx % np;
+        const int s = PARENT_OUTER ? idx % d : idx / np;
+        const uint64_t c = pcode[i];
+        ocode[idx] = (uint64_t)s + (uint64_t)d * c;
+        for (int k = 0; k < K; ++k) oacc[(size_t)idx * K + k] = pacc[(size_t)i * K + k] + w[(size_t)k * total_w + w_off + s];
+        if (rowmap) rowmap[idx] = srcpos[i] * d + s;
+    }
+    if (ne <= 0) return m0;
+    for (int i = tid; i < np; i += (int)blockDim.x) {
+        const unsigned long long key = (unsigned long long)pcode[i] + 1ull;
+        unsigned h = chain_hash(key);
+        for (;;) {
+            const unsigned long long old = atomicCAS(&hkeys[h], 0ull, key);
+            if (old == 0ull || old == key) break;
+            h = (h + 1) & (CHAIN_HASH - 1);
+        }
+    }
+    __syncthreads();
+    int count = m0;
+    for (int base = 0; base < ne; base += (int)blockDim.x) {
+        const int e = base + tid;
+        bool keep = false;
+        uint64_t c = 0ull;
+        if (e < ne) {
+            c = ecode[e];
+            const unsigned long long key = (unsigned long long)(c / (uint64_t)d) + 1ull;
+            unsigned h = chain_hash(key);
+            keep = true;
+            for (;;) {
+                const unsigned long long v = hkeys[h];
+                if (v == 0ull) break;
+                if (v == key) {
+                    keep = false;
+                    break;
+                }
+                h = (h + 1) & (CHAIN_HASH - 1);
+            }
+        }
+        int tot = 0;
+        const int pos = block_scan_flag(keep, wave_sums, &tot);
+        if (count + tot > ocap) return -1;
+        if (keep) {
+            const int o = count + pos;
+            ocode[o] = c;
+            for (int k = 0; k < K; ++k) oacc[(size_t)o * K + k] = eacc[(size_t)e * K + k];
+            if (rowmap) rowmap[o] = n_prev * d + e;
+        }
+        count += tot;
+    }
+    return count;
+}
+
+constexpr unsigned PIVLOG_END = 0x40000000u;
+__device__ __forceinline__ void pivlog_store(__amdgpu_buffer_rsrc_t mail, int log_base, int slot, unsigned x, unsigned y, unsigned z, unsigned tag)
+{
+    u32x4 gv;
+    gv.x = x;
+    gv.y = y;
+    gv.z = z;
+    gv.w = tag ^ x ^ y ^ z;
+    __builtin_amdgcn_raw_buffer_store_b128(gv, mail, log_base + slot * 16, 0, BUF_SC1);
+}
+
+constexpr int SIDE_O_HASH = 0;
+constexpr int SIDE_O_SRCPOS = SIDE_O_HASH + CHAIN_HASH * 8;
+constexpr int SIDE_O_SUMS = SIDE_O_SRCPOS + CHAIN_MAX_SET * 4;
+constexpr int SIDE_O_CTL = SIDE_O_SUMS + 64;
+constexpr int CHAIN_SIDE_LDS_BYTES = SIDE_O_CTL + 64;
+constexpr unsigned SIDE_SPIN = 1u << 21;
+
+__device__ __forceinline__ void chain_sidecar_body(const ChainSideArgs* spp, const RrluXcdArgs* pk, char* lds)
+{
+    const ChainSideArgs& s = *spp;
+    const ChainCommon& c = s.c;
+    unsigned long long* const hkeys = reinterpret_cast<unsigned long long*>(lds + SIDE_O_HASH);
+    int* const s_srcpos = reinterpret_cast<int*>(lds + SIDE_O_SRCPOS);
+    int* const wave_sums = reinterpret_cast<int*>(lds + SIDE_O_SUMS);
+    int* const s_ctl = reinterpret_cast<int*>(lds + SIDE_O_CTL);
+    const int tid = threadIdx.x, lane = tid & 63;
+    const int wave = __builtin_amdgcn_readfirstlane(tid >> 6);
+    const int K = c.K;
+    const size_t cap = (size_t)c.cap;
+    const int pb = s.prev_b, b = s.b;
+    const int* pd = c.dims + (size_t)pb * 4;
+    const int pm = pd[0], pn = pd[1];
+    int n_prev_dep = 0;
+
+    if (wave == 0) {
+        bool poison = pd[2] != 0 || pm <= 0 || pn <= 0;
+        bool out_of_polls = false;
+        int cnt = 0;
+        if (!poison) {
+            const bool swap = pk->dims_swap != 0;
+            const unsigned salt = pk->salt;
+            const int nlog = pk->max_steps + 1;
+            const __amdgpu_buffer_rsrc_t rs = __builtin_amdgcn_make_buffer_rsrc((void*)pk->pivlog, 0, nlog * 16, 0x00020000);
+            const uint64_t* const pind_code = c.ind_code + (size_t)pb * c.ind_cap;
+            const uint64_t* const pind_acc = c.ind_acc + (size_t)pb * c.ind_cap * K;
+            const uint64_t* rcode = c.forward ? s.prev_dep_code : pind_code;
+            const uint64_t* racc = c.forward ? s.prev_dep_acc : pind_acc;
+            const uint64_t* ccode = c.forward ? pind_code : s.prev_dep_code;
+            const uint64_t* cacc = c.forward ? pind_acc : s.prev_dep_acc;
+            const size_t oi = (size_t)(pb + 1) * cap, oj = (size_t)pb * cap;
+            auto gather = [&](int k, int ri, int ci) {
+                const uint64_t rc = rcode[ri], cc = ccode[ci];
+                c.I.code[oi + k] = rc;
+                c.J.code[oj + k] = cc;
+                c.mI.code[oi + k] = rc;
+                c.mJ.code[oj + k] = cc;
+                for (int q = 0; q < K; ++q) {
+                    const uint64_t ra = racc[(size_t)ri * K + q], ca = cacc[(size_t)ci * K + q];
+                    c.I.acc[(oi + k) * K + q] = ra;
+                    c.J.acc[(oj + k) * K + q] = ca;
+                    c.mI.acc[(oi + k) * K + q] = ra;
+                    c.mJ.acc[(oj + k) * K + q] = ca;
+                }
+                s_srcpos[k] = c.forward ? ri : ci;
+            };
+            int base = 0, r = -1;
+            unsigned polls = 0;
+            while (r < 0 && !poison && !out_of_polls) {
+                const int kn = base + lane;
+                const u32x4 g = __builtin_amdgcn_raw_buffer_load_b128(rs, kn * 16, 0, BUF_SC1);
+                const unsigned tag = (salt << 16) | (unsigned)(kn + 1);
+                const bool is_end = g.z == (PIVLOG_END | (unsigned)kn);
+                const bool valid = kn < nlog && ((g.x ^ g.y ^ g.z ^ g.w) == tag) && (is_end || g.z == (unsigned)kn);
+                const unsigned long long vb = __ballot(valid);
+                const int nv = (~vb == 0ull) ? 64 : (int)__builtin_ctzll(~vb);
+                const unsigned long long eb = __ballot(valid && is_end) & (nv == 64 ? ~0ull : ((1ull << nv) - 1ull));
+                int nent = nv;
+                if (eb != 0ull) {
+                    const int el = (int)__builtin_ctzll(eb);
+                    nent = el;
+                    r = __builtin_amdgcn_readlane((int)g.x, el);
+                    if (__builtin_amdgcn_readlane((int)g.y, el) != 0 || r != base + el) poison = true;
+                }
+                if (lane < nent) {
+                    const int ri = (int)(swap ? g.y : g.x), ci = (int)(swap ? g.x : g.y);
+                    if (kn < c.cap && ri >= 0 && ri < pm && ci >= 0 && ci < pn) gather(kn, ri, ci);
+                }
+                {
+                    const int ri = (int)(swap ? g.y : g.x), ci = (int)(swap ? g.x : g.y);
+                    const bool oob = lane < nent && !(kn < c.cap && ri >= 0 && ri < pm && ci >= 0 && ci < pn);
+                    if (__ballot(oob) != 0ull) poison = true;
+                }
+                base += nent;
+                if (nent == 0 && r < 0) {
+                    if (++polls > SIDE_SPIN) out_of_polls = true;
+                    __builtin_amdgcn_s_sleep(8);
+                }
+                xcd_poll_again();
+            }
+            if (!poison && !out_of_polls) {
+                cnt = r > 0 ? r : 1;
+                if (cnt > c.cap || cnt > pm || cnt > pn) {
+                    poison = true;
+                } else {
+                    if (r == 0 && lane == 0) gather(0, 0, 0);
+                    if (lane == 0) {
+                        c.I.cnt[pb + 1] = cnt;
+                        c.J.cnt[pb] = cnt;
+                        c.mI.cnt[pb + 1] = cnt;
+                        c.mJ.cnt[pb] = cnt;
+                    }
+                }
+            }
+        }
+        if (lane == 0) {
+            s_ctl[0] = (poison || out_of_polls) ? 1 : 0;
+            s_ctl[1] = cnt;
+            s_ctl[2] = out_of_polls ? 1 : 0;
+        }
+    }
+    __threadfence_block();
+    __syncthreads();
+
+    int* dims = c.dims + (size_t)b * 4;
+    int* hdims = c.hdims ? c.hdims + (size_t)b * 4 : nullptr;
+    if (s_ctl[0]) {
+        if (tid == 0) {
+            dims[0] = dims[1] = dims[3] = 0;
+            dims[2] = 1;
+            if (hdims) {
+                hdims[0] = hdims[1] = 0;
+                hdims[2] = 1;
+                if (s_ctl[2]) hdims[3] = 1;
+            }
+        }
+        return;
+    }
+    n_prev_dep = c.forward ? pm : pn;
+    const int np = s_ctl[1];
+    int nd = -1, lda = 0;
+    const uint64_t* const xcode = c.forward ? c.HI.code + (size_t)(b + 1) * cap : c.HJ.code + (size_t)b * cap;
+    const uint64_t* const xacc = c.forward ? c.HI.acc + (size_t)(b + 1) * cap * K : c.HJ.acc + (size_t)b * cap * K;
+    if (c.forward) {
+        const int ne = c.use_extras ? c.HI.cnt[b + 1] : 0;
+        if (np >= 1 && np <= c.cap && ne <= c.cap)
+            nd = build_side<true>(c.I.code + (size_t)b * cap, c.I.acc + (size_t)b * cap * K, np, c.ldim[b], c.w, K, c.total, c.woff[b], xcode, xacc, ne,
+                                  c.dep_code, c.dep_acc, c.dep_cap, s_srcpos, n_prev_dep, c.rowmap, hkeys, wave_sums);
+        lda = n_prev_dep * c.ldim[b] + ne;
+    } else {
+        const int ne = c.use_extras ? c.HJ.cnt[b] : 0;
+        if (np >= 1 && np <= c.cap && ne <= c.cap)
+            nd = build_side<false>(c.J.code + (size_t)(b + 1) * cap, c.J.acc + (size_t)(b + 1) * cap * K, np, c.ldim[b + 1], c.w, K, c.total,
+                                   c.woff[b + 1], xcode, xacc, ne, c.dep_code, c.dep_acc, c.dep_cap, s_srcpos, n_prev_dep, c.rowmap, hkeys,
+                                   wave_sums);
+        lda = n_prev_dep * c.ldim[b + 1] + ne;
+    }
+    if (tid == 0) {
+        const int ni = c.ind_cnt[b];
+        const bool ok = nd > 0 && ni > 0;
+        const int M = c.forward ? nd : ni, N = c.forward ? ni : nd;
+        dims[0] = ok ? M : 0;
+        dims[1] = ok ? N : 0;
+        dims[2] = ok ? 0 : 1;
+        dims[3] = lda;
+        if (hdims) {
+            hdims[0] = ok ? M : 0;
+            hdims[1] = ok ? N : 0;
+            hdims[2] = ok ? 0 : 1;
+        }
+    }
+}
+
+}
+
+}
diff --git a/tensor4all-rs_amd/csrc/kernels_rrlu_xcd2.hip b/tensor4all-rs_amd/csrc/kernels_rrlu_xcd2.hip
--- a/tensor4all-rs_amd/csrc/kernels_rrlu_xcd2.hip
+++ b/tensor4all-rs_amd/csrc/kernels_rrlu_xcd2.hip
@@ -1,4 +1,8 @@
 #include "kernels_rrlu_xcd_common.hpp"
+#include "kernels_chain_side.hpp"
+
+#include <algorithm>
+#include <cstring>
 
 namespace t4a {
 
@@ -33,7 +37,16 @@
 
 constexpr int X2_DIVW = XWAVES - 1;
 
-template <int RPT, int CPT, bool ROWMAJOR, int KX = 1>
+struct Xcd2SoloArgs {
+    RrluXcdArgs p;
+    ChainSideArgs side;
+};
+template <bool SIDE> __device__ __forceinline__ unsigned xcd2_pivlog_bytes(const RrluXcdArgs& p)
+{
+    if constexpr (SIDE) return p.pivlog ? (unsigned)(p.max_steps + 1) * 16u : 0u;
+    else return 0u;
+}
+template <int RPT, int CPT, bool ROWMAJOR, int KX = 1, bool SIDE = false>
 __device__ __forceinline__ void rrlu_xcd2_body(const RrluXcdArgs& p, const RrluXcdArgs* pk)
 {
     static_assert(XWAVES == 8, "the second-generation kernel is written for eight waves per workgroup");
@@ -180,7 +193,7 @@
     const unsigned fin_base = cols_base + 2u * (unsigned)NW * (unsigned)(MP / 16) * 256u;
     const unsigned k3_base = fin_base + 256u;
     const __amdgpu_buffer_rsrc_t mail =
-        __builtin_amdgcn_make_buffer_rsrc((void*)p.keys, 0, (int)(k3_base + (KX > 1 ? 2u * (unsigned)NW * 16u : 0u)), 0x00020000);
+        __builtin_amdgcn_make_buffer_rsrc((void*)p.keys, 0, (int)(k3_base + (KX > 1 ? 2u * (unsigned)NW * 16u : 0u) + xcd2_pivlog_bytes<SIDE>(p)), 0x00020000);
 
     int npiv = 0;
     double max_error = 0.0;
@@ -689,6 +702,8 @@
                     colpos[ck_] = (unsigned short)pcp;
                     colpos[pc] = (unsigned short)kn;
                     lds_pivots[kn] = wval;
+                    if constexpr (SIDE)
+                        if (g == 0) pivlog_store(mail, (int)(4u * (unsigned)NW * 16u + 2u * (unsigned)NW * (unsigned)(MP / 16) * 256u + 256u), kn, (unsigned)irow_p, (unsigned)pc, (unsigned)kn, tag);
                 }
             }
         }
@@ -829,6 +844,11 @@
     if (rank == 0 && tid == 0) {
         pe.iresult[0] = npiv;
         pe.dresult[0] = error;
+        if constexpr (SIDE) {
+            const unsigned why = timed_out ? (unsigned)(ctl[1] ? ctl[1] : 1) : 0u;
+            pivlog_store(mail, (int)k3_base, npiv, (unsigned)npiv, why, PIVLOG_END | (unsigned)npiv, (pe.salt << 16) | (unsigned)(npiv + 1));
+            if (timed_out) pivlog_store(mail, (int)k3_base, npiv + 1, (unsigned)(npiv + 1), why, PIVLOG_END | (unsigned)(npiv + 1), (pe.salt << 16) | (unsigned)(npiv + 2));
+        }
     }
     if (stamp_on) {
         for (int e = 0; e < 16; ++e) pe.stamps[e] = lds_stamps[e];
@@ -940,27 +960,44 @@
 }
 #elif !defined(T4A_XCD_GROUP_TU)
 template <int RPT, int CPT, bool ROWMAJOR>
-__global__ void __launch_bounds__(XT) __attribute__((amdgpu_waves_per_eu(XWAVES / 4, XWAVES / 4))) rrlu_xcd2_kernel(RrluXcdArgs p)
-{
-    rrlu_xcd2_body<RPT, CPT, ROWMAJOR>(p, reinterpret_cast<const RrluXcdArgs*>(kernarg_base()));
-}
-template <int RPT, int CPT, bool ROWMAJOR> void xcd2_launch_tie(const RrluXcdPlan& plan, const RrluXcdArgs& a, hipStream_t stream)
+__global__ void __launch_bounds__(XT) __attribute__((amdgpu_waves_per_eu(XWAVES / 4, XWAVES / 4))) rrlu_xcd2_kernel(Xcd2SoloArgs ka)
+{
+    constexpr bool SIDE = rrlu_xcd2_has_sidecar(RPT, CPT);
+    if constexpr (SIDE)
+    if (ka.p.pivlog && (int)(xcc_id() & 7u) == ((ka.p.xcc + 1) & 7)) {
+        extern __shared__ __attribute__((aligned(16))) char side_smem[];
+        int* const flag = reinterpret_cast<int*>(side_smem);
+        if (threadIdx.x == 0) *flag = atomicAdd(ka.side.elect, 1u) == 0u ? 1 : 0;
+        __syncthreads();
+        const bool elected = __builtin_amdgcn_readfirstlane(*flag) != 0;
+        __syncthreads();
+        if (elected) {
+            const char* kb = kernarg_base();
+            chain_sidecar_body(reinterpret_cast<const ChainSideArgs*>(kb + offsetof(Xcd2SoloArgs, side)), reinterpret_cast<const RrluXcdArgs*>(kb), side_smem);
+            return;
+        }
+    }
+    rrlu_xcd2_body<RPT, CPT, ROWMAJOR, 1, SIDE>(ka.p, reinterpret_cast<const RrluXcdArgs*>(kernarg_base()));
+}
+template <int RPT, int CPT, bool ROWMAJOR> void xcd2_launch_tie(const RrluXcdPlan& plan, const Xcd2SoloArgs& a, hipStream_t stream)
 {
     static std::once_flag attr_once;
     std::call_once(attr_once, [] {
         (void)hipFuncSetAttribute(reinterpret_cast<const void*>(&rrlu_xcd2_kernel<RPT, CPT, ROWMAJOR>),
                                   hipFuncAttributeMaxDynamicSharedMemorySize, 160 * 1024);
     });
-    hipLaunchKernelGGL((rrlu_xcd2_kernel<RPT, CPT, ROWMAJOR>), dim3(plan.grid), dim3(XT), plan.lds_bytes, stream, a);
-}
-
-template <int RPT, int CPT> void xcd2_launch_rc(const RrluXcdPlan& plan, const RrluXcdArgs& a, hipStream_t stream)
-{
-    if (a.tie_row_major) xcd2_launch_tie<RPT, CPT, true>(plan, a, stream);
+    if (a.p.pivlog && !rrlu_xcd2_has_sidecar(RPT, CPT)) throw std::runtime_error("single-XCD rrLU: this plan carries no sidecar");
+    const size_t lds = a.p.pivlog ? std::max<size_t>(plan.lds_bytes, (size_t)CHAIN_SIDE_LDS_BYTES) : plan.lds_bytes;
+    hipLaunchKernelGGL((rrlu_xcd2_kernel<RPT, CPT, ROWMAJOR>), dim3(plan.grid), dim3(XT), lds, stream, a);
+}
+
+template <int RPT, int CPT> void xcd2_launch_rc(const RrluXcdPlan& plan, const Xcd2SoloArgs& a, hipStream_t stream)
+{
+    if (a.p.tie_row_major) xcd2_launch_tie<RPT, CPT, true>(plan, a, stream);
     else xcd2_launch_tie<RPT, CPT, false>(plan, a, stream);
 }
 
-template <int RPT> void xcd2_launch_r(const RrluXcdPlan& plan, const RrluXcdArgs& a, hipStream_t stream)
+template <int RPT> void xcd2_launch_r(const RrluXcdPlan& plan, const Xcd2SoloArgs& a, hipStream_t stream)
 {
     switch (plan.CPT) {
     case 1: xcd2_launch_rc<RPT, 1>(plan, a, stream); break;
@@ -1017,8 +1054,13 @@
     if (!ok) throw std::runtime_error("no kernel instantiation for this multi-XCD rrLU plan");
 }
 #elif !defined(T4A_XCD_GROUP_TU)
-void rrlu_xcd2_launch(const RrluXcdPlan& plan, const RrluXcdArgs& a, hipStream_t stream)
-{
+void rrlu_xcd2_launch(const RrluXcdPlan& plan, const RrluXcdArgs& args, hipStream_t stream, const ChainSideArgs* side)
+{
+    Xcd2SoloArgs a;
+    a.p = args;
+    if (side) a.side = *side;
+    else std::memset(&a.side, 0, sizeof(a.side));
+    if (!side) a.p.pivlog = nullptr;
     switch (plan.RPT) {
 #ifdef T4A_XCD_DEV
     case 2: xcd2_launch_r<2>(plan, a, stream); break;
diff --git a/tensor4all-rs_amd/csrc/tci2.hpp b/tensor4all-rs_amd/csrc/tci2.hpp
--- a/tensor4all-rs_amd/csrc/tci2.hpp
+++ b/tensor4all-rs_amd/csrc/tci2.hpp
@@ -121,10 +121,12 @@
     }
     std::array<uint64_t, 5> chain_stats{{0, 0, 0, 0, 0}};
     std::array<uint64_t, 4> chain_stats_ext{{0, 0, 0, 0}};
+    std::array<uint64_t, 3> chain_side_stats{{0, 0, 0}};
     const uint64_t* fill_stats() const { return fill_stats_; }
     const RookWork& rook_work() const { return rook_work_; }
     bool chain_enabled = true;
     bool chain_verify = false;
+    bool chain_sidecar = true;
     bool chain_event_timing = false;
 
     std::vector<double> evaluate(const uint32_t* idx, size_t n_pts);
diff --git a/tensor4all-rs_amd/csrc/tci2_chain.hip b/tensor4all-rs_amd/csrc/tci2_chain.hip
--- a/tensor4all-rs_amd/csrc/tci2_chain.hip
+++ b/tensor4all-rs_amd/csrc/tci2_chain.hip
@@ -305,7 +305,7 @@
     }
     chain_.ind.reserve(nb * ind_cap * (1 + K));
     chain_.ind_cnt.reserve(nb);
-    chain_.dep.reserve(dep_cap * (1 + K));
+    chain_.dep.reserve(2 * dep_cap * (1 + K));
     chain_.rowmap.reserve(dep_cap);
     chain_.pi.reserve(std::max<size_t>(pi_cap, 64 * 64));
     chain_.factors_stride = 0;
@@ -327,7 +327,7 @@
     const RrluBlock proto = RrluBlock::layout(steps_cap, Mcap, Ncap, true);
     chain_.blocks.reserve(nb * proto.bytes);
     chain_.hblocks.reserve(nb * proto.bytes);
-    chain_.dims.reserve(nb * 5 + 2);
+    chain_.dims.reserve(nb * 6 + 2);
     chain_.hdims.reserve(nb * 4);
     const bool timed = eng.prof.enabled;
     const bool timed_events = timed && chain_event_timing;
@@ -399,7 +399,7 @@
     c.zero_a = reinterpret_cast<uint64_t*>(chain_.blocks.get());
     c.zero_a_words = nb * proto.bytes / 8;
     c.zero_b = reinterpret_cast<uint64_t*>(chain_.dims.get());
-    c.zero_b_words = (nb * 5 * sizeof(int) + 7) / 8;
+    c.zero_b_words = (nb * 6 * sizeof(int) + 7) / 8;
 
     chain_.common = c;
     chain_.prepared = true;
@@ -503,7 +503,14 @@
             prep_dbg = chain_.walk_dbg.get();
             chain_.prep_dbg = true;
         }
+        static const bool no_sidecar = std::getenv("T4A_NO_CHAIN_SIDECAR") != nullptr;
+        const bool sidecar_ok = !no_sidecar && chain_sidecar;
+        unsigned* const side_elect = reinterpret_cast<unsigned*>(chain_.dims.get() + nb * 5);
+        const size_t dep_words = (size_t)c.dep_cap * (1 + K);
+        int dep_cur = 0;
+        bool side_pending = false;
         bool spec_pending = false;
+        ChainCommon cb = c;
         for (size_t k = 0; !walk && k < nb; ++k) {
             const size_t b = order[k];
             const RrluRoute& pl = plans[b];
@@ -527,8 +534,15 @@
                 pa.prev_colperm = pblk.col_perm();
                 pa.prev_token = tokens[pb];
             }
-            chain_prep_launch(c, pa, st);
-            if (!fused && !spec_here) chain_pi_launch(c, fn_dev_, (int)b, (int)dep_ub[b], (int)ind_ub[b], chain_.pi.get(), st);
+            cb.dep_code = chain_.dep.get() + dep_cur * dep_words;
+            cb.dep_acc = cb.dep_code + c.dep_cap;
+            if (side_pending) {
+                ++chain_side_stats[0];
+            } else {
+                chain_prep_launch(cb, pa, st);
+                ++chain_side_stats[1];
+            }
+            if (!fused && !spec_here) chain_pi_launch(cb, fn_dev_, (int)b, (int)dep_ub[b], (int)ind_ub[b], chain_.pi.get(), st);
             XcdSpecArgs sp;
             std::memset(&sp, 0, sizeof(sp));
             spec_pending = false;
@@ -539,7 +553,7 @@
                     const ChainTab& H = forward ? c.HI : c.HJ;
                     const size_t hsite = forward ? nx + 1 : nx;
                     sp.out = chain_.spec[(k + 1) & 1].get();
-                    sp.dep_acc = c.dep_acc;
+                    sp.dep_acc = cb.dep_acc;
                     sp.w_site = c.w + offset_[site];
                     sp.ext_acc = H.acc + hsite * cap * K;
                     sp.ext_cnt = use_extras ? H.cnt + hsite : nullptr;
@@ -554,15 +568,32 @@
             }
             FusedPi fp;
             fp.fn = fn_dev_;
-            fp.d_rowacc = c.dep_acc;
+            ChainSideArgs sd;
+            side_pending = false;
+            if (spec_pending && sidecar_ok && pl.kind == RrluKind::SingleXcd && rrlu_xcd2_has_sidecar(pl.xcd.RPT, pl.xcd.CPT)) {
+                const size_t nx = order[k + 1];
+                std::memset(&sd, 0, sizeof(sd));
+                sd.c = c;
+                sd.c.dep_code = chain_.dep.get() + (1 - dep_cur) * dep_words;
+                sd.c.dep_acc = sd.c.dep_code + c.dep_cap;
+                sd.prev_dep_code = cb.dep_code;
+                sd.prev_dep_acc = cb.dep_acc;
+                sd.b = (int)nx;
+                sd.prev_b = (int)b;
+                sd.elect = side_elect + nx;
+                side_pending = true;
+            }
+            fp.d_rowacc = cb.dep_acc;
             fp.d_colacc = c.ind_acc + b * ind_cap * K;
             fp.host_resident = false;
             const double* A = fused ? nullptr : (spec_here ? chain_.spec[k & 1].get() : chain_.pi.get());
             if (timed_events) T4A_HIP(hipEventRecord(chain_.t0[b], st));
             tokens[b] = eng.chain_rrlu(pl, forward, A, spec_here ? c.rowmap : nullptr, fused ? &fp : nullptr, c.dims + b * 4, chi, chain_.tol,
                                        chain_.one_site ? chain_.abs_tol : 0.0, blk, spec_pending ? &sp : nullptr,
-                                       chain_.factors_stride ? chain_.factors.get() + b * chain_.factors_stride : nullptr, chain_.urows.get());
+                                       chain_.factors_stride ? chain_.factors.get() + b * chain_.factors_stride : nullptr, chain_.urows.get(),
+                                       side_pending ? &sd : nullptr);
             if (timed_events) T4A_HIP(hipEventRecord(chain_.t1[b], st));
+            if (side_pending) dep_cur = 1 - dep_cur;
         }
         if (!walk) {
             const size_t pb = order[nb - 1];
@@ -576,7 +607,9 @@
             pa.prev_rowperm = pblk.row_perm();
             pa.prev_colperm = pblk.col_perm();
             pa.prev_token = tokens[pb];
-            chain_prep_launch(c, pa, st);
+            cb.dep_code = chain_.dep.get() + dep_cur * dep_words;
+            cb.dep_acc = cb.dep_code + c.dep_cap;
+            chain_prep_launch(cb, pa, st);
         }
         chain_.cores_batched = false;
         if (chain_.one_site && chain_.factors_stride && forward && nb <= (size_t)LUCI_LEFT_CORES_MAX_JOBS) {
@@ -811,6 +844,8 @@
                      t[5] * 0.01, (double)(t[6] - t[4] - t[5]) * 0.01);
     }
     chain_.prep_dbg = false;
+    for (size_t b = 0; b < nb; ++b)
+        if (chain_.hdims.get()[b * 4 + 3] == 1) ++chain_side_stats[2];
     const int mnew = 1 - chain_.mcur;
     const ChainTab ni = chain_mirror(mnew, 0), nj = chain_mirror(mnew, 1);
     long failed_k = -1;
diff --git a/tensor4all-rs_amd/python/t4a_amd/__init__.py b/tensor4all-rs_amd/python/t4a_amd/__init__.py
--- a/tensor4all-rs_amd/python/t4a_amd/__init__.py
+++ b/tensor4all-rs_amd/python/t4a_amd/__init__.py
@@ -739,10 +739,11 @@
         return [dict(code=int(r[0]), ms=float(r[1]), launches=float(r[2]), bytes=float(r[3]), steps=float(r[4])) for r in out[: n.value]]
 
 
-    def set_chain(self, enable=True, verify=False, event_timing=False, small_engine=True, small_stamps=False, fill_graph_relaxed=False, small_tile32=False):
+    def set_chain(self, enable=True, verify=False, event_timing=False, small_engine=True, small_stamps=False, fill_graph_relaxed=False, small_tile32=False,
+                  sidecar=True):
         _check(_lib.t4a_gpu_tci2_set_chain(self._h, c_int32(1 if enable else 0),
                                            c_int32((1 if verify else 0) | (2 if event_timing else 0) | (0 if small_engine else 4) | (8 if small_stamps else 0)
-                                                   | (16 if fill_graph_relaxed else 0) | (32 if small_tile32 else 0))))
+                                                   | (16 if fill_graph_relaxed else 0) | (32 if small_tile32 else 0) | (0 if sidecar else 64))))
 
     def set_callback_threads(self, n):
         _check(_lib.t4a_gpu_tci2_set_callback_threads(self._h, c_size_t(n)))
@@ -772,6 +773,12 @@
         return dict(half_sweeps=int(out[0]), bonds=int(out[1]), fell_back=int(out[2]), not_eligible=int(out[3]),
                     group_half_sweeps=int(out[4]), walked_sweeps=int(ext[0]), one_site_sweeps=int(ext[1]),
                     one_site_not_eligible=int(ext[2]), one_site_fell_back=int(ext[3]))
+
+
+    def chain_sidecar_stats(self):
+        out = np.zeros(3, dtype=np.uint64)
+        _check(_lib.t4a_gpu_tci2_chain_side_stats(self._h, _p(out)))
+        return dict(sidecar_bonds=int(out[0]), launched_bonds=int(out[1]), sidecar_give_ups=int(out[2]))
 
 
 def optimize_group(tcis, options, final_sweep1site=True):
```
